# jasonleebrown/machisplin

Hardware: AMD Instinct MI355X
Metric: grid Mcells/s (ensemble+TPS predict) + TPS-solve GFLOP/s (higher is better)
Workload: dtype f64; 1 GPU; cfg3: 5000 stations, 3 covariates, 10000x10000 grid, 6-model ensemble + TPS residual correction; stations=5000, covariates=3 x float32 planes resident in HBM, rf_trees=500, tps_mode=global (one fit on all stations, GCV lambda, V73:748-753), parallelism=rowband1 + bcast(coef) + 1 all-gather

## Files before the change

include/machisplin_hip.h:

```cpp
#ifndef MACHISPLIN_HIP_H
#define MACHISPLIN_HIP_H

#include <stdint.h>

#if defined(__GNUC__)
#define MHS_API __attribute__((visibility("default")))
#else
#define MHS_API
#endif

#ifdef __cplusplus
extern "C" {
#endif

enum {
    MHS_OK = 0,
    MHS_ERR_INVALID = 1,
    MHS_ERR_HIP = 2,
    MHS_ERR_NODEVICE = 3,
    MHS_ERR_NUMERIC = 4,
    MHS_ERR_ALLOC = 5
};

enum { MHS_F64 = 0, MHS_F32 = 1, MHS_I16 = 2 };

enum {
    MHS_GCV_FIELDS = 0,
    MHS_GCV_CONVERGED = 1
};

typedef struct mhs_grid {
    double xmin, ymax;
    double xres, yres;
    int64_t nrow, ncol;
} mhs_grid;

typedef struct mhs_tps mhs_tps;
typedef struct mhs_model mhs_model;

MHS_API const char *mhs_last_error(void);
MHS_API const char *mhs_version(void);
MHS_API int mhs_init(int device);
MHS_API int mhs_shutdown(void);
MHS_API int mhs_device_count(int *count);
MHS_API int mhs_sync(void *stream);
MHS_API int mhs_fit_reserve_cus(int n_cus, int *previous);
MHS_API int mhs_timer_start(void *stream);
MHS_API int mhs_timer_stop(void *stream, double *elapsed_ms);

MHS_API int mhs_tps_fit(const double *xy, const double *y, int64_t N, double lambda,
                int gcv_mode, mhs_tps **out);
MHS_API int mhs_tps_fit_many(const double *const *xy, const double *const *y, const int64_t *N, int64_t count,
                             double lambda, int gcv_mode, mhs_tps **out, int *status);
MHS_API int mhs_tps_reduction_cache(int enable);
MHS_API int mhs_host_gcv_tridiag(const double *diag, const double *offdiag, const double *g,
                                 int64_t m, int64_t n_unique, int64_t n_obs, double pure_ss,
                                 double lambda, int gcv_mode, double *lambda_out,
                                 double *gcv_out, double *eff_df_out, double *q_out);
MHS_API int mhs_host_gcv_band(const double *ab, int bw, const double *g, int64_t m, int64_t n_unique,
                              int64_t n_obs, double pure_ss, double lambda, int gcv_mode,
                              double *lambda_out, double *gcv_out, double *eff_df_out, double *q_out);
MHS_API int mhs_band32_reduce(const double *B, const double *g, int64_t m, double *ab, double *gq,
                              const double *r, double *Qr, int *breakdown);
MHS_API int mhs_band32_gcv_terms(const double *ab, const double *g, int64_t m, const double *lambda, int n_lambda,
                                 int deriv, double *neg, double *tr_inv, double *gM2g);
MHS_API int mhs_band32_solve(const double *ab, const double *g, int64_t m, double lambda, double *q);
MHS_API int mhs_tps_from_coef(const double *knots_uv ,
                      const double *c, const double *d3, int64_t n, double lambda,
                      const double *center2, const double *scale2, mhs_tps **out);
MHS_API int mhs_tps_size(const mhs_tps *t, int64_t *n);
MHS_API int mhs_tps_get(const mhs_tps *t, double *c, double *d3, double *knots_uv, double *lambda,
                double *center2, double *scale2, double *eff_df, double *gcv);
MHS_API int mhs_tps_free(mhs_tps *t);

MHS_API int mhs_tps_predict_grid(const mhs_tps *t, const mhs_grid *g, int64_t r0, int64_t r1,
                         int64_t c0, int64_t c1, double *out_host);
MHS_API int mhs_tps_eval_mode(int mode);
MHS_API int mhs_tps_eval_plan(const mhs_tps *t, int *tile_cols, int *tile_rows, int64_t *node_pairs,
                      int64_t *cell_pairs);
MHS_API int mhs_tps_predict_grid_dev(const mhs_tps *t, const mhs_grid *g, int64_t r0, int64_t r1,
                             int64_t c0, int64_t c1, double *out_dev, int64_t ld, void *stream);
MHS_API int mhs_tps_predict_rows_dev(const mhs_tps *t, const mhs_grid *g, int64_t r0, int64_t r1, int64_t c0, int64_t c1,
                                     int64_t b0, int64_t b1, double *out_dev, int64_t ld, void *stream);
MHS_API int mhs_tps_predict_points(const mhs_tps *t, const double *xy, int64_t n, double *out_host);

#define MHS_TPS_SE_MAX_N 2048
MHS_API int mhs_tps_sigma2(const mhs_tps *t, double *sigma2);
MHS_API int mhs_tps_predict_se_points(const mhs_tps *t, const double *xy, int64_t n, double sigma2, double *out_host);
MHS_API int mhs_tps_predict_se_grid(const mhs_tps *t, const mhs_grid *g, int64_t r0, int64_t r1, int64_t c0, int64_t c1,
                                    double sigma2, double *out_host);
MHS_API int mhs_tps_predict_se_grid_dev(const mhs_tps *t, const mhs_grid *g, int64_t r0, int64_t r1, int64_t c0, int64_t c1,
                                        double sigma2, double *out_dev, int64_t ld, void *stream);


MHS_API int mhs_lm_load(const double *coef, int p, mhs_model **out);
MHS_API int mhs_lm_fit(const double *X, const double *y, int64_t n, int p, double *coef);
MHS_API int mhs_svr_fit(const double *X, const double *y, int64_t n, int p, double sigma, double C, double epsilon,
                        double tol, int64_t max_iter, double *beta, double *b, double *x_center, double *x_scale,
                        double *y_center, double *y_scale, int64_t *n_iter);
MHS_API int mhs_nnet_fit(const double *X, const double *y, int64_t n, int p, int size, double *wts, int maxit,
                         double abstol, double reltol, double *value, int *counts, int *fail);
MHS_API int mhs_nnet_load(const double *wts, int p, int size, double y_scale, double y_shift,
                          mhs_model **out);
MHS_API int mhs_earth_load(const double *coef, const int32_t *dirs, const double *cuts, int nterms,
                           int p, mhs_model **out);
MHS_API int mhs_svr_load(const double *alpha, const double *sv, int64_t nsv, int p, double b,
                         double sigma, const double *x_center, const double *x_scale,
                         double y_center, double y_scale, mhs_model **out);
MHS_API int mhs_gbm_load(double init_f, int64_t n_trees, const int64_t *tree_offsets,
                         const int32_t *split_var, const double *split_val, const int32_t *left,
                         const int32_t *right, const int32_t *missing, int p, mhs_model **out);
MHS_API int mhs_gbm_grow_many(int count, const double *const *X, const double *const *y, const int64_t *n, int p,
                              const int32_t *const *bags, const int64_t *bag_size, int n_new, int interaction_depth,
                              int n_minobsinnode, double shrinkage, int first_call, double *const *F, double *init_f,
                              int64_t *const *tree_offsets, int32_t *const *split_var, double *const *split_val,
                              int32_t *const *left, int32_t *const *right, int32_t *const *missing);
MHS_API int mhs_rf_load(int64_t n_trees, const int64_t *tree_offsets, const int32_t *left,
                        const int32_t *right, const int32_t *status, const int32_t *best_var,
                        const double *split, const double *node_pred, int p, mhs_model **out);
MHS_API int mhs_model_free(mhs_model *m);

typedef struct mhs_stack {
    const void *data;
    int32_t n_layers;
    int32_t dtype;
    int64_t plane_stride;
    int64_t ld;
    double nodata;
} mhs_stack;

MHS_API int mhs_predict_dev(const mhs_model *m, const mhs_grid *g, const mhs_stack *covars,
                            int64_t r0, int64_t r1, int64_t c0, int64_t c1, double weight,
                            int accumulate, double *out_dev, int64_t ld, void *stream);
MHS_API int mhs_members_predict_dev(const mhs_model *const *models, const double *weights, int n_models,
                            const mhs_grid *g, const mhs_stack *covars, int64_t r0, int64_t r1, int64_t c0,
                            int64_t c1, int accumulate, double *out_dev, int64_t ld, void *stream);
MHS_API int mhs_ensemble_predict_dev(const mhs_model *const *models, const double *weights,
                                     int n_models, double wt_total, const mhs_grid *g,
                                     const mhs_stack *covars, int64_t r0, int64_t r1, int64_t c0,
                                     int64_t c1, double *out_dev, int64_t ld, void *stream);
MHS_API int mhs_ensemble_predict(const mhs_model *const *models, const double *weights,
                                 int n_models, double wt_total, const mhs_grid *g,
                                 const mhs_stack *covars, int64_t r0, int64_t r1, int64_t c0,
                                 int64_t c1, double *out_host);
MHS_API int mhs_predict_points(const mhs_model *m, const double *X, int64_t n, double *out_host);
MHS_API int mhs_gbm_staged_points(const mhs_model *m, const double *X, int64_t n, int step, double *out_host);
MHS_API int mhs_model_info(const mhs_model *m, int *kind, int *p, int64_t *n_trees);

MHS_API int mhs_gbm_probe_last(const mhs_model *m, int64_t *cost, int64_t *count);
MHS_API int mhs_residual_points(const mhs_model *const *models, const double *weights, int n_models, double wt_total,
                                const double *X, const double *resp, int64_t n, double *out_host);

MHS_API int mhs_scale_add_dev(const double *a, double divisor, const double *b, double *out,
                              int64_t n, void *stream);


MHS_API int mhs_crop_window(const mhs_grid *g, const double *ext4, int64_t *win4);
MHS_API int mhs_step3_tile_windows(const mhs_grid *g, int64_t tile_edge, double fit_overlap,
                                   double keep_overlap, int64_t *nRx, int64_t *nCx,
                                   int64_t *fit_win, int64_t *keep_win, int64_t capacity);
MHS_API int mhs_tiles_create_windows(const mhs_grid *g, int64_t out_ncol, int64_t out_nrow,
                                     double feather_d, double *boxes, int64_t *win);
MHS_API int mhs_seam_count(int64_t nRx, int64_t nCx, int64_t *n_seams);
MHS_API int mhs_cells_from_xy(const mhs_grid *g, const double *xy, int64_t n, int64_t *rows,
                              int64_t *cols);
MHS_API int mhs_mosaic_feather_dev(const mhs_grid *g, int64_t nRx, int64_t nCx,
                                   const int64_t *tile_win, const double *const *tile_dev,
                                   int merge_mode, double *out_dev, int64_t ld,
                                   int64_t *seam_win_out, void *stream);
MHS_API int mhs_mosaic_feather(const mhs_grid *g, int64_t nRx, int64_t nCx, const int64_t *tile_win,
                               const double *const *tile_host, int merge_mode, double *out_host);
MHS_API int mhs_gather_cells_dev(const double *plane_dev, int64_t ld, const int64_t *rows,
                                 const int64_t *cols, int64_t n, double *out_host, void *stream);

MHS_API int mhs_tps_surface(const mhs_grid *g, const double *xy, const double *resid, int64_t n,
                            const double *cov1_at_stations, int64_t tile_edge, double lambda,
                            int gcv_mode, double *out_host, int64_t *tiles_out);
MHS_API int mhs_tps_tiles_dev(const mhs_grid *g, const double *xy, const double *resid, int64_t n,
                      const double *cov1_at_stations, int64_t tile_edge, double lambda, int gcv_mode,
                      const int64_t *tile_ids, int64_t n_ids, double *const *out_dev_ptrs);
MHS_API int mhs_tps_surface_dev(const mhs_grid *g, const double *xy, const double *resid, int64_t n,
                                const double *cov1_at_stations, int64_t tile_edge, double lambda,
                                int gcv_mode, double *out_dev, int64_t ld, int64_t *tiles_out,
                                void *stream);
MHS_API int mhs_tps_surface_se(const mhs_grid *g, const double *xy, const double *resid, int64_t n,
                               const double *cov1_at_stations, int64_t tile_edge, double lambda, int gcv_mode,
                               double *out_host, int64_t *tiles_out);
MHS_API int mhs_tps_surface_se_dev(const mhs_grid *g, const double *xy, const double *resid, int64_t n,
                                   const double *cov1_at_stations, int64_t tile_edge, double lambda,
                                   int gcv_mode, double *out_dev, int64_t ld, int64_t *tiles_out,
                                   void *stream);

MHS_API int mhs_init_devices(int n_devices, const int *device_ids);
MHS_API int mhs_device_slots(int *n_slots, int *device_ids );

typedef struct mhs_multi_stack mhs_multi_stack;
MHS_API int mhs_multi_stack_create(const mhs_grid *g, const mhs_stack *covars_host, double slot0_share,
                                   mhs_multi_stack **out);
MHS_API int mhs_multi_stack_free(mhs_multi_stack *ms);
MHS_API int mhs_plan_row_bands(int64_t nrow, int n_slots, double slot0_share, int64_t *r0, int64_t *r1, int64_t *band,
                               int64_t *lead);
MHS_API int mhs_multi_stack_bands(const mhs_multi_stack *ms, int *n_slots, int64_t *r0 , int64_t *r1 );

typedef struct mhs_mltps_info {
    double rsq_model, rsq_final;
    double lambda;
    int64_t n_knots;
    int64_t tiles_rows, tiles_cols;
    int32_t used_tps;
    int32_t n_slots;
    int32_t collective;
    int32_t reserved_;
    int64_t band_r0[16], band_r1[16];
    double band_ms[16];
    double tiles_ms[16];
    double fit_ms;
    double step_ms;
    double upload_ms, download_ms;
    double suggested_slot0_share;
    int64_t tiles_pulled_bytes[16];
    int32_t tiles_owned[16];
} mhs_mltps_info;

MHS_API int mhs_mltps_grid_multi_dev(const mhs_model *const *models, const double *weights, int n_models,
                                     double wt_total, mhs_multi_stack *ms, const double *X, const double *resp,
                                     int64_t n, int64_t tile_edge, double lambda, int gcv_mode, int gather,
                                     mhs_mltps_info *info );
MHS_API int mhs_multi_final_download(const mhs_multi_stack *ms, double *final_host);
MHS_API int mhs_multi_final_dev(const mhs_multi_stack *ms, int slot, double **band_dev, int64_t *r0, int64_t *r1,
                                double **full_dev);
MHS_API int mhs_multi_trim(void);
MHS_API int mhs_mltps_grid_multi(const mhs_model *const *models, const double *weights, int n_models, double wt_total,
                                 const mhs_grid *g, const mhs_stack *covars_host, const double *X, const double *resp,
                                 int64_t n, int64_t tile_edge, double lambda, int gcv_mode, double slot0_share,
                                 double *final_host, mhs_mltps_info *info );

typedef struct mhs_unit {
    const mhs_model *const *models;
    const double *weights;
    int32_t n_models, reserved_;
    double wt_total;
    const double *X, *resp;
    int64_t n;
} mhs_unit;
typedef struct mhs_units_info {
    int32_t n_slots, reserved_;
    int64_t n_units;
    double step_ms, unit_ms_sum, unit_ms_max;
    double slot_ms[16];
} mhs_units_info;
MHS_API int mhs_tiles_units_multi(const mhs_grid *g, const mhs_stack *covars_host, int64_t out_ncol, int64_t out_nrow,
                                  double feather_d, int n_layers, const mhs_unit *units, int tps, int64_t tile_edge,
                                  double lambda, int gcv_mode, double *const *merged_host, double *rsq,
                                  mhs_units_info *info );

typedef struct mhs_tiff_info {
    int64_t width, height;
    int32_t bits, sample_format;
    int32_t compression, n_ifd;
    int32_t dtype;
    int32_t has_geo;
    double nodata;
    double xmin, ymax, xres, yres;
} mhs_tiff_info;
MHS_API int mhs_tiff_info_read(const char *path, int ifd, mhs_tiff_info *out);
MHS_API int mhs_tiff_read_host(const char *path, int ifd, void *out, int64_t out_bytes);
MHS_API int mhs_tiff_read_dev(const char *path, int ifd, void *out_dev, int64_t ld_elems, void *stream);
MHS_API int mhs_tiff_write_f32_host(const char *path, const mhs_grid *g, const float *data, double nodata,
                                    int compression);
MHS_API int mhs_tiff_write_f32_dev(const char *path, const mhs_grid *g, const double *plane_dev, int64_t ld,
                                   double nodata, int compression, void *stream);
MHS_API int mhs_tfw_read(const char *path, double *six);

#ifdef __cplusplus
}
#endif
#endif
```

machisplin_amd/_lib.py:

```python
from __future__ import annotations

import atexit
import ctypes as C
import os
import threading

_HERE = os.path.dirname(os.path.abspath(__file__))
LIB_PATH = os.path.join(_HERE, "libmachisplin_hip.so")

OK, ERR_INVALID, ERR_HIP, ERR_NODEVICE, ERR_NUMERIC, ERR_ALLOC = range(6)
F64, F32, I16 = 0, 1, 2
GCV_FIELDS, GCV_CONVERGED = 0, 1


class MhsError(RuntimeError):
    def __init__(self, code: int, msg: str):
        super().__init__(f"[mhs status {code}] {msg}")
        self.code = code


class Grid(C.Structure):
    _fields_ = [("xmin", C.c_double), ("ymax", C.c_double), ("xres", C.c_double),
                ("yres", C.c_double), ("nrow", C.c_int64), ("ncol", C.c_int64)]


class Stack(C.Structure):
    _fields_ = [("data", C.c_void_p), ("n_layers", C.c_int32), ("dtype", C.c_int32),
                ("plane_stride", C.c_int64), ("ld", C.c_int64), ("nodata", C.c_double)]


class TiffInfo(C.Structure):
    _fields_ = [("width", C.c_int64), ("height", C.c_int64), ("bits", C.c_int32), ("sample_format", C.c_int32),
                ("compression", C.c_int32), ("n_ifd", C.c_int32), ("dtype", C.c_int32), ("has_geo", C.c_int32),
                ("nodata", C.c_double), ("xmin", C.c_double), ("ymax", C.c_double), ("xres", C.c_double),
                ("yres", C.c_double)]


class MltpsInfo(C.Structure):
    _fields_ = [("rsq_model", C.c_double), ("rsq_final", C.c_double), ("lambda_", C.c_double), ("n_knots", C.c_int64),
                ("tiles_rows", C.c_int64), ("tiles_cols", C.c_int64), ("used_tps", C.c_int32), ("n_slots", C.c_int32),
                ("collective", C.c_int32), ("reserved_", C.c_int32), ("band_r0", C.c_int64 * 16), ("band_r1", C.c_int64 * 16),
                ("band_ms", C.c_double * 16), ("tiles_ms", C.c_double * 16), ("fit_ms", C.c_double), ("step_ms", C.c_double),
                ("upload_ms", C.c_double), ("download_ms", C.c_double), ("suggested_slot0_share", C.c_double),
                ("tiles_pulled_bytes", C.c_int64 * 16), ("tiles_owned", C.c_int32 * 16)]


class Unit(C.Structure):
    _fields_ = [("models", C.POINTER(C.c_void_p)), ("weights", C.POINTER(C.c_double)), ("n_models", C.c_int32),
                ("reserved_", C.c_int32), ("wt_total", C.c_double), ("X", C.c_void_p), ("resp", C.c_void_p), ("n", C.c_int64)]


class UnitsInfo(C.Structure):
    _fields_ = [("n_slots", C.c_int32), ("reserved_", C.c_int32), ("n_units", C.c_int64), ("step_ms", C.c_double),
                ("unit_ms_sum", C.c_double), ("unit_ms_max", C.c_double), ("slot_ms", C.c_double * 16)]


_dp = C.POINTER(C.c_double)
_vp = C.c_void_p
_i64 = C.c_int64

SIGNATURES = {
    "mhs_last_error": (C.c_char_p, []),
    "mhs_version": (C.c_char_p, []),
    "mhs_init": (C.c_int, [C.c_int]),
    "mhs_shutdown": (C.c_int, []),
    "mhs_device_count": (C.c_int, [C.POINTER(C.c_int)]),
    "mhs_sync": (C.c_int, [_vp]),
    "mhs_tps_reduction_cache": (C.c_int, [C.c_int]),
    "mhs_fit_reserve_cus": (C.c_int, [C.c_int, C.POINTER(C.c_int)]),
    "mhs_timer_start": (C.c_int, [_vp]),
    "mhs_timer_stop": (C.c_int, [_vp, _dp]),
    "mhs_tps_fit": (C.c_int, [_vp, _vp, _i64, C.c_double, C.c_int, C.POINTER(_vp)]),
    "mhs_tps_fit_many": (C.c_int, [_vp, _vp, _vp, _i64, C.c_double, C.c_int, _vp, _vp]),
    "mhs_host_gcv_tridiag": (C.c_int, [_vp, _vp, _vp, _i64, _i64, _i64, C.c_double, C.c_double, C.c_int,
                                       _dp, _dp, _dp, _vp]),
    "mhs_host_gcv_band": (C.c_int, [_vp, C.c_int, _vp, _i64, _i64, _i64, C.c_double, C.c_double, C.c_int,
                                    _dp, _dp, _dp, _vp]),
    "mhs_band32_reduce": (C.c_int, [_vp, _vp, _i64, _vp, _vp, _vp, _vp, C.POINTER(C.c_int)]),
    "mhs_band32_gcv_terms": (C.c_int, [_vp, _vp, _i64, _vp, C.c_int, C.c_int, _vp, _vp, _vp]),
    "mhs_band32_solve": (C.c_int, [_vp, _vp, _i64, C.c_double, _vp]),
    "mhs_tps_from_coef": (C.c_int, [_vp, _vp, _vp, _i64, C.c_double, _vp, _vp, C.POINTER(_vp)]),
    "mhs_tps_size": (C.c_int, [_vp, C.POINTER(_i64)]),
    "mhs_tps_get": (C.c_int, [_vp, _vp, _vp, _vp, _dp, _vp, _vp, _dp, _dp]),
    "mhs_tps_free": (C.c_int, [_vp]),
    "mhs_tps_predict_grid": (C.c_int, [_vp, C.POINTER(Grid), _i64, _i64, _i64, _i64, _vp]),
    "mhs_tps_predict_grid_dev": (C.c_int, [_vp, C.POINTER(Grid), _i64, _i64, _i64, _i64, _vp, _i64, _vp]),
    "mhs_tps_predict_rows_dev": (C.c_int, [_vp, C.POINTER(Grid), _i64, _i64, _i64, _i64, _i64, _i64, _vp, _i64, _vp]),
    "mhs_tps_predict_points": (C.c_int, [_vp, _vp, _i64, _vp]),
    "mhs_tps_sigma2": (C.c_int, [_vp, _dp]),
    "mhs_tps_predict_se_points": (C.c_int, [_vp, _vp, _i64, C.c_double, _vp]),
    "mhs_tps_predict_se_grid": (C.c_int, [_vp, C.POINTER(Grid), _i64, _i64, _i64, _i64, C.c_double, _vp]),
    "mhs_tps_predict_se_grid_dev": (C.c_int, [_vp, C.POINTER(Grid), _i64, _i64, _i64, _i64, C.c_double, _vp, _i64, _vp]),
    "mhs_tps_eval_mode": (C.c_int, [C.c_int]),
    "mhs_tps_eval_plan": (C.c_int, [_vp, C.POINTER(C.c_int), C.POINTER(C.c_int), C.POINTER(_i64), C.POINTER(_i64)]),
    "mhs_lm_load": (C.c_int, [_vp, C.c_int, C.POINTER(_vp)]),
    "mhs_lm_fit": (C.c_int, [_vp, _vp, _i64, C.c_int, _vp]),
    "mhs_svr_fit": (C.c_int, [_vp, _vp, _i64, C.c_int, C.c_double, C.c_double, C.c_double, C.c_double, _i64, _vp, _vp, _vp, _vp,
                              _vp, _vp, _vp]),
    "mhs_nnet_fit": (C.c_int, [_vp, _vp, _i64, C.c_int, C.c_int, _vp, C.c_int, C.c_double, C.c_double, _vp, _vp, _vp]),
    "mhs_nnet_load": (C.c_int, [_vp, C.c_int, C.c_int, C.c_double, C.c_double, C.POINTER(_vp)]),
    "mhs_earth_load": (C.c_int, [_vp, _vp, _vp, C.c_int, C.c_int, C.POINTER(_vp)]),
    "mhs_svr_load": (C.c_int, [_vp, _vp, _i64, C.c_int, C.c_double, C.c_double, _vp, _vp, C.c_double,
                               C.c_double, C.POINTER(_vp)]),
    "mhs_gbm_load": (C.c_int, [C.c_double, _i64, _vp, _vp, _vp, _vp, _vp, _vp, C.c_int, C.POINTER(_vp)]),
    "mhs_gbm_grow_many": (C.c_int, [C.c_int, _vp, _vp, _vp, C.c_int, _vp, _vp, C.c_int, C.c_int, C.c_int, C.c_double, C.c_int, _vp, _vp,
                                    _vp, _vp, _vp, _vp, _vp, _vp]),
    "mhs_rf_load": (C.c_int, [_i64, _vp, _vp, _vp, _vp, _vp, _vp, _vp, C.c_int, C.POINTER(_vp)]),
    "mhs_model_free": (C.c_int, [_vp]),
    "mhs_predict_dev": (C.c_int, [_vp, C.POINTER(Grid), C.POINTER(Stack), _i64, _i64, _i64, _i64,
                                  C.c_double, C.c_int, _vp, _i64, _vp]),
    "mhs_members_predict_dev": (C.c_int, [C.POINTER(_vp), _dp, C.c_int, C.POINTER(Grid), C.POINTER(Stack), C.c_int64, C.c_int64,
                                          C.c_int64, C.c_int64, C.c_int, C.c_void_p, C.c_int64, C.c_void_p]),
    "mhs_ensemble_predict_dev": (C.c_int, [C.POINTER(_vp), _dp, C.c_int, C.c_double, C.POINTER(Grid),
                                           C.POINTER(Stack), _i64, _i64, _i64, _i64, _vp, _i64, _vp]),
    "mhs_ensemble_predict": (C.c_int, [C.POINTER(_vp), _dp, C.c_int, C.c_double, C.POINTER(Grid),
                                       C.POINTER(Stack), _i64, _i64, _i64, _i64, _vp]),
    "mhs_predict_points": (C.c_int, [_vp, _vp, _i64, _vp]),
    "mhs_gbm_staged_points": (C.c_int, [_vp, _vp, _i64, C.c_int, _vp]),
    "mhs_model_info": (C.c_int, [_vp, _vp, _vp, _vp]),
    "mhs_gbm_probe_last": (C.c_int, [_vp, _vp, _vp]),
    "mhs_residual_points": (C.c_int, [_vp, _vp, C.c_int, C.c_double, _vp, _vp, _i64, _vp]),
    "mhs_scale_add_dev": (C.c_int, [_vp, C.c_double, _vp, _vp, _i64, _vp]),
    "mhs_crop_window": (C.c_int, [C.POINTER(Grid), _vp, _vp]),
    "mhs_step3_tile_windows": (C.c_int, [C.POINTER(Grid), _i64, C.c_double, C.c_double, C.POINTER(_i64),
                                         C.POINTER(_i64), _vp, _vp, _i64]),
    "mhs_tiles_create_windows": (C.c_int, [C.POINTER(Grid), _i64, _i64, C.c_double, _vp, _vp]),
    "mhs_seam_count": (C.c_int, [_i64, _i64, C.POINTER(_i64)]),
    "mhs_cells_from_xy": (C.c_int, [C.POINTER(Grid), _vp, _i64, _vp, _vp]),
    "mhs_mosaic_feather_dev": (C.c_int, [C.POINTER(Grid), _i64, _i64, _vp, C.POINTER(_vp), C.c_int, _vp, _i64,
                                         _vp, _vp]),
    "mhs_mosaic_feather": (C.c_int, [C.POINTER(Grid), _i64, _i64, _vp, C.POINTER(_vp), C.c_int, _vp]),
    "mhs_gather_cells_dev": (C.c_int, [_vp, _i64, _vp, _vp, _i64, _vp, _vp]),
    "mhs_tiff_info_read": (C.c_int, [C.c_char_p, C.c_int, C.POINTER(TiffInfo)]),
    "mhs_tiff_read_host": (C.c_int, [C.c_char_p, C.c_int, _vp, _i64]),
    "mhs_tiff_read_dev": (C.c_int, [C.c_char_p, C.c_int, _vp, _i64, _vp]),
    "mhs_tiff_write_f32_host": (C.c_int, [C.c_char_p, C.POINTER(Grid), _vp, C.c_double, C.c_int]),
    "mhs_tiff_write_f32_dev": (C.c_int, [C.c_char_p, C.POINTER(Grid), _vp, _i64, C.c_double, C.c_int, _vp]),
    "mhs_tfw_read": (C.c_int, [C.c_char_p, _dp]),
    "mhs_tps_surface": (C.c_int, [C.POINTER(Grid), _vp, _vp, _i64, _vp, _i64, C.c_double, C.c_int, _vp, _vp]),
    "mhs_tps_tiles_dev": (C.c_int, [C.POINTER(Grid), _vp, _vp, _i64, _vp, _i64, C.c_double, C.c_int, _vp, _i64, _vp]),
    "mhs_tps_surface_dev": (C.c_int, [C.POINTER(Grid), _vp, _vp, _i64, _vp, _i64, C.c_double, C.c_int, _vp, _i64,
                                      _vp, _vp]),
    "mhs_tps_surface_se": (C.c_int, [C.POINTER(Grid), _vp, _vp, _i64, _vp, _i64, C.c_double, C.c_int, _vp, _vp]),
    "mhs_tps_surface_se_dev": (C.c_int, [C.POINTER(Grid), _vp, _vp, _i64, _vp, _i64, C.c_double, C.c_int, _vp, _i64,
                                         _vp, _vp]),
    "mhs_init_devices": (C.c_int, [C.c_int, C.POINTER(C.c_int)]),
    "mhs_device_slots": (C.c_int, [C.POINTER(C.c_int), C.POINTER(C.c_int)]),
    "mhs_multi_stack_create": (C.c_int, [C.POINTER(Grid), C.POINTER(Stack), C.c_double, C.POINTER(_vp)]),
    "mhs_multi_stack_free": (C.c_int, [_vp]),
    "mhs_plan_row_bands": (C.c_int, [_i64, C.c_int, C.c_double, _vp, _vp, C.POINTER(_i64), C.POINTER(_i64)]),
    "mhs_multi_trim": (C.c_int, []),
    "mhs_multi_stack_bands": (C.c_int, [_vp, C.POINTER(C.c_int), _vp, _vp]),
    "mhs_mltps_grid_multi_dev": (C.c_int, [C.POINTER(_vp), _dp, C.c_int, C.c_double, _vp, _vp, _vp, _i64, _i64, C.c_double,
                                           C.c_int, C.c_int, C.POINTER(MltpsInfo)]),
    "mhs_multi_final_download": (C.c_int, [_vp, _vp]),
    "mhs_multi_final_dev": (C.c_int, [_vp, C.c_int, C.POINTER(_vp), C.POINTER(_i64), C.POINTER(_i64), C.POINTER(_vp)]),
    "mhs_mltps_grid_multi": (C.c_int, [C.POINTER(_vp), _dp, C.c_int, C.c_double, C.POINTER(Grid), C.POINTER(Stack), _vp, _vp,
                                       _i64, _i64, C.c_double, C.c_int, C.c_double, _vp, C.POINTER(MltpsInfo)]),
    "mhs_tiles_units_multi": (C.c_int, [C.POINTER(Grid), C.POINTER(Stack), _i64, _i64, C.c_double, C.c_int, C.POINTER(Unit),
                                        C.c_int, _i64, C.c_double, C.c_int, C.POINTER(_vp), _vp, C.POINTER(UnitsInfo)]),
}

_lock = threading.Lock()
_lib = None
_inited_device = None


def _hip_runtimes_mapped():
    libs = set()
    try:
        with open("/proc/self/maps") as f:
            for line in f:
                if "libamdhip64" in line:
                    libs.add(line.split()[-1])
    except OSError:
        pass
    return libs


def load() -> C.CDLL:
    global _lib
    with _lock:
        if _lib is not None:
            return _lib
        if not os.path.exists(LIB_PATH):
            raise ImportError(
                f"{LIB_PATH} is missing: build it with `python -c 'import __graft_entry__ as g; g.build()'` "
                "(or `make -C machisplin_amd/csrc`).  machisplin_amd has no CPU fallback.")
        import torch
        lib = C.CDLL(LIB_PATH, mode=C.RTLD_GLOBAL)
        for name, (res, args) in SIGNATURES.items():
            fn = getattr(lib, name)
            fn.restype = res
            fn.argtypes = args
        mapped = _hip_runtimes_mapped()
        if len(mapped) > 1:
            raise ImportError(f"two HIP runtimes are mapped into this process: {sorted(mapped)}")
        _lib = lib
        return lib


def check(rc: int) -> None:
    if rc != OK:
        raise MhsError(rc, load().mhs_last_error().decode(errors="replace"))


def init(device: int | None = None) -> int:
    global _inited_device
    lib = load()
    if device is None:
        if _inited_device is not None:
            return _inited_device
        device = int(os.environ.get("LOCAL_RANK", "0"))
    if _inited_device == device:
        return device
    check(lib.mhs_init(int(device)))
    if _inited_device is None:
        atexit.register(_shutdown)
    _inited_device = device
    return device


def _shutdown() -> None:
    global _inited_device
    if _lib is not None and _inited_device is not None:
        _lib.mhs_shutdown()
        _inited_device = None


def lib() -> C.CDLL:
    if _inited_device is None:
        init()
    return load()


def ptr(a) -> int:
    if a is None:
        return None
    if hasattr(a, "data_ptr"):
        return a.data_ptr()
    return a.ctypes.data
```

machisplin_amd/csrc/common.h:

```cpp
#pragma once
#include <hip/hip_runtime.h>
#include <stdint.h>
#include <chrono>
#include <memory>
#include <mutex>
#include <string>
#include <vector>
#include "machisplin_hip.h"

namespace mhs {

void set_error(const char *fmt, ...);
int hip_fail(hipError_t e, const char *what, const char *file, int line);

#define MHS_HIP(call)                                                        \
    do {                                                                     \
        hipError_t e_ = (call);                                              \
        if (e_ != hipSuccess) return mhs::hip_fail(e_, #call, __FILE__, __LINE__); \
    } while (0)

#define MHS_REQUIRE(cond, msg)                                               \
    do {                                                                     \
        if (!(cond)) { mhs::set_error("%s: %s", __func__, msg); return MHS_ERR_INVALID; } \
    } while (0)

constexpr int LOG_TAB_BITS = 10;
constexpr int LOG_TAB_N = 1 << LOG_TAB_BITS;

constexpr int FIT_PANEL_CUS = 32;
struct FitLane {
    hipStream_t s = nullptr, s2 = nullptr;
    hipStream_t ms = nullptr, ms2 = nullptr;
    hipStream_t s2r = nullptr;
    std::vector<hipEvent_t> pool;
    char *arena = nullptr;
    size_t arena_cap = 0;
    double *pinned = nullptr;
};

struct Context {
    bool ready = false;
    int device = -1;
    hipStream_t stream = nullptr;
    std::vector<FitLane *> lanes;
    FitLane *batch = nullptr;
    double2 *log_tab = nullptr;
    double *exp_tab = nullptr;
    double *points_arena = nullptr;
    size_t points_arena_cap = 0;
    char *mosaic_arena[2] = {nullptr, nullptr};
    size_t mosaic_arena_cap[2] = {0, 0};
    double *surface_arena = nullptr;
    size_t surface_arena_cap = 0;
    hipEvent_t ev0 = nullptr, ev1 = nullptr;
    char *pipe_arena = nullptr;
    size_t pipe_arena_cap = 0;
    hipStream_t pipe_h2d = nullptr, pipe_d2h = nullptr, pipe_comp = nullptr;
    hipEvent_t pipe_in[8] = {}, pipe_done[8] = {}, pipe_out[8] = {};
    hipStream_t upload = nullptr;
    int n_cu = 0;
    int reserved_cus = 0;
    int masked_cus = 0;
    hipStream_t masked_stream = nullptr;
    std::vector<uint32_t> comp_mask;
    hipEvent_t mask_ev0 = nullptr, mask_ev1 = nullptr;
};
constexpr int MAX_SLOTS = 16;
int current_slot();
int slot_count();
int bind_slot(int slot);
struct SlotBind {
    int prev;
    explicit SlotBind(int slot) : prev(current_slot()) { (void)bind_slot(slot); }
    ~SlotBind() { (void)bind_slot(prev); }
    SlotBind(const SlotBind &) = delete;
    SlotBind &operator=(const SlotBind &) = delete;
};
std::mutex &pipe_mutex();
int host_pipe(size_t arena_bytes);
std::mutex &mask_mutex();
std::mutex &mosaic_mutex();
int cpu_budget();
int mosaic_lane();
void set_mosaic_lane(int lane);
Context &ctx();
Context &ctx_slot(int slot);
int fit_lane(int i, FitLane **out);
int batch_lane(FitLane **out);
std::mutex &batch_mutex();
int tps_fit_lane(FitLane &L, const double *xy, const double *y, int64_t N, double lambda, int gcv_mode,
                 int gcv_threads, mhs_tps **out);
void *pool_alloc(size_t bytes);
void pool_release(void *p);
void pool_clear();
int require_ready();
int mosaic_feather_impl(const mhs_grid *g, int64_t nRx, int64_t nCx, const int64_t *tile_win, const double *const *tile_dev,
                        int merge_mode, double *out_dev, int64_t ld, int64_t *seam_win_out, void *stream, bool finite_tiles,
                        int64_t row_lo = 0, int64_t row_hi = -1);
void reduction_cache_clear();
void multi_reset();
int h2d_sync(void *dst, const void *src, size_t bytes);
inline hipStream_t pick_stream(void *s) { return (hipStream_t)s; }
inline double now_ms() {
    return std::chrono::duration<double, std::milli>(std::chrono::steady_clock::now().time_since_epoch()).count();
}

template <typename T>
struct DevBuf {
    T *p = nullptr;
    size_t n = 0;
    DevBuf() = default;
    DevBuf(const DevBuf &) = delete;
    DevBuf &operator=(const DevBuf &) = delete;
    ~DevBuf() { if (p) (void)hipFree(p); }
    hipError_t alloc(size_t count) {
        if (p) { (void)hipFree(p); p = nullptr; }
        n = count;
        return hipMalloc((void **)&p, (count ? count : 1) * sizeof(T));
    }
    T *release() { T *q = p; p = nullptr; return q; }
};

struct Knot { double u, v, cw, pad; };

}

struct mhs_tps;
namespace mhs {
struct TpsPrep;
struct SeState;
void se_state_free(SeState *s);
int upload_knots(mhs_tps *t);
int tps_free_quiet(mhs_tps *t);
int tps_predict_rows_dev(const mhs_tps *t, const mhs_grid *g, int64_t r0, int64_t r1, int64_t c0, int64_t c1,
                         int64_t b0, int64_t b1, double *out_dev, int64_t ld, void *stream);
}

struct mhs_model;
namespace mhs {
int model_on_slot(const mhs_model *m, int slot, const mhs_model **out);
int members_rows_dev(const mhs_model *const *models, const double *weights, int n_models, int accumulate, int scale, double wt_total,
                     const mhs_grid *g, const void *buf, int64_t buf_r0, int64_t buf_r1, int n_layers, int dtype, int64_t ld,
                     double nodata, int64_t b0, int64_t b1, double *out_dev, int64_t ld_out, hipStream_t st);
int ensemble_band_dev(const mhs_model *const *models, const double *weights, int n_models, double wt_total, const mhs_grid *g,
                      const void *band_data, int n_layers, int dtype, int64_t ld, double nodata, int64_t b0, int64_t b1,
                      double *out_dev, int64_t ld_out, hipStream_t st);
}

struct mhs_tps {
    int64_t n = 0;
    double lambda = 0, eff_df = 0, gcv = 0;
    double center[2] = {0, 0}, scale[2] = {1, 1};
    double d[3] = {0, 0, 0};
    std::vector<double> c;
    std::vector<double> knots_uv;
    mhs::Knot *knots_dev = nullptr;
    struct FarPlan {
        double xmin = 0, ymax = 0, xres = 0, yres = 0;
        int64_t r0 = -1, r1 = -1, c0 = -1, c1 = -1;
        int tx = 0, ty = 0, ntx = 0, nty = 0;
        mhs::Knot *sorted_dev = nullptr;
        int *bin_start_dev = nullptr;
        double *nodes_dev = nullptr;
        double *lx_dev = nullptr, *ly_dev = nullptr;
        size_t nodes_cap = 0, bins_cap = 0, lx_cap = 0, ly_cap = 0;
        bool last_used = false;
        hipStream_t last_stream = nullptr;
        bool in_flight = false;
        int64_t node_pairs = 0, cell_pairs = 0;
    } far;
    std::mutex mu;
    std::shared_ptr<const mhs::TpsPrep> prep;
    mhs::SeState *se = nullptr;
};
```

machisplin_amd/csrc/multi.hip:

```cpp
#include <atomic>
#include <chrono>
#include <cmath>
#include <condition_variable>
#include <cstdio>
#include <cstdlib>
#include <cstring>
#include <deque>
#include <dlfcn.h>
#include <mutex>
#include <string>
#include <thread>
#include <vector>
#include "common.h"

using namespace mhs;

namespace {

constexpr int64_t BAND_ROWS_ALIGN = 16;

struct MultiSlot {
    hipStream_t s = nullptr;
    hipEvent_t e0 = nullptr, e1 = nullptr;
    hipStream_t u = nullptr;
    hipEvent_t up[5] = {}, dn[5] = {};
    hipStream_t h = nullptr;
};
MultiSlot g_ms[MAX_SLOTS];
std::mutex g_ms_mu;

int multi_slot(int slot, MultiSlot **out) {
    std::lock_guard<std::mutex> lk(g_ms_mu);
    MultiSlot &m = g_ms[slot];
    if (!m.s) {
        MHS_HIP(hipStreamCreateWithFlags(&m.s, hipStreamNonBlocking));
        MHS_HIP(hipEventCreate(&m.e0));
        MHS_HIP(hipEventCreate(&m.e1));
        int prio_lo = 0, prio_hi = 0;
        MHS_HIP(hipDeviceGetStreamPriorityRange(&prio_lo, &prio_hi));
        MHS_HIP(hipStreamCreateWithPriority(&m.u, hipStreamNonBlocking, prio_lo));
        MHS_HIP(hipStreamCreateWithPriority(&m.h, hipStreamNonBlocking, prio_lo));
        for (hipEvent_t &e : m.up) MHS_HIP(hipEventCreateWithFlags(&e, hipEventDisableTiming));
        for (hipEvent_t &e : m.dn) MHS_HIP(hipEventCreateWithFlags(&e, hipEventDisableTiming));
    }
    *out = &m;
    return MHS_OK;
}

typedef void *nccl_comm;
struct Rccl {
    void *h = nullptr;
    int (*CommInitAll)(nccl_comm *, int, const int *) = nullptr;
    int (*CommDestroy)(nccl_comm) = nullptr;
    int (*AllGather)(const void *, void *, size_t, int, nccl_comm, hipStream_t) = nullptr;
    const char *(*GetErrorString)(int) = nullptr;
    nccl_comm comm[MAX_SLOTS] = {};
    int n = 0;
    bool tried = false, usable = false;
    std::string why;
};
Rccl g_rccl;
std::mutex g_rccl_mu;
constexpr int NCCL_FLOAT64 = 8;

bool slots_distinct() {
    const int n = slot_count();
    for (int a = 0; a < n; ++a)
        for (int b = a + 1; b < n; ++b)
            if (ctx_slot(a).device == ctx_slot(b).device) return false;
    return true;
}

void rccl_prepare() {
    std::lock_guard<std::mutex> lk(g_rccl_mu);
    const int n = slot_count();
    if (g_rccl.tried && g_rccl.n == n) return;
    g_rccl.tried = true; g_rccl.usable = false; g_rccl.n = n;
    if (!slots_distinct()) { g_rccl.why = "slots share a physical device (RCCL needs one device per rank): peer copies instead"; return; }
    if (getenv("MHS_MULTI_NO_RCCL")) { g_rccl.why = "MHS_MULTI_NO_RCCL is set: peer copies instead"; return; }
    if (!g_rccl.h) {
        for (const char *name : {"librccl.so.1", "librccl.so", "/opt/rocm/lib/librccl.so.1"}) {
            g_rccl.h = dlopen(name, RTLD_NOW | RTLD_GLOBAL);
            if (g_rccl.h) break;
        }
        if (!g_rccl.h) { g_rccl.why = std::string("librccl not found: ") + dlerror(); return; }
        g_rccl.CommInitAll = (int (*)(nccl_comm *, int, const int *))dlsym(g_rccl.h, "ncclCommInitAll");
        g_rccl.CommDestroy = (int (*)(nccl_comm))dlsym(g_rccl.h, "ncclCommDestroy");
        g_rccl.AllGather = (int (*)(const void *, void *, size_t, int, nccl_comm, hipStream_t))dlsym(g_rccl.h, "ncclAllGather");
        g_rccl.GetErrorString = (const char *(*)(int))dlsym(g_rccl.h, "ncclGetErrorString");
        if (!g_rccl.CommInitAll || !g_rccl.CommDestroy || !g_rccl.AllGather) { g_rccl.why = "librccl lacks ncclCommInitAll / ncclAllGather"; return; }
    }
    int devs[MAX_SLOTS];
    for (int k = 0; k < n; ++k) devs[k] = ctx_slot(k).device;
    const int rc = g_rccl.CommInitAll(g_rccl.comm, n, devs);
    if (rc != 0) {
        g_rccl.why = std::string("ncclCommInitAll failed: ") + (g_rccl.GetErrorString ? g_rccl.GetErrorString(rc) : "?");
        return;
    }
    g_rccl.usable = true;
    g_rccl.why = "rccl";
}

void rccl_reset() {
    std::lock_guard<std::mutex> lk(g_rccl_mu);
    if (g_rccl.usable && g_rccl.CommDestroy)
        for (int k = 0; k < g_rccl.n; ++k) if (g_rccl.comm[k]) { (void)g_rccl.CommDestroy(g_rccl.comm[k]); g_rccl.comm[k] = nullptr; }
    g_rccl.tried = g_rccl.usable = false;
    g_rccl.n = 0;
}

struct Barrier {
    std::mutex mu;
    std::condition_variable cv;
    int n, waiting = 0;
    uint64_t phase = 0;
    explicit Barrier(int n_) : n(n_) {}
    void wait() {
        std::unique_lock<std::mutex> lk(mu);
        const uint64_t ph = phase;
        if (++waiting == n) { waiting = 0; ++phase; cv.notify_all(); }
        else cv.wait(lk, [&] { return phase != ph; });
    }
};

struct Team {
    int n;
    Barrier bar;
    std::atomic<int> rc{MHS_OK};
    std::mutex err_mu;
    std::string err;
    explicit Team(int n_) : n(n_), bar(n_) {}
    bool failed() const { return rc.load() != MHS_OK; }
    void fail(int code) {
        int expected = MHS_OK;
        if (rc.compare_exchange_strong(expected, code)) {
            std::lock_guard<std::mutex> lk(err_mu);
            err = mhs_last_error();
        }
    }
    template <typename F>
    int run(F body) {
        const int home = current_slot();
        std::vector<std::thread> th;
        auto wrap = [&](int slot) {
            SlotBind bind(slot);
            body(slot);
        };
        for (int k = 1; k < n; ++k) th.emplace_back(wrap, k);
        wrap(0);
        for (std::thread &t : th) t.join();
        (void)bind_slot(home);
        if (failed()) { set_error("%s", err.c_str()); return rc.load(); }
        return MHS_OK;
    }
};

#define TEAM_DO(team, expr)                                      \
    do {                                                         \
        if (!(team).failed()) { const int rc_ = (expr); if (rc_ != MHS_OK) (team).fail(rc_); } \
    } while (0)

struct BandPlan {
    int64_t band = 0, lead = 0;
    std::vector<int64_t> r0, r1;
};

BandPlan plan_bands(int64_t nrow, int n, double slot0_share) {
    BandPlan p;
    p.r0.assign((size_t)n, 0); p.r1.assign((size_t)n, 0);
    if (n == 1) { p.band = nrow; p.r1[0] = nrow; return p; }
    const int64_t even = (nrow + n - 1) / n;
    const int64_t align = even >= BAND_ROWS_ALIGN ? BAND_ROWS_ALIGN : 1;
    auto up = [&](int64_t v) { return (v + align - 1) / align * align; };
    auto equal = [&] {
        p.band = up(even); p.lead = 0;
        for (int k = 0; k < n; ++k) { p.r0[(size_t)k] = std::min<int64_t>(k * p.band, nrow); p.r1[(size_t)k] = std::min<int64_t>((k + 1) * p.band, nrow); }
    };
    if (std::isnan(slot0_share)) { equal(); return p; }
    const double sh = std::min(std::max(slot0_share, 0.0), 1.0);
    int64_t n0 = std::min<int64_t>(nrow, (int64_t)llround(sh * (double)nrow / (double)align) * align);
    const int64_t rest = nrow - n0, others = n - 1;
    const int64_t h = up((rest + others - 1) / others);
    if (n0 > h) { equal(); return p; }
    p.band = std::max(h, n0); p.lead = p.band - n0;
    p.r0[0] = 0; p.r1[0] = n0;
    for (int k = 1; k < n; ++k) {
        p.r0[(size_t)k] = std::min<int64_t>(n0 + (k - 1) * h, nrow);
        p.r1[(size_t)k] = std::min<int64_t>(n0 + k * h, nrow);
    }
    return p;
}

}

struct MultiBand {
    int64_t r0 = 0, r1 = 0;
    char *cov = nullptr;
    double *ens = nullptr;
    double *tot = nullptr;
    double *full = nullptr;
    double *tiles = nullptr;
    size_t tiles_cap = 0;
};

struct mhs_multi_stack {
    mhs_grid g{};
    int C = 0, dtype = 0;
    int64_t ld = 0;
    double nodata = NAN;
    int n = 0;
    int dev[MAX_SLOTS] = {};
    BandPlan plan;
    MultiBand b[MAX_SLOTS];
    int used_tps = 0;
    bool gathered = false;
    bool have_result = false;
    const mhs_stack *pending = nullptr;
    double *pending_out = nullptr;
    bool downloaded = false;
    double upload_ms = 0;
    double download_ms = 0;
};

namespace {

size_t elem_size(int dtype) { return dtype == MHS_F64 ? 8 : dtype == MHS_F32 ? 4 : 2; }

struct Balance { int n = 0; int64_t nrow = 0, ncol = 0, stations = 0; double share = NAN; };
Balance g_balance;
std::mutex g_balance_mu;

mhs_multi_stack *g_host_ms = nullptr;
std::mutex g_host_mu;
struct UnitsArena { char *base = nullptr; size_t cap = 0; };
UnitsArena g_units_arena[MAX_SLOTS];

constexpr int RING_BUFS = 8, SINK_THREADS = 3;
constexpr size_t RING_CHUNK = (size_t)8 << 20;
struct PinnedRing { char *buf[RING_BUFS] = {}; hipEvent_t ev[RING_BUFS] = {}; bool ok = false; };
PinnedRing g_ring[MAX_SLOTS];

int ring_prepare(int slot) {
    PinnedRing &R = g_ring[slot];
    if (R.ok) return MHS_OK;
    for (int b = 0; b < RING_BUFS; ++b) {
        if (!R.buf[b]) MHS_HIP(hipHostMalloc((void **)&R.buf[b], RING_CHUNK, hipHostMallocDefault));
        if (!R.ev[b]) MHS_HIP(hipEventCreateWithFlags(&R.ev[b], hipEventDisableTiming));
    }
    R.ok = true;
    return MHS_OK;
}

class HostSink {
  public:
    HostSink(int slot, hipStream_t st) : slot_(slot), st_(st), R_(g_ring[slot]) {
        for (int b = 0; b < RING_BUFS; ++b) free_[b] = true;
        const int nth = std::min(SINK_THREADS, std::max(1, cpu_budget() / (4 * std::max(1, slot_count()))));
        for (int w = 0; w < nth; ++w) th_.emplace_back([this] { work(); });
    }
    ~HostSink() {
        { std::lock_guard<std::mutex> lk(mu_); stop_ = true; }
        cv_.notify_all();
        for (std::thread &t : th_) t.join();
    }
    int download(void *dst, const void *src, size_t bytes) {
        size_t off = 0;
        for (int c = 0; off < bytes; ++c) {
            const size_t sz = std::min(RING_CHUNK, bytes - off);
            int b = -1;
            {
                std::unique_lock<std::mutex> lk(mu_);
                cv_.wait(lk, [&] { for (int q = 0; q < RING_BUFS; ++q) if (free_[q]) { b = q; return true; } return false; });
                free_[b] = false;
            }
            hipError_t e = hipMemcpyAsync(R_.buf[b], (const char *)src + off, sz, hipMemcpyDeviceToHost, st_);
            if (e == hipSuccess) e = hipEventRecord(R_.ev[b], st_);
            if (e != hipSuccess) {
                set_error("HostSink: %s", hipGetErrorString(e));
                std::lock_guard<std::mutex> lk(mu_);
                free_[b] = true; rc_ = MHS_ERR_HIP;
                break;
            }
            {
                std::lock_guard<std::mutex> lk(mu_);
                jobs_.push_back(Job{b, (char *)dst + off, sz});
                ++pending_;
            }
            cv_.notify_all();
            off += sz;
        }
        std::unique_lock<std::mutex> lk(mu_);
        cv_.wait(lk, [&] { return pending_ == 0; });
        return rc_;
    }

  private:
    struct Job { int b; char *dst; size_t sz; };
    void work() {
        SlotBind bind(slot_);
        for (;;) {
            Job j;
            {
                std::unique_lock<std::mutex> lk(mu_);
                cv_.wait(lk, [&] { return stop_ || !jobs_.empty(); });
                if (jobs_.empty()) return;
                j = jobs_.front(); jobs_.pop_front();
            }
            const hipError_t e = hipEventSynchronize(R_.ev[j.b]);
            if (e == hipSuccess) memcpy(j.dst, R_.buf[j.b], j.sz);
            {
                std::lock_guard<std::mutex> lk(mu_);
                if (e != hipSuccess) rc_ = MHS_ERR_HIP;
                free_[j.b] = true; --pending_;
            }
            cv_.notify_all();
        }
    }
    int slot_;
    hipStream_t st_;
    PinnedRing &R_;
    std::vector<std::thread> th_;
    std::mutex mu_;
    std::condition_variable cv_;
    std::deque<Job> jobs_;
    bool free_[RING_BUFS];
    int pending_ = 0, rc_ = MHS_OK;
    bool stop_ = false;
};

bool stack_current(const mhs_multi_stack *ms) {
    if (ms->n != slot_count()) return false;
    for (int k = 0; k < ms->n; ++k) if (!ctx_slot(k).ready || ctx_slot(k).device != ms->dev[k]) return false;
    return true;
}

int free_stack(mhs_multi_stack *ms) {
    if (!ms) return MHS_OK;
    if (!stack_current(ms)) { delete ms; return MHS_OK; }
    const int home = current_slot();
    for (int k = 0; k < ms->n; ++k) {
        (void)bind_slot(k);
        MultiBand &b = ms->b[k];
        if (g_ms[k].s) (void)hipStreamSynchronize(g_ms[k].s);
        for (void *q : {(void *)b.cov, (void *)b.ens, (void *)b.tot, (void *)b.full, (void *)b.tiles})
            if (q) (void)hipFree(q);
    }
    (void)bind_slot(home);
    delete ms;
    return MHS_OK;
}

}

static void trim_caches() {
    std::lock_guard<std::mutex> lk(g_host_mu);
    if (g_host_ms) { bool alive = true; for (int k = 0; k < g_host_ms->n; ++k) alive = alive && ctx_slot(k).ready; if (alive) free_stack(g_host_ms); else delete g_host_ms; }
    g_host_ms = nullptr;
    const int home = current_slot();
    for (int k = 0; k < MAX_SLOTS; ++k) {
        if (ctx_slot(k).ready) {
            (void)bind_slot(k);
            if (g_units_arena[k].base) { (void)hipDeviceSynchronize(); (void)hipFree(g_units_arena[k].base); }
            for (int b = 0; b < RING_BUFS; ++b) {
                if (g_ring[k].buf[b]) (void)hipHostFree(g_ring[k].buf[b]);
                if (g_ring[k].ev[b]) (void)hipEventDestroy(g_ring[k].ev[b]);
            }
        }
        g_units_arena[k] = UnitsArena();
        g_ring[k] = PinnedRing();
    }
    (void)bind_slot(home);
}

extern "C" int mhs_multi_trim(void) {
    if (int rc = require_ready()) return rc;
    trim_caches();
    return MHS_OK;
}

void mhs::multi_reset() {
    trim_caches();
    rccl_reset();
    std::lock_guard<std::mutex> lk(g_ms_mu);
    for (int k = 0; k < MAX_SLOTS; ++k) {
        MultiSlot &m = g_ms[k];
        if (!m.s) continue;
        if (ctx_slot(k).ready) {
            SlotBind bind(k);
            (void)hipStreamSynchronize(m.s); (void)hipStreamDestroy(m.s);
            (void)hipEventDestroy(m.e0); (void)hipEventDestroy(m.e1);
            if (m.u) { (void)hipStreamSynchronize(m.u); (void)hipStreamDestroy(m.u); }
            if (m.h) { (void)hipStreamSynchronize(m.h); (void)hipStreamDestroy(m.h); }
            for (hipEvent_t e : m.up) if (e) (void)hipEventDestroy(e);
            for (hipEvent_t e : m.dn) if (e) (void)hipEventDestroy(e);
        }
        m = MultiSlot();
    }
}

extern "C" {

static int stack_build(const mhs_grid *g, const mhs_stack *covars_host, double slot0_share, bool upload, mhs_multi_stack **out) {
    if (int rc = require_ready()) return rc;
    MHS_REQUIRE(g && covars_host && covars_host->data && out, "NULL argument");
    MHS_REQUIRE(g->nrow > 0 && g->ncol > 0 && g->xres > 0 && g->yres > 0, "bad grid geometry");
    MHS_REQUIRE(covars_host->n_layers >= 1 && covars_host->n_layers <= 64, "bad number of layers");
    MHS_REQUIRE(covars_host->dtype == MHS_F64 || covars_host->dtype == MHS_F32 || covars_host->dtype == MHS_I16, "bad stack dtype");
    MHS_REQUIRE(covars_host->ld >= g->ncol && covars_host->plane_stride >= covars_host->ld * g->nrow, "stack strides smaller than the grid");
    const int n = slot_count();
    mhs_multi_stack *ms = new mhs_multi_stack();
    ms->g = *g; ms->C = covars_host->n_layers; ms->dtype = covars_host->dtype; ms->ld = g->ncol; ms->nodata = covars_host->nodata;
    ms->n = n;
    for (int k = 0; k < n; ++k) ms->dev[k] = ctx_slot(k).device;
    ms->plan = plan_bands(g->nrow, n, slot0_share);
    const size_t esz = elem_size(ms->dtype);
    Team team(n);
    const int rc = team.run([&](int slot) {
        MultiBand &b = ms->b[slot];
        b.r0 = ms->plan.r0[(size_t)slot]; b.r1 = ms->plan.r1[(size_t)slot];
        const int64_t nb = b.r1 - b.r0;
        auto work = [&]() -> int {
            MultiSlot *S = nullptr;
            if (int rc2 = multi_slot(slot, &S)) return rc2;
            if (nb == 0) return MHS_OK;
            const size_t plane = (size_t)nb * (size_t)ms->ld * esz;
            MHS_HIP(hipMalloc((void **)&b.cov, plane * (size_t)ms->C));
            MHS_HIP(hipMalloc((void **)&b.ens, sizeof(double) * (size_t)nb * (size_t)g->ncol));
            MHS_HIP(hipMalloc((void **)&b.tot, sizeof(double) * (size_t)nb * (size_t)g->ncol));
            if (!upload) return MHS_OK;
            for (int k = 0; k < ms->C; ++k) {
                const char *src = (const char *)covars_host->data + ((size_t)k * covars_host->plane_stride + (size_t)b.r0 * covars_host->ld) * esz;
                if (covars_host->ld == g->ncol)
                    MHS_HIP(hipMemcpyAsync(b.cov + plane * k, src, plane, hipMemcpyHostToDevice, S->s));
                else
                    MHS_HIP(hipMemcpy2DAsync(b.cov + plane * k, (size_t)ms->ld * esz, src, (size_t)covars_host->ld * esz, (size_t)g->ncol * esz,
                                             (size_t)nb, hipMemcpyHostToDevice, S->s));
            }
            MHS_HIP(hipStreamSynchronize(S->s));
            return MHS_OK;
        };
        TEAM_DO(team, work());
    });
    if (rc) { free_stack(ms); return rc; }
    *out = ms;
    return MHS_OK;
}

int mhs_multi_stack_create(const mhs_grid *g, const mhs_stack *covars_host, double slot0_share, mhs_multi_stack **out) {
    return stack_build(g, covars_host, slot0_share, true, out);
}

int mhs_multi_stack_free(mhs_multi_stack *ms) { return free_stack(ms); }

int mhs_plan_row_bands(int64_t nrow, int n_slots, double slot0_share, int64_t *r0, int64_t *r1, int64_t *band, int64_t *lead) {
    MHS_REQUIRE(nrow > 0 && n_slots >= 1 && n_slots <= MAX_SLOTS && r0 && r1, "bad arguments");
    const BandPlan p = plan_bands(nrow, n_slots, slot0_share);
    for (int k = 0; k < n_slots; ++k) { r0[k] = p.r0[(size_t)k]; r1[k] = p.r1[(size_t)k]; }
    if (band) *band = p.band;
    if (lead) *lead = p.lead;
    return MHS_OK;
}

int mhs_multi_stack_bands(const mhs_multi_stack *ms, int *n_slots, int64_t *r0, int64_t *r1) {
    MHS_REQUIRE(ms && n_slots, "NULL argument");
    *n_slots = ms->n;
    for (int k = 0; k < ms->n; ++k) {
        if (r0) r0[k] = ms->b[k].r0;
        if (r1) r1[k] = ms->b[k].r1;
    }
    return MHS_OK;
}

}

namespace {

enum { BANDS_UP = 0, BANDS_UP_F64 = 1, BANDS_DOWN = 2 };
constexpr int MAX_SUB = 5;
int sub_bands(int64_t r0, int64_t r1, int mode, int64_t cut[MAX_SUB + 1]) {
    static const int pct[3][MAX_SUB] = {{4, 16, 40, 40, 0}, {3, 6, 13, 28, 50}, {48, 30, 14, 6, 2}};
    const int nq = mode == BANDS_UP ? 4 : 5;
    const int64_t nb = r1 - r0;
    cut[0] = r0;
    for (int q = 0, a = 0; q < nq; ++q) {
        a += pct[mode][q];
        cut[q + 1] = q == nq - 1 ? r1 : std::min(r1, std::max(cut[q], (r0 + nb * a / 100 + BAND_ROWS_ALIGN / 2) / BAND_ROWS_ALIGN * BAND_ROWS_ALIGN));
    }
    return nq;
}

struct Uploader {
    std::thread th;
    std::mutex mu;
    std::condition_variable cv;
    int issued = 0, rc = MHS_OK;
    std::string err;
    template <typename F>
    void start(int slot, int nq, F issue) {
        th = std::thread([this, slot, nq, issue] {
            SlotBind bind(slot);
            for (int q = 0; q < nq; ++q) {
                const int r = issue(q);
                std::lock_guard<std::mutex> lk(mu);
                if (r) { rc = r; err = mhs_last_error(); issued = nq; } else issued = q + 1;
                cv.notify_all();
                if (r) break;
            }
        });
    }
    int wait(int q) {
        std::unique_lock<std::mutex> lk(mu);
        cv.wait(lk, [&] { return issued > q; });
        if (rc) set_error("%s", err.c_str());
        return rc;
    }
    void join() { if (th.joinable()) th.join(); }
    ~Uploader() { join(); }
};

struct StepShared {
    std::vector<double> resid;
    double rsq_model = NAN, tss = NAN;
    int64_t nk = 0;
    std::vector<double> c, knots_uv;
    double d[3] = {0, 0, 0}, center[2] = {0, 0}, scale[2] = {1, 1}, lambda = NAN;
    int64_t nRx = 1, nCx = 1;
    std::vector<int64_t> fit_win, keep_win;
    std::vector<int> owner;
    std::vector<size_t> tile_cells;
    std::vector<int64_t> slot_off[MAX_SLOTS];
    size_t slot_need[MAX_SLOTS] = {};
    int64_t pulled_bytes[MAX_SLOTS] = {};
    std::vector<double> f_actual;
    int used_tps = 0;
    double rsq_final = NAN;
    double fit_ms = 0, band_ms[MAX_SLOTS] = {}, tiles_ms[MAX_SLOTS] = {}, upload_ms[MAX_SLOTS] = {}, download_ms[MAX_SLOTS] = {};
};

}

extern "C" {

int mhs_mltps_grid_multi_dev(const mhs_model *const *models, const double *weights, int n_models, double wt_total,
                             mhs_multi_stack *ms, const double *X, const double *resp, int64_t n, int64_t tile_edge,
                             double lambda, int gcv_mode, int gather, mhs_mltps_info *info) {
    if (int rc = require_ready()) return rc;
    MHS_REQUIRE(models && weights && n_models >= 1 && n_models <= 8 && ms && X && resp && n > 3, "bad arguments");
    MHS_REQUIRE(stack_current(ms), "the stack was built for another set of device slots");
    MHS_REQUIRE(wt_total != 0.0 && !std::isnan(wt_total), "wt_total must be non-zero");
    const int N = ms->n;
    const mhs_grid g = ms->g;
    const int p = ms->C + 2;
    int kind0 = 0, p0 = 0;
    for (int k = 0; k < n_models; ++k) {
        MHS_REQUIRE(models[k] != nullptr, "NULL model");
        if (int rc = mhs_model_info(models[k], &kind0, &p0, nullptr)) return rc;
        MHS_REQUIRE(p0 == p, "a model's predictor count does not match the stack (layers + 2)");
    }
    const double t_step0 = now_ms();
    const double *knots = X + (size_t)(p - 2) * (size_t)n;
    std::vector<int64_t> rows((size_t)n), cols((size_t)n);
    if (int rc = mhs_cells_from_xy(&g, knots, n, rows.data(), cols.data())) return rc;
    StepShared S;
    S.f_actual.assign((size_t)n, NAN);
    int64_t nt = 1;
    if (tile_edge > 0) {
        if (int rc = mhs_step3_tile_windows(&g, tile_edge, 0.2, 0.025, &S.nRx, &S.nCx, nullptr, nullptr, 0)) return rc;
        nt = S.nRx * S.nCx;
    }
    const bool tiled = nt > 1;
    if (tiled) {
        S.fit_win.resize((size_t)nt * 4); S.keep_win.resize((size_t)nt * 4);
        if (int rc = mhs_step3_tile_windows(&g, tile_edge, 0.2, 0.025, &S.nRx, &S.nCx, S.fit_win.data(), S.keep_win.data(), nt)) return rc;
        S.tile_cells.resize((size_t)nt);
        S.owner.assign((size_t)nt, 0);
        for (int k = 0; k < N; ++k) S.slot_off[k].assign((size_t)nt, -1);
        for (int64_t h = 0; h < nt; ++h) {
            const int64_t *kw = &S.keep_win[(size_t)h * 4];
            S.tile_cells[(size_t)h] = ((size_t)((kw[1] - kw[0]) * (kw[3] - kw[2])) + 31) & ~(size_t)31;
            int64_t best_rows = -1;
            for (int k = 0; k < N; ++k) {
                const int64_t ov = std::min(kw[1], ms->b[k].r1) - std::max(kw[0], ms->b[k].r0);
                if (ov > best_rows) { best_rows = ov; S.owner[(size_t)h] = k; }
            }
            for (int k = 0; k < N; ++k) {
                const bool reaches = ms->b[k].r1 > ms->b[k].r0 && kw[0] < ms->b[k].r1 && kw[1] > ms->b[k].r0;
                if (reaches || S.owner[(size_t)h] == k) { S.slot_off[k][(size_t)h] = (int64_t)S.slot_need[k]; S.slot_need[k] += S.tile_cells[(size_t)h]; }
            }
        }
    }
    if (gather) rccl_prepare();
    const bool use_rccl = gather && g_rccl.usable;
    std::vector<const mhs_model *> mods((size_t)N * (size_t)n_models);
    std::vector<mhs_tps *> tps((size_t)N, nullptr);
    Team team(N);
    const int rc = team.run([&](int slot) {
        MultiBand &b = ms->b[slot];
        const int64_t nb = b.r1 - b.r0;
        MultiSlot *M = nullptr;
        TEAM_DO(team, multi_slot(slot, &M));
        for (int k = 0; k < n_models; ++k) TEAM_DO(team, model_on_slot(models[k], slot, &mods[(size_t)slot * n_models + k]));
        const mhs_model *const *my = &mods[(size_t)slot * n_models];
        auto fit = [&]() -> int {
            S.resid.resize((size_t)n);
            if (int rc2 = mhs_residual_points(my, weights, n_models, wt_total, X, resp, n, S.resid.data())) return rc2;
            long double msum = 0.0L, ss = 0.0L, rs = 0.0L;
            for (int64_t i = 0; i < n; ++i) msum += resp[i];
            const double mean = (double)(msum / (long double)n);
            for (int64_t i = 0; i < n; ++i) { ss += (long double)((resp[i] - mean) * (resp[i] - mean)); rs += (long double)(S.resid[(size_t)i] * S.resid[(size_t)i]); }
            S.tss = (double)ss; S.rsq_model = 1.0 - (double)rs / (double)ss;
            if (tiled) return MHS_OK;
            const double t0 = now_ms();
            mhs_tps *t = nullptr;
            if (int rc2 = mhs_tps_fit(knots, S.resid.data(), n, lambda, gcv_mode, &t)) return rc2;
            S.fit_ms = now_ms() - t0;
            tps[0] = t;
            if (int rc2 = mhs_tps_size(t, &S.nk)) return rc2;
            S.c.resize((size_t)S.nk); S.knots_uv.resize((size_t)S.nk * 2);
            return mhs_tps_get(t, S.c.data(), S.d, S.knots_uv.data(), &S.lambda, S.center, S.scale, nullptr, nullptr);
        };
        const bool piped = ms->pending && ms->pending_out;
        const int banded = n_models > 1 ? n_models - 1 : 1;
        Uploader up;
        if (ms->pending && nb > 0 && !team.failed()) {
            const mhs_stack *h = ms->pending;
            const size_t esz = elem_size(ms->dtype), plane = (size_t)nb * (size_t)ms->ld * esz;
            int64_t cut[MAX_SUB + 1];
            const int nq = sub_bands(b.r0, b.r1, ms->dtype == MHS_F64 ? BANDS_UP_F64 : BANDS_UP, cut);
            const double t0 = now_ms();
            up.start(slot, nq, [=, &S](int q) -> int {
                const int64_t rows_q = cut[q + 1] - cut[q];
                for (int k = 0; k < ms->C && rows_q > 0; ++k) {
                    const char *src = (const char *)h->data + ((size_t)k * h->plane_stride + (size_t)cut[q] * h->ld) * esz;
                    char *dst = b.cov + plane * k + (size_t)(cut[q] - b.r0) * (size_t)ms->ld * esz;
                    if (h->ld == g.ncol)
                        MHS_HIP(hipMemcpyAsync(dst, src, (size_t)rows_q * (size_t)ms->ld * esz, hipMemcpyHostToDevice, M->u));
                    else
                        MHS_HIP(hipMemcpy2DAsync(dst, (size_t)ms->ld * esz, src, (size_t)h->ld * esz, (size_t)g.ncol * esz, (size_t)rows_q,
                                                 hipMemcpyHostToDevice, M->u));
                }
                MHS_HIP(hipEventRecord(M->up[q], M->u));
                if (q == nq - 1) S.upload_ms[slot] = now_ms() - t0;
                return MHS_OK;
            });
            std::thread fitter;
            int fit_rc = MHS_OK;
            std::string fit_err;
            if (slot == 0)
                fitter = std::thread([&] {
                    SlotBind bind(slot);
                    fit_rc = fit();
                    if (fit_rc) fit_err = mhs_last_error();
                });
            auto launch = [&]() -> int {
                MHS_HIP(hipEventRecord(M->e0, M->s));
                for (int q = 0; q < nq; ++q) {
                    if (int rc2 = up.wait(q)) return rc2;
                    MHS_HIP(hipStreamWaitEvent(M->s, M->up[q], 0));
                    if (int rc2 = members_rows_dev(my, weights, banded, 0, 0, wt_total, &g, b.cov, b.r0, b.r1, ms->C, ms->dtype, ms->ld, ms->nodata,
                                                   cut[q], cut[q + 1], b.ens + (size_t)(cut[q] - b.r0) * (size_t)g.ncol, g.ncol, M->s)) return rc2;
                }
                if (!piped) {
                    if (int rc2 = members_rows_dev(my + banded, weights + banded, n_models - banded, 1, 1, wt_total, &g, b.cov, b.r0, b.r1,
                                                   ms->C, ms->dtype, ms->ld, ms->nodata, b.r0, b.r1, b.ens, g.ncol, M->s)) return rc2;
                    MHS_HIP(hipEventRecord(M->e1, M->s));
                }
                return MHS_OK;
            };
            TEAM_DO(team, launch());
            if (fitter.joinable()) {
                fitter.join();
                if (fit_rc) { set_error("%s", fit_err.c_str()); team.fail(fit_rc); }
            }
            up.join();
            if (team.failed()) (void)hipStreamSynchronize(M->u);
        } else {
            if (nb > 0 && !team.failed()) {
                auto launch = [&]() -> int {
                    MHS_HIP(hipEventRecord(M->e0, M->s));
                    if (int rc2 = ensemble_band_dev(my, weights, n_models, wt_total, &g, b.cov, ms->C, ms->dtype, ms->ld, ms->nodata, b.r0, b.r1,
                                                    b.ens, g.ncol, M->s)) return rc2;
                    MHS_HIP(hipEventRecord(M->e1, M->s));
                    return MHS_OK;
                };
                TEAM_DO(team, launch());
            }
            if (slot == 0) TEAM_DO(team, fit());
        }
        team.bar.wait();
        auto down = [&]() -> int {
            int64_t cut[MAX_SUB + 1];
            const int nd = sub_bands(b.r0, b.r1, BANDS_DOWN, cut);
            for (int q = 0; q < nd; ++q) {
                const size_t off = (size_t)(cut[q] - b.r0) * (size_t)g.ncol;
                if (cut[q + 1] > cut[q]) {
                    if (int rc2 = members_rows_dev(my + banded, weights + banded, n_models - banded, 1, 1, wt_total, &g, b.cov, b.r0, b.r1, ms->C,
                                                   ms->dtype, ms->ld, ms->nodata, cut[q], cut[q + 1], b.ens + off, g.ncol, M->s)) return rc2;
                    if (int rc2 = mhs_scale_add_dev(b.ens + off, 1.0, b.tot + off, b.tot + off, (cut[q + 1] - cut[q]) * g.ncol, M->s)) return rc2;
                }
                MHS_HIP(hipEventRecord(M->dn[q], M->s));
            }
            MHS_HIP(hipEventRecord(M->e1, M->s));
            const double t0 = now_ms();
            for (int q = 0; q < nd; ++q) {
                if (cut[q + 1] == cut[q]) continue;
                const size_t off = (size_t)(cut[q] - b.r0) * (size_t)g.ncol;
                MHS_HIP(hipStreamWaitEvent(M->u, M->dn[q], 0));
                if (q == nd - 1) S.download_ms[slot] = -now_ms();
                MHS_HIP(hipMemcpyAsync(ms->pending_out + (size_t)b.r0 * (size_t)g.ncol + off, b.tot + off,
                                       sizeof(double) * (size_t)(cut[q + 1] - cut[q]) * (size_t)g.ncol, hipMemcpyDeviceToHost, M->u));
            }
            MHS_HIP(hipStreamSynchronize(M->u));
            S.download_ms[slot] = S.download_ms[slot] < 0 ? S.download_ms[slot] + now_ms() : now_ms() - t0;
            return MHS_OK;
        };
        if (!tiled) {
            if (slot != 0 && nb > 0)
                TEAM_DO(team, mhs_tps_from_coef(S.knots_uv.data(), S.c.data(), S.d, S.nk, S.lambda, S.center, S.scale, &tps[(size_t)slot]));
            if (nb > 0)
                TEAM_DO(team, tps_predict_rows_dev(tps[(size_t)slot], &g, 0, g.nrow, 0, g.ncol, b.r0, b.r1, b.tot, g.ncol, M->s));
            if (piped && nb > 0) {
                const int rcd = team.failed() ? MHS_OK : down();
                if (rcd) { (void)hipStreamSynchronize(M->u); team.fail(rcd); }
            }
        } else {
            const double t0 = now_ms();
            auto my_tiles = [&]() -> int {
                if (b.tiles_cap < S.slot_need[slot]) {
                    if (b.tiles) { MHS_HIP(hipStreamSynchronize(M->s)); MHS_HIP(hipFree(b.tiles)); b.tiles = nullptr; b.tiles_cap = 0; }
                    MHS_HIP(hipMalloc((void **)&b.tiles, sizeof(double) * S.slot_need[slot]));
                    b.tiles_cap = S.slot_need[slot];
                }
                std::vector<int64_t> ids;
                std::vector<double *> outs;
                for (int64_t h = 0; h < nt; ++h)
                    if (S.owner[(size_t)h] == slot) { ids.push_back(h); outs.push_back(b.tiles + S.slot_off[slot][(size_t)h]); }
                if (ids.empty()) return MHS_OK;
                return mhs_tps_tiles_dev(&g, knots, S.resid.data(), n, X , tile_edge, lambda, gcv_mode,
                                         ids.data(), (int64_t)ids.size(), outs.data());
            };
            TEAM_DO(team, my_tiles());
            S.tiles_ms[slot] = now_ms() - t0;
            team.bar.wait();
            auto bring = [&]() -> int {
                if (nb == 0) return MHS_OK;
                std::vector<const double *> ptrs((size_t)nt, nullptr);
                for (int64_t h = 0; h < nt; ++h) {
                    const int64_t *kw = &S.keep_win[(size_t)h * 4];
                    if (!(kw[0] < b.r1 && kw[1] > b.r0)) continue;
                    const int o = S.owner[(size_t)h];
                    ptrs[(size_t)h] = b.tiles + S.slot_off[slot][(size_t)h];
                    if (o == slot) continue;
                    const size_t bytes = sizeof(double) * S.tile_cells[(size_t)h];
                    MHS_HIP(hipMemcpyPeerAsync(b.tiles + S.slot_off[slot][(size_t)h], ctx_slot(slot).device,
                                               ms->b[o].tiles + S.slot_off[o][(size_t)h], ctx_slot(o).device, bytes, M->s));
                    S.pulled_bytes[slot] += (int64_t)bytes;
                }
                return mosaic_feather_impl(&g, S.nRx, S.nCx, S.keep_win.data(), ptrs.data(), 0, b.tot, g.ncol, nullptr, M->s, true, b.r0, b.r1);
            };
            TEAM_DO(team, bring());
            if (piped && nb > 0) {
                const int rcd = team.failed() ? MHS_OK : down();
                if (rcd) { (void)hipStreamSynchronize(M->u); team.fail(rcd); }
            }
        }
        if (nb > 0 && !team.failed()) {
            auto step5 = [&]() -> int {
                if (!piped) if (int rc2 = mhs_scale_add_dev(b.ens, 1.0, b.tot, b.tot, nb * g.ncol, M->s)) return rc2;
                std::vector<int64_t> rr, cc, idx;
                for (int64_t i = 0; i < n; ++i)
                    if (rows[(size_t)i] >= b.r0 && rows[(size_t)i] < b.r1 && cols[(size_t)i] >= 0) {
                        rr.push_back(rows[(size_t)i] - b.r0); cc.push_back(cols[(size_t)i]); idx.push_back(i);
                    }
                std::vector<double> f(rr.size());
                if (int rc2 = mhs_gather_cells_dev(b.tot, g.ncol, rr.data(), cc.data(), (int64_t)rr.size(), f.data(), M->s)) return rc2;
                for (size_t q = 0; q < idx.size(); ++q) S.f_actual[(size_t)idx[q]] = f[q];
                return MHS_OK;
            };
            TEAM_DO(team, step5());
        }
        team.bar.wait();
        if (slot == 0 && !team.failed()) {
            long double rs = 0.0L;
            for (int64_t i = 0; i < n; ++i) { const double e = resp[i] - S.f_actual[(size_t)i]; rs += (long double)(e * e); }
            S.rsq_final = 1.0 - (double)rs / S.tss;
            S.used_tps = S.rsq_final > S.rsq_model ? 1 : 0;
        }
        team.bar.wait();
        const bool go = !team.failed();
        if (piped && nb > 0 && go && !S.used_tps) {
            auto resend = [&]() -> int {
                MHS_HIP(hipMemcpyAsync(ms->pending_out + (size_t)b.r0 * (size_t)g.ncol, b.ens, sizeof(double) * (size_t)nb * (size_t)g.ncol,
                                       hipMemcpyDeviceToHost, M->s));
                return MHS_OK;
            };
            TEAM_DO(team, resend());
        }
        if (gather && go) {
            auto stitch = [&]() -> int {
                const int64_t band = ms->plan.band;
                if (!b.full) MHS_HIP(hipMalloc((void **)&b.full, sizeof(double) * (size_t)band * (size_t)N * (size_t)g.ncol));
                const double *src = S.used_tps ? b.tot : b.ens;
                double *mine = b.full + ((size_t)ms->plan.lead + (size_t)b.r0) * (size_t)g.ncol;
                if (nb > 0) MHS_HIP(hipMemcpyAsync(mine, src, sizeof(double) * (size_t)nb * (size_t)g.ncol, hipMemcpyDeviceToDevice, M->s));
                return MHS_OK;
            };
            int rcs = stitch();
            if (rcs) team.fail(rcs);
            team.bar.wait();
            const bool go2 = !team.failed();
            if (go2 && use_rccl) {
                const size_t count = (size_t)ms->plan.band * (size_t)g.ncol;
                const int rcn = g_rccl.AllGather(b.full + (size_t)slot * count, b.full, count, NCCL_FLOAT64, g_rccl.comm[slot], M->s);
                if (rcn != 0) { set_error("ncclAllGather failed: %s", g_rccl.GetErrorString ? g_rccl.GetErrorString(rcn) : "?"); team.fail(MHS_ERR_HIP); }
            } else if (go2 && nb > 0) {
                auto push = [&]() -> int {
                    const double *mine = b.full + ((size_t)ms->plan.lead + (size_t)b.r0) * (size_t)g.ncol;
                    for (int o = 0; o < N; ++o) {
                        if (o == slot) continue;
                        double *dst = ms->b[o].full + ((size_t)ms->plan.lead + (size_t)b.r0) * (size_t)g.ncol;
                        MHS_HIP(hipMemcpyPeerAsync(dst, ctx_slot(o).device, mine, ctx_slot(slot).device, sizeof(double) * (size_t)nb * (size_t)g.ncol, M->s));
                    }
                    return MHS_OK;
                };
                rcs = push();
                if (rcs) team.fail(rcs);
            }
        }
        if (M) (void)hipStreamSynchronize(M->s);
        if (nb > 0 && M && !team.failed()) {
            float ms_f = 0.f;
            if (hipEventElapsedTime(&ms_f, M->e0, M->e1) == hipSuccess) S.band_ms[slot] = (double)ms_f;
        }
        team.bar.wait();
        if (tps[(size_t)slot]) { (void)mhs_tps_free(tps[(size_t)slot]); tps[(size_t)slot] = nullptr; }
    });
    if (ms->pending) {
        ms->downloaded = !rc && ms->pending_out;
        ms->pending = nullptr; ms->pending_out = nullptr;
        ms->upload_ms = ms->download_ms = 0;
        for (int k = 0; k < N; ++k) { ms->upload_ms = std::max(ms->upload_ms, S.upload_ms[k]); ms->download_ms = std::max(ms->download_ms, S.download_ms[k]); }
    }
    if (rc) return rc;
    ms->used_tps = S.used_tps;
    ms->gathered = gather != 0;
    ms->have_result = true;
    const double step_ms = now_ms() - t_step0;
    double suggested = NAN;
    if (N > 1 && !tiled) {
        double ms_per_row = 0.0;
        int64_t rows_timed = 0;
        for (int k = 0; k < N; ++k) if (ms->b[k].r1 > ms->b[k].r0) { ms_per_row += S.band_ms[k]; rows_timed += ms->b[k].r1 - ms->b[k].r0; }
        if (rows_timed > 0 && ms_per_row > 0) {
            const double cells_ms = ms_per_row / (double)rows_timed * (double)g.nrow;
            const double s0 = 1.0 / N - S.fit_ms * (N - 1) / ((double)N * cells_ms);
            suggested = std::min(std::max(s0, 0.0), 1.0 / N);
            std::lock_guard<std::mutex> lk(g_balance_mu);
            const bool same_shape = g_balance.n == N && g_balance.nrow == g.nrow && g_balance.ncol == g.ncol && g_balance.stations == n;
            if (!same_shape || !(fabs(suggested - g_balance.share) <= 0.05 / (double)N))
                g_balance = Balance{N, g.nrow, g.ncol, n, suggested};
        }
    }
    if (info) {
        memset(info, 0, sizeof(*info));
        info->rsq_model = S.rsq_model; info->rsq_final = S.rsq_final; info->lambda = tiled ? NAN : S.lambda;
        info->n_knots = tiled ? 0 : S.nk; info->used_tps = S.used_tps; info->n_slots = N;
        info->tiles_rows = S.nRx; info->tiles_cols = S.nCx;
        info->collective = !gather ? 0 : use_rccl ? 1 : 2;
        info->fit_ms = S.fit_ms; info->step_ms = step_ms; info->suggested_slot0_share = suggested;
        for (int k = 0; k < N; ++k) {
            info->band_r0[k] = ms->b[k].r0; info->band_r1[k] = ms->b[k].r1; info->band_ms[k] = S.band_ms[k]; info->tiles_ms[k] = S.tiles_ms[k];
            info->tiles_pulled_bytes[k] = S.pulled_bytes[k];
            info->tiles_owned[k] = 0;
            for (size_t h = 0; h < S.owner.size(); ++h) if (S.owner[h] == k) ++info->tiles_owned[k];
        }
    }
    return MHS_OK;
}

int mhs_multi_final_download(const mhs_multi_stack *ms, double *final_host) {
    if (int rc = require_ready()) return rc;
    MHS_REQUIRE(ms && final_host && ms->have_result, "no result to download");
    MHS_REQUIRE(stack_current(ms), "the stack was built for another set of device slots");
    Team team(ms->n);
    return team.run([&](int slot) {
        const MultiBand &b = ms->b[slot];
        const int64_t nb = b.r1 - b.r0;
        auto work = [&]() -> int {
            if (nb == 0) return MHS_OK;
            MultiSlot *M = nullptr;
            if (int rc2 = multi_slot(slot, &M)) return rc2;
            const double *src = ms->used_tps ? b.tot : b.ens;
            MHS_HIP(hipMemcpyAsync(final_host + (size_t)b.r0 * (size_t)ms->g.ncol, src, sizeof(double) * (size_t)nb * (size_t)ms->g.ncol,
                                   hipMemcpyDeviceToHost, M->s));
            MHS_HIP(hipStreamSynchronize(M->s));
            return MHS_OK;
        };
        TEAM_DO(team, work());
    });
}

int mhs_multi_final_dev(const mhs_multi_stack *ms, int slot, double **band_dev, int64_t *r0, int64_t *r1, double **full_dev) {
    MHS_REQUIRE(ms && slot >= 0 && slot < ms->n && ms->have_result, "bad arguments");
    const MultiBand &b = ms->b[slot];
    if (band_dev) *band_dev = ms->used_tps ? b.tot : b.ens;
    if (r0) *r0 = b.r0;
    if (r1) *r1 = b.r1;
    if (full_dev) *full_dev = (ms->gathered && b.full) ? b.full + (size_t)ms->plan.lead * (size_t)ms->g.ncol : nullptr;
    return MHS_OK;
}

int mhs_mltps_grid_multi(const mhs_model *const *models, const double *weights, int n_models, double wt_total, const mhs_grid *g,
                         const mhs_stack *covars_host, const double *X, const double *resp, int64_t n, int64_t tile_edge,
                         double lambda, int gcv_mode, double slot0_share, double *final_host, mhs_mltps_info *info) {
    if (int rc = require_ready()) return rc;
    MHS_REQUIRE(g && covars_host && final_host, "NULL argument");
    double share = slot0_share;
    if (std::isnan(share)) {
        std::lock_guard<std::mutex> lk(g_balance_mu);
        if (g_balance.n == slot_count() && g_balance.nrow == g->nrow && g_balance.ncol == g->ncol && g_balance.stations == n) share = g_balance.share;
    }
    MHS_REQUIRE(covars_host->data && g->nrow > 0 && g->ncol > 0, "bad arguments");
    MHS_REQUIRE(covars_host->dtype == MHS_F64 || covars_host->dtype == MHS_F32 || covars_host->dtype == MHS_I16, "bad stack dtype");
    MHS_REQUIRE(covars_host->ld >= g->ncol && covars_host->plane_stride >= covars_host->ld * g->nrow, "stack strides smaller than the grid");
    std::lock_guard<std::mutex> lk(g_host_mu);
    const double t0 = now_ms();
    const BandPlan want = plan_bands(g->nrow, slot_count(), share);
    mhs_multi_stack *ms = g_host_ms;
    if (ms && !(stack_current(ms) && ms->g.nrow == g->nrow && ms->g.ncol == g->ncol && ms->C == covars_host->n_layers &&
                ms->dtype == covars_host->dtype && ms->plan.r0 == want.r0 && ms->plan.r1 == want.r1)) {
        free_stack(ms);
        ms = g_host_ms = nullptr;
    }
    if (!ms) {
        if (int rc = stack_build(g, covars_host, share, false, &ms)) return rc;
        g_host_ms = ms;
    }
    ms->g = *g; ms->nodata = covars_host->nodata; ms->have_result = false;
    ms->pending = covars_host;
    ms->pending_out = final_host;
    ms->downloaded = false;
    const double t1 = now_ms();
    int rc = mhs_mltps_grid_multi_dev(models, weights, n_models, wt_total, ms, X, resp, n, tile_edge, lambda, gcv_mode, 0, info);
    ms->pending = nullptr; ms->pending_out = nullptr;
    const double t2 = now_ms();
    if (!rc && !ms->downloaded) rc = mhs_multi_final_download(ms, final_host);
    if (info && !rc) { info->upload_ms = (t1 - t0) + ms->upload_ms; info->download_ms = ms->downloaded ? ms->download_ms : now_ms() - t2; }
    return rc;
}

}

namespace {

struct UnitSlot {
    std::vector<char *> cov;
    double *ens = nullptr, *tps = nullptr;
    std::vector<double *> merge_in;
    double *merged = nullptr;
};

struct LayerBoard {
    std::mutex mu;
    std::condition_variable cv;
    std::vector<int64_t> done;
    bool stop = false;
    void finished(int l) { std::lock_guard<std::mutex> lk(mu); ++done[(size_t)l]; cv.notify_all(); }
    void abort() { std::lock_guard<std::mutex> lk(mu); stop = true; cv.notify_all(); }
    bool wait(int l, int64_t n_tiles) {
        std::unique_lock<std::mutex> lk(mu);
        cv.wait(lk, [&] { return stop || done[(size_t)l] >= n_tiles; });
        return !stop;
    }
};

}

extern "C" int mhs_tiles_units_multi(const mhs_grid *g, const mhs_stack *covars_host, int64_t out_ncol, int64_t out_nrow,
                                     double feather_d, int n_layers, const mhs_unit *units, int tps, int64_t tile_edge,
                                     double lambda, int gcv_mode, double *const *merged_host, double *rsq,
                                     mhs_units_info *info) {
    if (int rc = require_ready()) return rc;
    MHS_REQUIRE(g && covars_host && covars_host->data && units && merged_host, "NULL argument");
    MHS_REQUIRE(g->nrow > 0 && g->ncol > 0 && g->xres > 0 && g->yres > 0, "bad grid geometry");
    MHS_REQUIRE(out_ncol >= 1 && out_nrow >= 1 && out_ncol * out_nrow <= 4096 && n_layers >= 1, "bad tile layout");
    MHS_REQUIRE(covars_host->dtype == MHS_F64 || covars_host->dtype == MHS_F32 || covars_host->dtype == MHS_I16, "bad stack dtype");
    MHS_REQUIRE(covars_host->ld >= g->ncol && covars_host->plane_stride >= covars_host->ld * g->nrow, "stack strides smaller than the grid");
    const int N = slot_count();
    const int64_t n_tiles = out_ncol * out_nrow, n_units = n_tiles * n_layers;
    const int C = covars_host->n_layers, p = C + 2;
    const size_t esz = elem_size(covars_host->dtype);
    std::vector<double> boxes((size_t)n_tiles * 4);
    std::vector<int64_t> win((size_t)n_tiles * 4);
    if (int rc = mhs_tiles_create_windows(g, out_ncol, out_nrow, feather_d, boxes.data(), win.data())) return rc;
    int64_t max_cells = 0;
    for (int64_t t = 0; t < n_tiles; ++t) max_cells = std::max(max_cells, (win[4 * t + 1] - win[4 * t]) * (win[4 * t + 3] - win[4 * t + 2]));
    for (int64_t u = 0; u < n_units; ++u) {
        const mhs_unit &U = units[u];
        MHS_REQUIRE(U.models && U.weights && U.n_models >= 1 && U.n_models <= 8 && U.X && U.resp && U.n > 3, "bad unit");
        MHS_REQUIRE(U.wt_total != 0.0 && !std::isnan(U.wt_total), "a unit's wt_total must be non-zero");
    }
    std::lock_guard<std::mutex> arena_lk(g_host_mu);
    const double t_start = now_ms();
    std::vector<double *> plane((size_t)n_units, nullptr);
    std::vector<double> rsq_model((size_t)n_units, NAN), rsq_final((size_t)n_units, NAN), unit_ms((size_t)n_units, 0.0);
    std::vector<UnitSlot> us((size_t)N);
    LayerBoard board;
    board.done.assign((size_t)n_layers, 0);
    Team team(N);
    const int rc = team.run([&](int slot) {
        UnitSlot &L = us[(size_t)slot];
        MultiSlot *M = nullptr;
        TEAM_DO(team, multi_slot(slot, &M));
        auto alloc = [&]() -> int {
            auto cells_of = [&](int64_t t) { return (size_t)((win[4 * t + 1] - win[4 * t]) * (win[4 * t + 3] - win[4 * t + 2])); };
            auto up = [](size_t bytes) { return (bytes + 255) & ~(size_t)255; };
            std::vector<char> mine((size_t)n_tiles, 0);
            size_t need = 2 * up(sizeof(double) * (size_t)max_cells);
            for (int64_t u = slot; u < n_units; u += N) { mine[(size_t)(u % n_tiles)] = 1; need += up(sizeof(double) * cells_of(u % n_tiles)); }
            for (int64_t t = 0; t < n_tiles; ++t) if (mine[(size_t)t]) need += up(cells_of(t) * esz * (size_t)C);
            bool merges = false;
            for (int l = slot; l < n_layers; l += N) merges = merges || merged_host[l] != nullptr;
            if (merges) {
                for (int64_t t = 0; t < n_tiles; ++t) need += up(sizeof(double) * cells_of(t));
                need += up(sizeof(double) * (size_t)g->nrow * (size_t)g->ncol);
            }
            UnitsArena &A = g_units_arena[slot];
            if (need > A.cap) {
                if (A.base) { MHS_HIP(hipDeviceSynchronize()); MHS_HIP(hipFree(A.base)); A.base = nullptr; A.cap = 0; }
                MHS_HIP(hipMalloc((void **)&A.base, need));
                A.cap = need;
            }
            char *q = A.base;
            auto take = [&](size_t bytes) { char *r = q; q += up(bytes); return r; };
            L.ens = (double *)take(sizeof(double) * (size_t)max_cells);
            L.tps = (double *)take(sizeof(double) * (size_t)max_cells);
            L.cov.assign((size_t)n_tiles, nullptr);
            for (int64_t t = 0; t < n_tiles; ++t) if (mine[(size_t)t]) L.cov[(size_t)t] = take(cells_of(t) * esz * (size_t)C);
            for (int64_t u = slot; u < n_units; u += N)
                plane[(size_t)u] = (double *)take(sizeof(double) * cells_of(u % n_tiles));
            if (merges) {
                L.merge_in.assign((size_t)n_tiles, nullptr);
                for (int64_t t = 0; t < n_tiles; ++t) L.merge_in[(size_t)t] = (double *)take(sizeof(double) * cells_of(t));
                L.merged = (double *)take(sizeof(double) * (size_t)g->nrow * (size_t)g->ncol);
            }
            return MHS_OK;
        };
        TEAM_DO(team, alloc());
        TEAM_DO(team, mhs_tps_reduction_cache(1));
        std::vector<int64_t> order;
        std::vector<int> pos((size_t)n_tiles, -1);
        for (int64_t u = slot; u < n_units; u += N)
            if (pos[(size_t)(u % n_tiles)] < 0) { pos[(size_t)(u % n_tiles)] = (int)order.size(); order.push_back(u % n_tiles); }
        std::vector<hipEvent_t> tev(order.size(), nullptr);
        Uploader pre;
        if (!order.empty() && !team.failed())
            pre.start(slot, (int)order.size(), [&](int q) -> int {
                const int64_t t = order[(size_t)q];
                const int64_t *w = &win[(size_t)t * 4];
                const int64_t nr = w[1] - w[0], nc = w[3] - w[2];
                for (int k = 0; k < C; ++k) {
                    const char *src = (const char *)covars_host->data + ((size_t)k * covars_host->plane_stride + (size_t)w[0] * covars_host->ld + (size_t)w[2]) * esz;
                    MHS_HIP(hipMemcpy2DAsync(L.cov[(size_t)t] + (size_t)k * (size_t)nr * (size_t)nc * esz, (size_t)nc * esz, src, (size_t)covars_host->ld * esz,
                                             (size_t)nc * esz, (size_t)nr, hipMemcpyHostToDevice, M->h));
                }
                MHS_HIP(hipEventCreateWithFlags(&tev[(size_t)q], hipEventDisableTiming));
                MHS_HIP(hipEventRecord(tev[(size_t)q], M->h));
                return MHS_OK;
            });
        std::vector<char> ready((size_t)n_tiles, 0);
        std::thread merger;
        {
            bool any = false;
            for (int l = slot; l < n_layers; l += N) any = any || merged_host[l] != nullptr;
            if (any && !team.failed()) merger = std::thread([&, slot] {
                SlotBind bind(slot);
                set_mosaic_lane(1);
                if (const int rcr = ring_prepare(slot)) { team.fail(rcr); board.abort(); return; }
                HostSink sink(slot, M->u);
                for (int l = slot; l < n_layers; l += N) {
                    if (!merged_host[l]) continue;
                    if (!board.wait(l, n_tiles)) return;
                    auto merge = [&]() -> int {
                        std::vector<const double *> ptrs((size_t)n_tiles);
                        for (int64_t t = 0; t < n_tiles; ++t) {
                            const int64_t u = (int64_t)l * n_tiles + t;
                            const int owner = (int)(u % N);
                            const size_t bytes = sizeof(double) * (size_t)((win[4 * t + 1] - win[4 * t]) * (win[4 * t + 3] - win[4 * t + 2]));
                            if (owner == slot) { ptrs[(size_t)t] = plane[(size_t)u]; continue; }
                            MHS_HIP(hipMemcpyPeerAsync(L.merge_in[(size_t)t], ctx_slot(slot).device, plane[(size_t)u], ctx_slot(owner).device, bytes, M->u));
                            ptrs[(size_t)t] = L.merge_in[(size_t)t];
                        }
                        if (int rc2 = mhs_mosaic_feather_dev(g, out_nrow, out_ncol, win.data(), ptrs.data(), 1, L.merged, g->ncol, nullptr, M->u)) return rc2;
                        return sink.download(merged_host[l], L.merged, sizeof(double) * (size_t)g->nrow * (size_t)g->ncol);
                    };
                    const int rcm = merge();
                    if (rcm) { team.fail(rcm); board.abort(); (void)hipStreamSynchronize(M->u); return; }
                }
            });
        }
        for (int64_t u = slot; u < n_units && !team.failed(); u += N) {
            const int64_t t = u % n_tiles;
            const mhs_unit &U = units[u];
            const int64_t *w = &win[(size_t)t * 4];
            const int64_t nr = w[1] - w[0], nc = w[3] - w[2];
            auto run = [&]() -> int {
                const double t0 = now_ms();
                mhs_grid gt = {g->xmin + (double)w[2] * g->xres, g->ymax - (double)w[0] * g->yres, g->xres, g->yres, nr, nc};
                if (!ready[(size_t)t]) {
                    if (int rc2 = pre.wait(pos[(size_t)t])) return rc2;
                    MHS_HIP(hipStreamWaitEvent(M->s, tev[(size_t)pos[(size_t)t]], 0));
                    ready[(size_t)t] = 1;
                }
                std::vector<const mhs_model *> my((size_t)U.n_models);
                int p0 = 0;
                for (int k = 0; k < U.n_models; ++k) {
                    MHS_REQUIRE(U.models[k] != nullptr, "NULL model in a unit");
                    if (int rc2 = mhs_model_info(U.models[k], nullptr, &p0, nullptr)) return rc2;
                    MHS_REQUIRE(p0 == p, "a unit's model does not match the stack (layers + 2 predictors)");
                    if (int rc2 = model_on_slot(U.models[k], slot, &my[(size_t)k])) return rc2;
                }
                if (int rc2 = ensemble_band_dev(my.data(), U.weights, U.n_models, U.wt_total, &gt, L.cov[(size_t)t], C, covars_host->dtype, nc,
                                                covars_host->nodata, 0, nr, L.ens, nc, M->s)) return rc2;
                std::vector<double> res((size_t)U.n);
                if (int rc2 = mhs_residual_points(my.data(), U.weights, U.n_models, U.wt_total, U.X, U.resp, U.n, res.data())) return rc2;
                long double msum = 0.0L, tss_l = 0.0L, rs = 0.0L;
                for (int64_t i = 0; i < U.n; ++i) msum += U.resp[i];
                const double mean = (double)(msum / (long double)U.n);
                for (int64_t i = 0; i < U.n; ++i) { tss_l += (long double)((U.resp[i] - mean) * (U.resp[i] - mean)); rs += (long double)(res[(size_t)i] * res[(size_t)i]); }
                const double tss = (double)tss_l;
                rsq_model[(size_t)u] = 1.0 - (double)rs / tss;
                const double *fin = L.ens;
                if (tps) {
                    const double *knots = U.X + (size_t)(p - 2) * (size_t)U.n;
                    if (int rc2 = mhs_tps_surface_dev(&gt, knots, res.data(), U.n, U.X, tile_edge, lambda, gcv_mode, L.tps, nc, nullptr, M->s)) return rc2;
                    if (int rc2 = mhs_scale_add_dev(L.ens, 1.0, L.tps, L.tps, nr * nc, M->s)) return rc2;
                    std::vector<int64_t> rows((size_t)U.n), cols((size_t)U.n);
                    if (int rc2 = mhs_cells_from_xy(&gt, knots, U.n, rows.data(), cols.data())) return rc2;
                    std::vector<double> f((size_t)U.n);
                    if (int rc2 = mhs_gather_cells_dev(L.tps, nc, rows.data(), cols.data(), U.n, f.data(), M->s)) return rc2;
                    rs = 0.0L;
                    for (int64_t i = 0; i < U.n; ++i) { const double e = U.resp[i] - f[(size_t)i]; rs += (long double)(e * e); }
                    rsq_final[(size_t)u] = 1.0 - (double)rs / tss;
                    if (rsq_final[(size_t)u] > rsq_model[(size_t)u]) fin = L.tps;
                }
                MHS_HIP(hipMemcpyAsync(plane[(size_t)u], fin, sizeof(double) * (size_t)nr * (size_t)nc, hipMemcpyDeviceToDevice, M->s));
                MHS_HIP(hipStreamSynchronize(M->s));
                unit_ms[(size_t)u] = now_ms() - t0;
                return MHS_OK;
            };
            TEAM_DO(team, run());
            if (team.failed()) board.abort(); else board.finished((int)(u / n_tiles));
        }
        if (team.failed()) board.abort();
        if (ctx().ready) (void)mhs_tps_reduction_cache(0);
        pre.join();
        if (M && M->h) (void)hipStreamSynchronize(M->h);
        for (hipEvent_t e : tev) if (e) (void)hipEventDestroy(e);
        if (merger.joinable()) merger.join();
        team.bar.wait();
        if (M) (void)hipStreamSynchronize(M->s);
    });
    if (rc) return rc;
    if (rsq) for (int64_t u = 0; u < n_units; ++u) { rsq[2 * u] = rsq_model[(size_t)u]; rsq[2 * u + 1] = rsq_final[(size_t)u]; }
    if (info) {
        memset(info, 0, sizeof(*info));
        info->n_slots = N; info->n_units = n_units; info->step_ms = now_ms() - t_start;
        for (int64_t u = 0; u < n_units; ++u) {
            info->unit_ms_sum += unit_ms[(size_t)u];
            info->unit_ms_max = std::max(info->unit_ms_max, unit_ms[(size_t)u]);
            info->slot_ms[u % N] += unit_ms[(size_t)u];
        }
    }
    return MHS_OK;
}
```

machisplin_amd/csrc/tps_eval.hip:

```cpp
#include <algorithm>
#include <cmath>
#include <cstdlib>
#include <cstring>
#include <vector>
#include "common.h"
#include "devmath.h"
#include "tps_batch.h"

namespace mhs {

constexpr int EVAL_ROWS = 4;
constexpr int EVAL_WAVES = 4;
constexpr int EVAL_TILE_ROWS = EVAL_ROWS * EVAL_WAVES;

struct EvalGeom {
    double xmin, ymax, xres, yres;
    double cx, cy, sx, sy;
    double d0, d1, d2;
    int64_t r0, c0;
    int nr, nc;
    int64_t ld;
};

__device__ __forceinline__ void tps_accumulate(const Knot *__restrict__ knots, const int j0, const int j1,
                                               const double u, const double (&v)[EVAL_ROWS],
                                               double (&acc)[EVAL_ROWS], const double2 *tab) {
#pragma unroll 2
    for (int j = j0; j < j1; ++j) {
        const Knot kn = knots[j];
        const double dx = u - kn.u;
        const double dx2 = dx * dx;
#pragma unroll
        for (int k = 0; k < EVAL_ROWS; ++k) {
            const double dy = v[k] - kn.v;
            const double dd = fma(dy, dy, dx2);
            acc[k] = fma(kn.cw, r2logr2(dd, tab), acc[k]);
        }
    }
}

__device__ __forceinline__ void eval_direct_block(const Knot *__restrict__ knots, int n, const double2 *tab, const EvalGeom &g,
                                                  double *__restrict__ out, int bx, int by) {
    const int lane = threadIdx.x & 63;
    const int wave = threadIdx.x >> 6;
    const int col = bx * 64 + lane;
    const int row0 = by * EVAL_TILE_ROWS + wave * EVAL_ROWS;
    if (row0 >= g.nr) return;

    const double x = g.xmin + ((double)(g.c0 + col) + 0.5) * g.xres;
    const double u = (x - g.cx) / g.sx;
    double v[EVAL_ROWS], acc[EVAL_ROWS];
#pragma unroll
    for (int k = 0; k < EVAL_ROWS; ++k) {
        const double y = g.ymax - ((double)(g.r0 + row0 + k) + 0.5) * g.yres;
        v[k] = (y - g.cy) / g.sy;
        acc[k] = 0.0;
    }

    tps_accumulate(knots, 0, n, u, v, acc, tab);

    if (col < g.nc) {
#pragma unroll
        for (int k = 0; k < EVAL_ROWS; ++k)
            if (row0 + k < g.nr)
                out[(int64_t)(row0 + k) * g.ld + col] = g.d0 + g.d1 * u + g.d2 * v[k] + acc[k];
    }
}

__global__ __launch_bounds__(64 * EVAL_WAVES) void tps_eval_grid_kernel(
    const Knot *__restrict__ knots, int n, const double2 *__restrict__ gtab, EvalGeom g,
    double *__restrict__ out) {
    __shared__ double2 tab[LOG_TAB_N];
    stage_log_table(tab, gtab);
    eval_direct_block(knots, n, tab, g, out, blockIdx.x, blockIdx.y);
}

__global__ __launch_bounds__(256) void tps_eval_points_kernel(
    const Knot *__restrict__ knots, int n, const double2 *__restrict__ gtab, EvalGeom g,
    const double *__restrict__ px, const double *__restrict__ py, int64_t npts,
    double *__restrict__ out) {
    __shared__ double2 tab[LOG_TAB_N];
    stage_log_table(tab, gtab);
    const int64_t i = (int64_t)blockIdx.x * 256 + threadIdx.x;
    const int64_t ii = i < npts ? i : npts - 1;
    const double u = (px[ii] - g.cx) / g.sx;
    const double v = (py[ii] - g.cy) / g.sy;
    double acc = 0.0;
    for (int j = 0; j < n; ++j) {
        const Knot kn = knots[j];
        const double dx = u - kn.u, dy = v - kn.v;
        const double dd = fma(dy, dy, dx * dx);
        acc = fma(kn.cw, r2logr2(dd, tab), acc);
    }
    if (i < npts) out[i] = g.d0 + g.d1 * u + g.d2 * v + acc;
}

constexpr int FF_N = 16;
constexpr int FF_NODES = FF_N * FF_N;
constexpr int FF_PAD = 2;

struct FarGeom {
    int tx, ty, ntx, nty;
    double t[FF_N];
    int row_lo, row_hi, ty_lo, ty_hi;
};

__device__ __forceinline__ void ff_nodes_block(const Knot *__restrict__ knots, int n, const int *__restrict__ bin_start,
                                               const double2 *tab, const EvalGeom &g, const FarGeom &f,
                                               double *__restrict__ nodes, int blk) {
    const int lane = threadIdx.x & 63;
    const int tile = f.ty_lo * f.ntx + blk * 4 + (threadIdx.x >> 6);
    if (tile >= f.ty_hi * f.ntx) return;
    const int tyi = tile / f.ntx, txi = tile - tyi * f.ntx;
    const int a = lane & 15, bg = lane >> 4;
    const double hx = 0.5 * (double)f.tx * g.xres, hy = 0.5 * (double)f.ty * g.yres;
    const double xc = g.xmin + (double)(g.c0 + (int64_t)txi * f.tx) * g.xres + hx;
    const double yc = g.ymax - (double)(g.r0 + (int64_t)tyi * f.ty) * g.yres - hy;
    const double u = (xc + hx * f.t[a] - g.cx) / g.sx;
    double v[EVAL_ROWS], acc[EVAL_ROWS];
#pragma unroll
    for (int k = 0; k < EVAL_ROWS; ++k) {
        v[k] = (yc + hy * f.t[bg * EVAL_ROWS + k] - g.cy) / g.sy;
        acc[k] = 0.0;
    }
    const int nbx = f.ntx + 2 * FF_PAD;
    int j = 0;
#pragma unroll 1
    for (int r = 0; r < 3; ++r) {
        const int *row = bin_start + (int64_t)(tyi + FF_PAD - 1 + r) * nbx + (txi + FF_PAD - 1);
        const int s0 = row[0], e0 = row[3];
        tps_accumulate(knots, j, s0, u, v, acc, tab);
        j = e0;
    }
    tps_accumulate(knots, j, n, u, v, acc, tab);
#pragma unroll
    for (int k = 0; k < EVAL_ROWS; ++k)
        nodes[(int64_t)tile * FF_NODES + (bg * EVAL_ROWS + k) * FF_N + a] = g.d0 + g.d1 * u + g.d2 * v[k] + acc[k];
}

__global__ __launch_bounds__(256) void tps_ff_nodes_kernel(const Knot *__restrict__ knots, int n,
                                                           const int *__restrict__ bin_start,
                                                           const double2 *__restrict__ gtab, EvalGeom g,
                                                           FarGeom f, double *__restrict__ nodes) {
    __shared__ double2 tab[LOG_TAB_N];
    stage_log_table(tab, gtab);
    ff_nodes_block(knots, n, bin_start, tab, g, f, nodes, blockIdx.x);
}

struct FfCellsShared {
    double2 tab[LOG_TAB_N];
    double sF[FF_NODES];
    double sG[FF_N][64];
};
__device__ __forceinline__ void ff_cells_block(const Knot *__restrict__ knots, const int *__restrict__ bin_start,
                                               const double2 *__restrict__ gtab, const EvalGeom &g, const FarGeom &f,
                                               const double *__restrict__ nodes, const double *__restrict__ lx,
                                               const double *__restrict__ ly, double *__restrict__ out, FfCellsShared &sh,
                                               int bx, int by_in) {
    const int lane = threadIdx.x & 63;
    const int wave = threadIdx.x >> 6;
    const int cchunks = f.tx / 64, rchunks = f.ty / EVAL_TILE_ROWS;
    const int txi = bx / cchunks, cc = bx - txi * cchunks;
    const int by = by_in + f.ty_lo * rchunks;
    const int tyi = by / rchunks, rc = by - tyi * rchunks;
    const int tile = tyi * f.ntx + txi;
    const int lcol = cc * 64 + lane;
    const int lrow0 = rc * EVAL_TILE_ROWS + wave * EVAL_ROWS;
    const int col = txi * f.tx + lcol;
    const int row0 = tyi * f.ty + lrow0;
    if (tyi * f.ty + rc * EVAL_TILE_ROWS >= f.row_hi || tyi * f.ty + (rc + 1) * EVAL_TILE_ROWS <= f.row_lo ||
        txi * f.tx + cc * 64 >= g.nc) return;
    for (int i = threadIdx.x; i < LOG_TAB_N; i += 64 * EVAL_WAVES) sh.tab[i] = gtab[i];
    sh.sF[threadIdx.x] = nodes[(int64_t)tile * FF_NODES + threadIdx.x];
    __syncthreads();
    {
        double lxr[FF_N];
#pragma unroll
        for (int a = 0; a < FF_N; ++a) lxr[a] = lx[(int64_t)lcol * FF_N + a];
#pragma unroll
        for (int k = 0; k < EVAL_ROWS; ++k) {
            const int b = wave * EVAL_ROWS + k;
            double s = 0.0;
#pragma unroll
            for (int a = 0; a < FF_N; ++a) s = fma(sh.sF[b * FF_N + a], lxr[a], s);
            sh.sG[b][lane] = s;
        }
    }
    __syncthreads();
    const double x = g.xmin + ((double)(g.c0 + col) + 0.5) * g.xres;
    const double u = (x - g.cx) / g.sx;
    double v[EVAL_ROWS], acc[EVAL_ROWS];
#pragma unroll
    for (int k = 0; k < EVAL_ROWS; ++k) {
        const double y = g.ymax - ((double)(g.r0 + row0 + k) + 0.5) * g.yres;
        v[k] = (y - g.cy) / g.sy;
        const double *lyr = ly + (int64_t)(lrow0 + k) * FF_N;
        double s = 0.0;
#pragma unroll
        for (int b = 0; b < FF_N; ++b) s = fma(lyr[b], sh.sG[b][lane], s);
        acc[k] = s;
    }
    const int nbx = f.ntx + 2 * FF_PAD;
#pragma unroll 1
    for (int r = 0; r < 3; ++r) {
        const int *brow = bin_start + (int64_t)(tyi + FF_PAD - 1 + r) * nbx + (txi + FF_PAD - 1);
        tps_accumulate(knots, brow[0], brow[3], u, v, acc, sh.tab);
    }
    if (col < g.nc) {
#pragma unroll
        for (int k = 0; k < EVAL_ROWS; ++k)
            if (row0 + k >= f.row_lo && row0 + k < f.row_hi) out[(int64_t)(row0 + k - f.row_lo) * g.ld + col] = acc[k];
    }
}

__global__ __launch_bounds__(64 * EVAL_WAVES) void tps_ff_cells_kernel(
    const Knot *__restrict__ knots, const int *__restrict__ bin_start, const double2 *__restrict__ gtab,
    EvalGeom g, FarGeom f, const double *__restrict__ nodes, const double *__restrict__ lx,
    const double *__restrict__ ly, double *__restrict__ out) {
    __shared__ FfCellsShared sh;
    ff_cells_block(knots, bin_start, gtab, g, f, nodes, lx, ly, out, sh, blockIdx.x, blockIdx.y);
}

struct EvalWindow {
    EvalGeom g;
    FarGeom f;
    const Knot *knots;
    const int *bin_start;
    double *nodes;
    const double *lx, *ly;
    double *out;
    const double *d3;
    int n, far;
    int node_blocks;
    int cgx, cgy;
};
__global__ __launch_bounds__(256) void tps_batch_nodes_kernel(const EvalWindow *__restrict__ W, const double2 *__restrict__ gtab) {
    __shared__ double2 tab[LOG_TAB_N];
    const EvalWindow &D = W[blockIdx.y];
    if (!D.far || (int)blockIdx.x >= D.node_blocks) return;
    stage_log_table(tab, gtab);
    EvalGeom g = D.g;
    g.d0 = D.d3[0]; g.d1 = D.d3[1]; g.d2 = D.d3[2];
    ff_nodes_block(D.knots, D.n, D.bin_start, tab, g, D.f, D.nodes, blockIdx.x);
}
__global__ __launch_bounds__(64 * EVAL_WAVES) void tps_batch_cells_kernel(const EvalWindow *__restrict__ W, const double2 *__restrict__ gtab) {
    __shared__ FfCellsShared sh;
    const EvalWindow &D = W[blockIdx.y];
    if ((int)blockIdx.x >= D.cgx * D.cgy) return;
    const int by = blockIdx.x / D.cgx, bx = blockIdx.x - by * D.cgx;
    if (D.far) {
        ff_cells_block(D.knots, D.bin_start, gtab, D.g, D.f, D.nodes, D.lx, D.ly, D.out, sh, bx, by);
    } else {
        stage_log_table(sh.tab, gtab);
        EvalGeom g = D.g;
        g.d0 = D.d3[0]; g.d1 = D.d3[1]; g.d2 = D.d3[2];
        eval_direct_block(D.knots, D.n, sh.tab, g, D.out, bx, by);
    }
}

int upload_knots(mhs_tps *t) {
    std::vector<Knot> h((size_t)t->n);
    const double k = 0.5 / (8.0 * M_PI);
    for (int64_t j = 0; j < t->n; ++j) {
        h[j].u = t->knots_uv[j];
        h[j].v = t->knots_uv[t->n + j];
        h[j].cw = t->c[j] * k;
        h[j].pad = 0.0;
    }
    t->far.r0 = -1;
    if (t->knots_dev) { (void)hipDeviceSynchronize(); pool_release(t->knots_dev); t->knots_dev = nullptr; }
    t->knots_dev = (Knot *)pool_alloc(sizeof(Knot) * (size_t)(t->n ? t->n : 1));
    if (!t->knots_dev) return MHS_ERR_ALLOC;
    return h2d_sync(t->knots_dev, h.data(), sizeof(Knot) * (size_t)t->n);
}

static EvalGeom make_geom(const mhs_tps *t, const mhs_grid *g, int64_t r0, int64_t r1, int64_t c0,
                          int64_t c1, int64_t ld) {
    EvalGeom e;
    if (g) { e.xmin = g->xmin; e.ymax = g->ymax; e.xres = g->xres; e.yres = g->yres; }
    else { e.xmin = e.ymax = 0; e.xres = e.yres = 1; }
    e.cx = t->center[0]; e.cy = t->center[1]; e.sx = t->scale[0]; e.sy = t->scale[1];
    e.d0 = t->d[0]; e.d1 = t->d[1]; e.d2 = t->d[2];
    e.r0 = r0; e.c0 = c0; e.nr = (int)(r1 - r0); e.nc = (int)(c1 - c0); e.ld = ld;
    return e;
}

static int g_eval_mode = 0;

template <typename T>
static int grow(T **p, size_t *cap, size_t need) {
    if (*cap >= need && *p) return MHS_OK;
    if (*p) { (void)hipDeviceSynchronize(); pool_release(*p); *p = nullptr; *cap = 0; }
    *p = (T *)pool_alloc((need ? need : 1) * sizeof(T));
    if (!*p) return MHS_ERR_ALLOC;
    *cap = need;
    return MHS_OK;
}

static void cheb_matrix(int cells, bool flip, const double (&t)[FF_N], std::vector<double> &L) {
    double w[FF_N];
    for (int a = 0; a < FF_N; ++a) w[a] = ((a & 1) ? -1.0 : 1.0) * sin((2 * a + 1) * M_PI / (2.0 * FF_N));
    L.assign((size_t)cells * FF_N, 0.0);
    for (int i = 0; i < cells; ++i) {
        double tau = (2.0 * i + 1.0) / (double)cells - 1.0;
        if (flip) tau = -tau;
        int hit = -1;
        double q[FF_N], sum = 0.0;
        for (int a = 0; a < FF_N; ++a) {
            const double d = tau - t[a];
            if (d == 0.0) { hit = a; break; }
            q[a] = w[a] / d;
            sum += q[a];
        }
        for (int a = 0; a < FF_N; ++a) L[(size_t)i * FF_N + a] = hit >= 0 ? (a == hit ? 1.0 : 0.0) : q[a] / sum;
    }
}

static void far_plan_choose(const double *knots_uv, int64_t N, const EvalGeom &e, FarGeom *f, bool *use,
                            std::vector<double> &kc, std::vector<double> &kr) {
    *use = false;
    if (g_eval_mode == 1 || e.nc < 64 || e.nr < 16 || N < 32) return;
    kc.resize((size_t)N); kr.resize((size_t)N);
    int64_t inside = 0;
    for (int64_t j = 0; j < N; ++j) {
        const double x = knots_uv[j] * e.sx + e.cx, y = knots_uv[N + j] * e.sy + e.cy;
        kc[j] = (x - e.xmin) / e.xres - (double)e.c0;
        kr[j] = (e.ymax - y) / e.yres - (double)e.r0;
        if (kc[j] >= 0 && kc[j] < e.nc && kr[j] >= 0 && kr[j] < e.nr) ++inside;
    }
    const double cells = (double)e.nr * (double)e.nc;
    const double rho = (double)(inside > 0 ? inside : 1) / cells;
    const double aspect = (e.xres / e.sx) / (e.yres / e.sy);
    double best = 1e300;
    int btx = 0, bty = 0;
    for (int tx = 64; tx <= 1024; tx += 64) {
        int ty = (int)llround((double)tx * aspect / 16.0) * 16;
        if (ty < 16) ty = 16;
        if (ty > 4096) continue;
        const double ntx = ceil((double)e.nc / tx), nty = ceil((double)e.nr / ty);
        const double cost = ntx * nty * FF_NODES * (double)N / cells + 9.0 * rho * tx * ty + 4.0;
        if (cost < best) { best = cost; btx = tx; bty = ty; }
    }
    if (btx == 0) return;
    if (g_eval_mode != 2 && best > 0.5 * (double)N) return;
    const double tile_aspect = ((double)btx * e.xres / e.sx) / ((double)bty * e.yres / e.sy);
    if (tile_aspect > 1.25 || tile_aspect < 0.8) return;
    f->tx = btx; f->ty = bty;
    f->ntx = (int)((e.nc + btx - 1) / btx); f->nty = (int)((e.nr + bty - 1) / bty);
    for (int a = 0; a < FF_N; ++a) f->t[a] = cos((2 * a + 1) * M_PI / (2.0 * FF_N));
    f->row_lo = 0; f->row_hi = e.nr; f->ty_lo = 0; f->ty_hi = f->nty;
    *use = true;
}
static void far_plan_sort(int64_t N, const EvalGeom &e, const FarGeom &f, const std::vector<double> &kc,
                          const std::vector<double> &kr, std::vector<int> &start, std::vector<int> &order,
                          int64_t *node_pairs, int64_t *cell_pairs) {
    const int btx = f.tx, bty = f.ty;
    const int nbx = f.ntx + 2 * FF_PAD, nby = f.nty + 2 * FF_PAD;
    std::vector<int> bin((size_t)N);
    start.assign((size_t)nbx * nby + 1, 0);
    for (int64_t j = 0; j < N; ++j) {
        double bx = floor(kc[j] / btx), by = floor(kr[j] / bty);
        bx = std::min(std::max(bx, (double)-FF_PAD), (double)(f.ntx + FF_PAD - 1));
        by = std::min(std::max(by, (double)-FF_PAD), (double)(f.nty + FF_PAD - 1));
        bin[j] = ((int)by + FF_PAD) * nbx + ((int)bx + FF_PAD);
        ++start[(size_t)bin[j] + 1];
    }
    for (size_t b = 0; b + 1 < start.size(); ++b) start[b + 1] += start[b];
    std::vector<int> fill(start.begin(), start.end() - 1);
    order.resize((size_t)N);
    for (int64_t j = 0; j < N; ++j) order[(size_t)fill[(size_t)bin[j]]++] = (int)j;
    int64_t np = 0, cp = 0;
    for (int tyi = 0; tyi < f.nty; ++tyi)
        for (int txi = 0; txi < f.ntx; ++txi) {
            int64_t near = 0;
            for (int r = 0; r < 3; ++r) {
                const size_t b = (size_t)(tyi + FF_PAD - 1 + r) * nbx + (size_t)(txi + FF_PAD - 1);
                near += start[b + 3] - start[b];
            }
            const int64_t tc = std::min<int64_t>(btx, e.nc - (int64_t)txi * btx) * std::min<int64_t>(bty, e.nr - (int64_t)tyi * bty);
            np += (int64_t)FF_NODES * (N - near);
            cp += tc * near;
        }
    if (node_pairs) *node_pairs = np;
    if (cell_pairs) *cell_pairs = cp;
}

static int plan_far(mhs_tps *t, const mhs_grid *g, const EvalGeom &e, int64_t r1, int64_t c1, FarGeom *f, bool *use) {
    const int64_t N = t->n;
    std::vector<double> kc, kr;
    far_plan_choose(t->knots_uv.data(), N, e, f, use, kc, kr);
    if (!*use) return MHS_OK;
    const int btx = f->tx, bty = f->ty;
    mhs_tps::FarPlan &P = t->far;
    const bool same = P.sorted_dev && P.xmin == e.xmin && P.ymax == e.ymax && P.xres == e.xres && P.yres == e.yres &&
                      P.r0 == e.r0 && P.r1 == r1 && P.c0 == e.c0 && P.c1 == c1 && P.tx == btx && P.ty == bty;
    if (same) return MHS_OK;
    if (P.in_flight) { MHS_HIP(hipStreamSynchronize(P.last_stream)); P.in_flight = false; }
    std::vector<int> start, order;
    far_plan_sort(N, e, *f, kc, kr, start, order, &P.node_pairs, &P.cell_pairs);
    std::vector<Knot> sorted((size_t)N);
    const double kk = 0.5 / (8.0 * M_PI);
    for (int64_t p = 0; p < N; ++p) {
        const int j = order[(size_t)p];
        Knot &k = sorted[(size_t)p];
        k.u = t->knots_uv[j]; k.v = t->knots_uv[N + j]; k.cw = t->c[j] * kk; k.pad = 0.0;
    }
    std::vector<double> lx, ly;
    cheb_matrix(btx, false, f->t, lx);
    cheb_matrix(bty, true, f->t, ly);
    if (!P.sorted_dev) { P.sorted_dev = (Knot *)pool_alloc(sizeof(Knot) * (size_t)N); if (!P.sorted_dev) return MHS_ERR_ALLOC; }
    if (int rc = grow(&P.bin_start_dev, &P.bins_cap, start.size())) return rc;
    if (int rc = grow(&P.nodes_dev, &P.nodes_cap, (size_t)f->ntx * f->nty * FF_NODES)) return rc;
    if (int rc = grow(&P.lx_dev, &P.lx_cap, lx.size())) return rc;
    if (int rc = grow(&P.ly_dev, &P.ly_cap, ly.size())) return rc;
    if (int rc = h2d_sync(P.sorted_dev, sorted.data(), sizeof(Knot) * (size_t)N)) return rc;
    if (int rc = h2d_sync(P.bin_start_dev, start.data(), sizeof(int) * start.size())) return rc;
    if (int rc = h2d_sync(P.lx_dev, lx.data(), sizeof(double) * lx.size())) return rc;
    if (int rc = h2d_sync(P.ly_dev, ly.data(), sizeof(double) * ly.size())) return rc;
    P.xmin = e.xmin; P.ymax = e.ymax; P.xres = e.xres; P.yres = e.yres;
    P.r0 = e.r0; P.r1 = r1; P.c0 = e.c0; P.c1 = c1; P.tx = btx; P.ty = bty; P.ntx = f->ntx; P.nty = f->nty;
    return MHS_OK;
}

struct EvalBatch {
    struct Item {
        EvalWindow w;
        int64_t knot_off = 0;
        int res_index = 0;
        size_t bins_off = 0, nodes_off = 0;
        int lxy = -1;
    };
    struct Mats { int tx, ty; std::vector<double> lx, ly; size_t lx_off = 0, ly_off = 0; };
    std::vector<Item> items;
    std::vector<EvalWindow> wh;
    std::vector<int> bins;
    std::vector<Mats> mats;
    size_t nodes_total = 0;
    unsigned max_node_blocks = 0, max_cell_blocks = 0;
};
EvalBatch *eval_batch_create() { return new EvalBatch(); }
void eval_batch_destroy(EvalBatch *B) { delete B; }

struct EvalPlan { EvalBatch::Item it; std::vector<int> start; bool far = false; };
static int eval_plan_one(const double *knots_uv, int n, const double *center, const double *scale, const mhs_grid *grid,
                         int64_t r0, int64_t r1, int64_t c0, int64_t c1, double *out_dev, int64_t ld, EvalPlan &P, std::vector<int> &perm) {
    MHS_REQUIRE(r1 - r0 < (1LL << 30) && c1 - c0 < (1LL << 30) && r1 > r0 && c1 > c0, "window too large or empty");
    EvalBatch::Item &it = P.it;
    memset(&it.w, 0, sizeof(it.w));
    EvalGeom &e = it.w.g;
    e.xmin = grid->xmin; e.ymax = grid->ymax; e.xres = grid->xres; e.yres = grid->yres;
    e.cx = center[0]; e.cy = center[1]; e.sx = scale[0]; e.sy = scale[1];
    e.d0 = e.d1 = e.d2 = 0.0;
    e.r0 = r0; e.c0 = c0; e.nr = (int)(r1 - r0); e.nc = (int)(c1 - c0); e.ld = ld;
    it.w.out = out_dev; it.w.n = n;
    std::vector<double> kc, kr;
    far_plan_choose(knots_uv, n, e, &it.w.f, &P.far, kc, kr);
    perm.resize((size_t)n);
    if (P.far) {
        std::vector<int> order;
        far_plan_sort(n, e, it.w.f, kc, kr, P.start, order, nullptr, nullptr);
        for (int p = 0; p < n; ++p) perm[(size_t)order[(size_t)p]] = p;
        it.w.far = 1;
        it.w.node_blocks = (it.w.f.ntx * it.w.f.nty + 3) / 4;
        it.w.cgx = it.w.f.ntx * (it.w.f.tx / 64);
        it.w.cgy = it.w.f.nty * (it.w.f.ty / EVAL_TILE_ROWS);
    } else {
        for (int p = 0; p < n; ++p) perm[(size_t)p] = p;
        it.w.far = 0; it.w.node_blocks = 0;
        it.w.cgx = (e.nc + 63) / 64;
        it.w.cgy = (e.nr + EVAL_TILE_ROWS - 1) / EVAL_TILE_ROWS;
    }
    return MHS_OK;
}
static void eval_plan_commit(EvalBatch *B, EvalPlan &P, int res_index, int64_t knot_off) {
    EvalBatch::Item &it = P.it;
    it.knot_off = knot_off; it.res_index = res_index;
    if (P.far) {
        it.bins_off = B->bins.size();
        B->bins.insert(B->bins.end(), P.start.begin(), P.start.end());
        it.nodes_off = B->nodes_total;
        B->nodes_total += (size_t)it.w.f.ntx * it.w.f.nty * FF_NODES;
        it.lxy = -1;
        for (size_t q = 0; q < B->mats.size(); ++q)
            if (B->mats[q].tx == it.w.f.tx && B->mats[q].ty == it.w.f.ty) it.lxy = (int)q;
        if (it.lxy < 0) {
            EvalBatch::Mats m;
            m.tx = it.w.f.tx; m.ty = it.w.f.ty;
            cheb_matrix(m.tx, false, it.w.f.t, m.lx);
            cheb_matrix(m.ty, true, it.w.f.t, m.ly);
            it.lxy = (int)B->mats.size();
            B->mats.push_back(std::move(m));
        }
    }
    B->max_node_blocks = std::max(B->max_node_blocks, (unsigned)it.w.node_blocks);
    B->max_cell_blocks = std::max(B->max_cell_blocks, (unsigned)(it.w.cgx * it.w.cgy));
    B->items.push_back(it);
}
int eval_batch_add(EvalBatch *B, const double *knots_uv, int n, const double *center, const double *scale, const mhs_grid *grid,
                   int64_t r0, int64_t r1, int64_t c0, int64_t c1, double *out_dev, int64_t ld, int res_index, int64_t knot_off,
                   std::vector<int> &perm) {
    EvalPlan P;
    if (int rc = eval_plan_one(knots_uv, n, center, scale, grid, r0, r1, c0, c1, out_dev, ld, P, perm)) return rc;
    eval_plan_commit(B, P, res_index, knot_off);
    return MHS_OK;
}
EvalPlanHandle *eval_batch_plan(const double *knots_uv, int n, const double *center, const double *scale, const mhs_grid *grid,
                                int64_t r0, int64_t r1, int64_t c0, int64_t c1, double *out_dev, int64_t ld, std::vector<int> &perm, int *rc_out) {
    EvalPlan *P = new EvalPlan();
    const int rc = eval_plan_one(knots_uv, n, center, scale, grid, r0, r1, c0, c1, out_dev, ld, *P, perm);
    if (rc_out) *rc_out = rc;
    if (rc) { delete P; return nullptr; }
    return reinterpret_cast<EvalPlanHandle *>(P);
}
void eval_batch_commit(EvalBatch *B, EvalPlanHandle *h, int res_index, int64_t knot_off) {
    EvalPlan *P = reinterpret_cast<EvalPlan *>(h);
    eval_plan_commit(B, *P, res_index, knot_off);
    delete P;
}
void eval_plan_drop(EvalPlanHandle *h) { delete reinterpret_cast<EvalPlan *>(h); }

static size_t eb_up(size_t x) { return (x + 255) & ~(size_t)255; }
size_t eval_batch_device_bytes(const EvalBatch *B) {
    size_t off = 0;
    off = eb_up(off + sizeof(EvalWindow) * B->items.size());
    off = eb_up(off + sizeof(int) * B->bins.size());
    for (const EvalBatch::Mats &m : B->mats) off = eb_up(off + sizeof(double) * (m.lx.size() + m.ly.size()));
    off = eb_up(off + sizeof(double) * B->nodes_total);
    return off;
}

int eval_batch_launch(EvalBatch *B, char *dev, const Knot *knots_base, const SmallResult *res_base, hipStream_t s) {
    if (B->items.empty()) return MHS_OK;
    size_t off = 0;
    EvalWindow *wdev = (EvalWindow *)(dev + off); off = eb_up(off + sizeof(EvalWindow) * B->items.size());
    int *bins_dev = (int *)(dev + off); off = eb_up(off + sizeof(int) * B->bins.size());
    std::vector<double *> lxd, lyd;
    for (EvalBatch::Mats &m : B->mats) {
        double *p = (double *)(dev + off);
        off = eb_up(off + sizeof(double) * (m.lx.size() + m.ly.size()));
        lxd.push_back(p); lyd.push_back(p + m.lx.size());
        MHS_HIP(hipMemcpyAsync(p, m.lx.data(), sizeof(double) * m.lx.size(), hipMemcpyHostToDevice, s));
        MHS_HIP(hipMemcpyAsync(p + m.lx.size(), m.ly.data(), sizeof(double) * m.ly.size(), hipMemcpyHostToDevice, s));
    }
    double *nodes_dev = (double *)(dev + off);
    std::vector<EvalWindow> &w = B->wh;
    w.resize(B->items.size());
    for (size_t k = 0; k < B->items.size(); ++k) {
        const EvalBatch::Item &it = B->items[k];
        w[k] = it.w;
        w[k].knots = knots_base + it.knot_off;
        w[k].d3 = res_base[it.res_index].d;
        if (it.w.far) {
            w[k].bin_start = bins_dev + it.bins_off;
            w[k].nodes = nodes_dev + it.nodes_off;
            w[k].lx = lxd[(size_t)it.lxy]; w[k].ly = lyd[(size_t)it.lxy];
        }
    }
    MHS_HIP(hipMemcpyAsync(wdev, w.data(), sizeof(EvalWindow) * w.size(), hipMemcpyHostToDevice, s));
    if (!B->bins.empty()) MHS_HIP(hipMemcpyAsync(bins_dev, B->bins.data(), sizeof(int) * B->bins.size(), hipMemcpyHostToDevice, s));
    const unsigned nt = (unsigned)B->items.size();
    MHS_REQUIRE(nt <= 65535u, "too many windows for one launch");
    if (B->max_node_blocks > 0)
        hipLaunchKernelGGL(tps_batch_nodes_kernel, dim3(B->max_node_blocks, nt), dim3(256), 0, s, wdev, ctx().log_tab);
    hipLaunchKernelGGL(tps_batch_cells_kernel, dim3(B->max_cell_blocks, nt), dim3(64 * EVAL_WAVES), 0, s, wdev, ctx().log_tab);
    MHS_HIP(hipGetLastError());
    return MHS_OK;
}

}

using namespace mhs;

extern "C" {

int mhs_tps_from_coef(const double *knots_uv, const double *c, const double *d3, int64_t n,
                      double lambda, const double *center2, const double *scale2, mhs_tps **out) {
    if (int rc = require_ready()) return rc;
    MHS_REQUIRE(knots_uv && c && d3 && center2 && scale2 && out, "NULL argument");
    MHS_REQUIRE(n >= 1 && n < (1LL << 31), "n out of range");
    MHS_REQUIRE(scale2[0] > 0 && scale2[1] > 0, "scale must be positive");
    mhs_tps *t = new mhs_tps();
    t->n = n;
    t->lambda = lambda;
    t->eff_df = t->gcv = NAN;
    t->c.assign(c, c + n);
    t->knots_uv.assign(knots_uv, knots_uv + 2 * n);
    memcpy(t->d, d3, sizeof(t->d));
    memcpy(t->center, center2, sizeof(t->center));
    memcpy(t->scale, scale2, sizeof(t->scale));
    if (int rc = upload_knots(t)) { mhs_tps_free(t); return rc; }
    *out = t;
    return MHS_OK;
}

int mhs_tps_size(const mhs_tps *t, int64_t *n) {
    MHS_REQUIRE(t && n, "NULL argument");
    *n = t->n;
    return MHS_OK;
}

int mhs_tps_get(const mhs_tps *t, double *c, double *d3, double *knots_uv, double *lambda,
                double *center2, double *scale2, double *eff_df, double *gcv) {
    MHS_REQUIRE(t != nullptr, "NULL handle");
    if (c) memcpy(c, t->c.data(), sizeof(double) * (size_t)t->n);
    if (d3) memcpy(d3, t->d, sizeof(t->d));
    if (knots_uv) memcpy(knots_uv, t->knots_uv.data(), sizeof(double) * 2 * (size_t)t->n);
    if (lambda) *lambda = t->lambda;
    if (center2) memcpy(center2, t->center, sizeof(t->center));
    if (scale2) memcpy(scale2, t->scale, sizeof(t->scale));
    if (eff_df) *eff_df = t->eff_df;
    if (gcv) *gcv = t->gcv;
    return MHS_OK;
}

}
int mhs::tps_free_quiet(mhs_tps *t) {
    if (!t) return MHS_OK;
    for (void *q : {(void *)t->knots_dev, (void *)t->far.sorted_dev, (void *)t->far.bin_start_dev, (void *)t->far.nodes_dev,
                    (void *)t->far.lx_dev, (void *)t->far.ly_dev}) pool_release(q);
    se_state_free(t->se);
    delete t;
    return MHS_OK;
}
extern "C" {

int mhs_tps_free(mhs_tps *t) {
    if (!t) return MHS_OK;
    if ((t->knots_dev || t->se) && ctx().ready) (void)hipDeviceSynchronize();
    return tps_free_quiet(t);
}

int mhs_tps_eval_mode(int mode) {
    MHS_REQUIRE(mode >= 0 && mode <= 2, "mode must be 0 (auto), 1 (direct) or 2 (far-field-interpolated)");
    g_eval_mode = mode;
    return MHS_OK;
}

int mhs_tps_eval_plan(const mhs_tps *t, int *tile_cols, int *tile_rows, int64_t *node_pairs, int64_t *cell_pairs) {
    MHS_REQUIRE(t != nullptr, "NULL handle");
    const mhs_tps::FarPlan &P = t->far;
    if (tile_cols) *tile_cols = P.last_used ? P.tx : 0;
    if (tile_rows) *tile_rows = P.last_used ? P.ty : 0;
    if (node_pairs) *node_pairs = P.last_used ? P.node_pairs : 0;
    if (cell_pairs) *cell_pairs = P.last_used ? P.cell_pairs : 0;
    return MHS_OK;
}

int mhs_tps_predict_grid_dev(const mhs_tps *t, const mhs_grid *g, int64_t r0, int64_t r1,
                             int64_t c0, int64_t c1, double *out_dev, int64_t ld, void *stream) {
    return tps_predict_rows_dev(t, g, r0, r1, c0, c1, r0, r1, out_dev, ld, stream);
}

int mhs_tps_predict_rows_dev(const mhs_tps *t, const mhs_grid *g, int64_t r0, int64_t r1, int64_t c0, int64_t c1,
                             int64_t b0, int64_t b1, double *out_dev, int64_t ld, void *stream) {
    return tps_predict_rows_dev(t, g, r0, r1, c0, c1, b0, b1, out_dev, ld, stream);
}

}

int mhs::tps_predict_rows_dev(const mhs_tps *t, const mhs_grid *g, int64_t r0, int64_t r1, int64_t c0, int64_t c1,
                              int64_t b0, int64_t b1, double *out_dev, int64_t ld, void *stream) {
    if (int rc = require_ready()) return rc;
    MHS_REQUIRE(t && g && out_dev, "NULL argument");
    MHS_REQUIRE(g->nrow > 0 && g->ncol > 0 && g->xres > 0 && g->yres > 0, "bad grid geometry");
    MHS_REQUIRE(0 <= r0 && r0 <= r1 && r1 <= g->nrow && 0 <= c0 && c0 <= c1 && c1 <= g->ncol,
                "window outside the grid");
    MHS_REQUIRE(r0 <= b0 && b0 <= b1 && b1 <= r1, "row band outside the window");
    MHS_REQUIRE(ld >= c1 - c0, "ld smaller than the window width");
    MHS_REQUIRE(r1 - r0 < (1LL << 30) && c1 - c0 < (1LL << 30), "window too large");
    if (b1 == b0 || c1 == c0) return MHS_OK;
    const EvalGeom e = make_geom(t, g, r0, r1, c0, c1, ld);
    FarGeom f;
    bool far = false;
    mhs_tps *tm = const_cast<mhs_tps *>(t);
    std::lock_guard<std::mutex> lk(tm->mu);
    if (int rc = plan_far(tm, g, e, r1, c1, &f, &far)) return rc;
    tm->far.last_used = far;
    if (far) {
        mhs_tps::FarPlan &Pm = tm->far;
        if (Pm.in_flight && Pm.last_stream != pick_stream(stream)) MHS_HIP(hipStreamSynchronize(Pm.last_stream));
        Pm.last_stream = pick_stream(stream);
        Pm.in_flight = true;
        const mhs_tps::FarPlan &P = t->far;
        f.row_lo = (int)(b0 - r0); f.row_hi = (int)(b1 - r0);
        f.ty_lo = f.row_lo / f.ty; f.ty_hi = (f.row_hi + f.ty - 1) / f.ty;
        const int ntiles = f.ntx * (f.ty_hi - f.ty_lo);
        dim3 cgrid((unsigned)(f.ntx * (f.tx / 64)), (unsigned)((f.ty_hi - f.ty_lo) * (f.ty / EVAL_TILE_ROWS)));
        MHS_REQUIRE(cgrid.y <= 65535u, "too many rows for one launch");
        hipLaunchKernelGGL(tps_ff_nodes_kernel, dim3((unsigned)((ntiles + 3) / 4)), dim3(256), 0, pick_stream(stream),
                           P.sorted_dev, (int)t->n, P.bin_start_dev, ctx().log_tab, e, f, P.nodes_dev);
        hipLaunchKernelGGL(tps_ff_cells_kernel, cgrid, dim3(64 * EVAL_WAVES), 0, pick_stream(stream), P.sorted_dev,
                           P.bin_start_dev, ctx().log_tab, e, f, P.nodes_dev, P.lx_dev, P.ly_dev, out_dev);
        MHS_HIP(hipGetLastError());
        return MHS_OK;
    }
    const EvalGeom eb = make_geom(t, g, b0, b1, c0, c1, ld);
    dim3 grid((unsigned)((eb.nc + 63) / 64), (unsigned)((eb.nr + EVAL_TILE_ROWS - 1) / EVAL_TILE_ROWS));
    MHS_REQUIRE(grid.y <= 65535u, "too many rows for one launch");
    hipLaunchKernelGGL(tps_eval_grid_kernel, grid, dim3(64 * EVAL_WAVES), 0, pick_stream(stream),
                       t->knots_dev, (int)t->n, ctx().log_tab, eb, out_dev);
    MHS_HIP(hipGetLastError());
    return MHS_OK;
}

extern "C" {

int mhs_tps_predict_grid(const mhs_tps *t, const mhs_grid *g, int64_t r0, int64_t r1, int64_t c0,
                         int64_t c1, double *out_host) {
    if (int rc = require_ready()) return rc;
    MHS_REQUIRE(t && g && out_host, "NULL argument");
    MHS_REQUIRE(0 <= r0 && r0 <= r1 && 0 <= c0 && c0 <= c1, "bad window");
    const int64_t nr = r1 - r0, nc = c1 - c0;
    if (nr == 0 || nc == 0) return MHS_OK;
    std::lock_guard<std::mutex> lk(pipe_mutex());
    if (int rc = host_pipe(sizeof(double) * (size_t)(nr * nc))) return rc;
    double *buf = (double *)ctx().pipe_arena;
    hipStream_t s = ctx().pipe_comp;
    if (int rc = mhs_tps_predict_grid_dev(t, g, r0, r1, c0, c1, buf, nc, s)) return rc;
    MHS_HIP(hipMemcpyAsync(out_host, buf, sizeof(double) * (size_t)(nr * nc), hipMemcpyDeviceToHost, s));
    MHS_HIP(hipStreamSynchronize(s));
    return MHS_OK;
}

int mhs_tps_predict_points(const mhs_tps *t, const double *xy, int64_t n, double *out_host) {
    if (int rc = require_ready()) return rc;
    MHS_REQUIRE(t && out_host && (xy || n == 0), "NULL argument");
    MHS_REQUIRE(n >= 0, "negative n");
    if (n == 0) return MHS_OK;
    DevBuf<double> dxy, dout;
    MHS_HIP(dxy.alloc((size_t)(2 * n)));
    MHS_HIP(dout.alloc((size_t)n));
    hipStream_t s = ctx().stream;
    MHS_HIP(hipMemcpyAsync(dxy.p, xy, sizeof(double) * 2 * (size_t)n, hipMemcpyHostToDevice, s));
    const EvalGeom e = make_geom(t, nullptr, 0, 0, 0, 0, 0);
    hipLaunchKernelGGL(tps_eval_points_kernel, dim3((unsigned)((n + 255) / 256)), dim3(256), 0, s,
                       t->knots_dev, (int)t->n, ctx().log_tab, e, dxy.p, dxy.p + n, n, dout.p);
    MHS_HIP(hipGetLastError());
    MHS_HIP(hipMemcpyAsync(out_host, dout.p, sizeof(double) * (size_t)n, hipMemcpyDeviceToHost, s));
    MHS_HIP(hipStreamSynchronize(s));
    return MHS_OK;
}

}
```

machisplin_amd/sharded.py:

```python
from __future__ import annotations

import contextlib
import os

import numpy as np

FIT_RESERVE_CANDIDATES = (0, 32, 64, 96)


BAND_ALIGN = 16


def row_bands(nrow: int, world: int, rank0_share: float | None = None):
    if world == 1:
        return nrow, [(0, nrow)]
    even = -(-nrow // world)
    align = BAND_ALIGN if even >= BAND_ALIGN else 1
    up = lambda n: -(-n // align) * align
    if rank0_share is None:
        band = up(even)
        return band, [(min(r * band, nrow), min((r + 1) * band, nrow)) for r in range(world)]
    n0 = min(nrow, int(round(min(max(rank0_share, 0.0), 1.0) * nrow / align)) * align)
    rest, others = nrow - n0, world - 1
    h = up(-(-rest // others))
    if n0 > h:
        n0 = h = up(-(-nrow // world))
        return h, [(min(r * h, nrow), min((r + 1) * h, nrow)) for r in range(world)]
    bands = [(0, n0)] + [(min(n0 + k * h, nrow), min(n0 + (k + 1) * h, nrow)) for k in range(others)]
    return max(h, n0), bands


def balanced_rank0_share(world: int, cells_ms: float, fit_ms: float) -> float:
    if world <= 1:
        return 1.0
    s0 = 1.0 / world - fit_ms * (world - 1) / (world * max(cells_ms, 1e-9))
    return min(max(s0, 0.0), 1.0 / world)


def tps_msg_len(n_stations: int) -> int:
    return 3 * int(n_stations) + 9


def pack_tps(knots, c, d, center, scale, lambda_, n_stations: int | None = None):
    knots = np.asarray(knots, dtype=np.float64)
    n = knots.shape[0]
    msg = np.concatenate([[float(n)], knots[:, 0], knots[:, 1], np.asarray(c, dtype=np.float64),
                          np.asarray(d, dtype=np.float64), np.asarray(center, dtype=np.float64),
                          np.asarray(scale, dtype=np.float64), [float(lambda_)]])
    if n_stations is not None:
        if n > n_stations:
            raise ValueError("fit has more knots than station rows")
        msg = np.concatenate([msg, np.zeros(tps_msg_len(n_stations) - msg.size)])
    return msg


def unpack_tps(buf):
    buf = np.asarray(buf, dtype=np.float64)
    n = int(buf[0])
    b = buf[1:]
    return {"knots": np.column_stack([b[:n], b[n:2 * n]]), "c": b[2 * n:3 * n], "d": b[3 * n:3 * n + 3],
            "center": b[3 * n + 3:3 * n + 5], "scale": b[3 * n + 5:3 * n + 7], "lambda": float(b[3 * n + 7]), "n": n}


class ShardedMltps:

    def __init__(self, ops, dist, rank: int, world: int, nrow: int, ncol: int, rank0_share: float | None = None):
        import torch
        self.ops, self.dist, self.rank, self.world = ops, dist, rank, world
        self.nrow, self.ncol = nrow, ncol
        self.band, self.bands = row_bands(nrow, world, rank0_share)
        self.r0, self.r1 = self.bands[rank]
        self.lead = self.band - (self.bands[0][1] - self.bands[0][0]) if world > 1 else 0
        kw = {"dtype": torch.float64, "device": ops.device}
        self.full = torch.zeros((self.band * world, ncol), **kw) if world > 1 else None
        self.pred = torch.zeros((self.band, ncol), **kw)
        self.tot = torch.zeros((self.band, ncol), **kw)
        self.torch = torch
        self.fit_reserve_cus = int(os.environ.get("MHS_FIT_RESERVE_CUS", 0))
        self.reservation_calibration = None

    def calibrate_reservation(self, candidates=FIT_RESERVE_CANDIDATES, repeats: int = 2):
        import time
        torch = self.torch
        if "MHS_FIT_RESERVE_CUS" in os.environ or not hasattr(self.ops, "reserve"):
            return None
        timings = {}
        for cus in candidates:
            self.fit_reserve_cus = cus
            best = float("inf")
            for _ in range(repeats):
                if self.world > 1:
                    self.dist.barrier()
                torch.cuda.synchronize()
                t0 = time.perf_counter()
                self.step()
                torch.cuda.synchronize()
                best = min(best, (time.perf_counter() - t0) * 1e3)
            timings[cus] = best
        if self.rank == 0:
            self.fit_reserve_cus = min(timings, key=lambda c: (timings[c], c))
        else:
            self.fit_reserve_cus = 0
        self.reservation_calibration = {"step_ms_by_reserved_units": timings, "chosen": self.fit_reserve_cus}
        return timings

    def step(self):
        side = getattr(self.ops, "side_stream", None) or contextlib.nullcontext
        with side():
            out = self._step()
        join = getattr(self.ops, "join_side_stream", None)
        if join:
            join()
        return out

    def _step(self):
        ops, torch = self.ops, self.torch
        nb = self.r1 - self.r0
        off = self.lead if self.rank == 0 else 0
        reserve = getattr(ops, "reserve", None) if (self.rank == 0 and self.fit_reserve_cus > 0 and nb > 0) else None
        prev = reserve(self.fit_reserve_cus) if reserve else None
        try:
            if nb > 0:
                ops.ensemble_band(self.r0, self.r1, self.pred[off:off + nb])
            knots, resid, resp, rows, cols = ops.station_residuals()
            n = knots.shape[0]
            msg = torch.zeros(tps_msg_len(n), dtype=torch.float64, device=ops.device)
            if self.rank == 0:
                packed0 = np.ascontiguousarray(ops.tps_fit(knots, resid))
                msg[:packed0.size].copy_(torch.from_numpy(packed0))
        finally:
            if prev is not None:
                reserve(prev)
        if self.world > 1:
            self.dist.broadcast(msg, src=0)
        packed = msg.cpu().numpy()
        rows, cols = np.asarray(rows), np.asarray(cols)
        band_pred, band_tot = self.pred[off:off + nb], self.tot[off:off + nb]
        f_actual = np.zeros(n)
        if nb > 0:
            ops.tps_band(packed, self.r0, self.r1, band_tot)
            ops.add(band_pred, band_tot, band_tot)
            mine = (rows >= self.r0) & (rows < self.r1)
            if mine.any():
                f_actual[mine] = ops.gather(band_tot, rows[mine] - self.r0, cols[mine])
        if self.world > 1:
            t = torch.from_numpy(f_actual).to(ops.device)
            self.dist.all_reduce(t)
            f_actual = t.cpu().numpy()
        f_actual[(rows < 0) | (cols < 0)] = np.nan
        tss = float(np.sum((resp - resp.mean()) ** 2))
        rsq_model = 1.0 - float(np.sum(resid ** 2)) / tss
        rsq_final = 1.0 - float(np.sum((resp - f_actual) ** 2)) / tss
        src = self.tot if rsq_final > rsq_model else self.pred
        if self.world > 1:
            self.dist.all_gather_into_tensor(self.full, src)
            final = self.full[self.lead:self.lead + self.nrow]
        else:
            final = src[:self.nrow]
        return {"final": final, "rsq_model": rsq_model, "rsq_final": rsq_final, "lambda": unpack_tps(packed)["lambda"]}


def assign_tiles(costs, world: int):
    order = sorted(range(len(costs)), key=lambda h: (-float(costs[h]), h))
    load, owner = [0.0] * world, [0] * len(costs)
    for h in order:
        r = min(range(world), key=lambda k: (load[k], k))
        owner[h] = r
        load[r] += float(costs[h])
    return owner


class TiledTpsShardedMltps:

    def __init__(self, ops, dist, rank: int, world: int, nrow: int, ncol: int, tile_edge: int = 1500):
        import torch
        self.ops, self.dist, self.rank, self.world = ops, dist, rank, world
        self.nrow, self.ncol = nrow, ncol
        self.band, self.bands = row_bands(nrow, world)
        self.r0, self.r1 = self.bands[rank]
        self.layout = ops.tps_tiles(tile_edge)
        keep = [tuple(int(v) for v in w) for w in self.layout["keep"]]
        self.keep = keep
        self.cells = [(w[1] - w[0]) * (w[3] - w[2]) for w in keep]
        self.owner = assign_tiles(self.layout["cost"], world)
        self.offset, fill = [0] * len(keep), [0] * world
        for h in range(len(keep)):
            self.offset[h] = fill[self.owner[h]]
            fill[self.owner[h]] += self.cells[h]
        self.band_len = self.band * ncol
        self.chunk = self.band_len + max(fill + [1])
        kw = {"dtype": torch.float64, "device": ops.device}
        self.full = torch.zeros(world * self.chunk, **kw)
        self.mine = self.full[:self.chunk] if world == 1 else torch.zeros(self.chunk, **kw)
        self.total = torch.zeros((nrow, ncol), **kw)
        self.pred_full = None
        self.torch = torch
        self.fit_reserve_cus = int(os.environ.get("MHS_TILED_FIT_RESERVE_CUS", 0))

    def _tile_view(self, buf, base, h):
        r0, r1, c0, c1 = self.keep[h]
        o = base + self.band_len + self.offset[h]
        return buf[o:o + self.cells[h]].view(r1 - r0, c1 - c0)

    def step(self):
        side = getattr(self.ops, "side_stream", None) or contextlib.nullcontext
        with side():
            out = self._step()
        join = getattr(self.ops, "join_side_stream", None)
        if join:
            join()
        return out

    def _step(self):
        ops = self.ops
        nb = self.r1 - self.r0
        reserve = getattr(ops, "reserve", None) if (self.fit_reserve_cus > 0 and nb > 0) else None
        prev = reserve(self.fit_reserve_cus) if reserve else None
        try:
            if nb > 0:
                ops.ensemble_band(self.r0, self.r1, self.mine[:nb * self.ncol].view(nb, self.ncol))
            knots, resid, resp, rows, cols = ops.station_residuals()
            mine = [h for h in range(len(self.keep)) if self.owner[h] == self.rank]
            if hasattr(ops, "tps_tiles_batch"):
                ops.tps_tiles_batch(mine, knots, resid, [self._tile_view(self.mine, 0, h) for h in mine])
            else:
                for h in mine:
                    ops.tps_tile(h, knots, resid, self._tile_view(self.mine, 0, h))
        finally:
            if prev is not None:
                reserve(prev)
        if self.world > 1:
            self.dist.all_gather_into_tensor(self.full, self.mine)
        tiles = [self._tile_view(self.full, self.owner[h] * self.chunk, h) for h in range(len(self.keep))]
        ops.tps_mosaic(self.layout["nRx"], self.layout["nCx"], self.keep, tiles, self.total)
        bands = []
        for r, (a, b) in enumerate(self.bands):
            if b > a:
                pb = self.full[r * self.chunk:r * self.chunk + (b - a) * self.ncol].view(b - a, self.ncol)
                bands.append((a, b, pb))
        f_tps = ops.gather(self.total, rows, cols)
        for a, b, pb in bands:
            ops.add(pb, self.total[a:b], self.total[a:b])
        f_actual = ops.gather(self.total, rows, cols)
        tss = float(np.sum((resp - resp.mean()) ** 2))
        rsq_model = 1.0 - float(np.sum(resid ** 2)) / tss
        rsq_final = 1.0 - float(np.sum((resp - f_actual) ** 2)) / tss
        if rsq_final > rsq_model:
            final = self.total
        else:
            if self.pred_full is None:
                self.pred_full = self.torch.zeros_like(self.total)
            for a, b, pb in bands:
                self.pred_full[a:b].copy_(pb)
            final = self.pred_full
        return {"final": final, "rsq_model": rsq_model, "rsq_final": rsq_final, "tps_at_stations": f_tps,
                "tile_owner": list(self.owner)}


class HipOps:

    def __init__(self, stack, int_xy, resp, models, weights, wt_total, lambda_=None, gcv_mode="fields",
                 timed: bool = False, keep=None):
        import torch
        from . import _lib, mltps
        self.torch, self._lib = torch, _lib
        self.stack, self.models, self.weights, self.wt_total = stack, models, list(weights), float(wt_total)
        self.lambda_, self.gcv_mode = lambda_, gcv_mode
        self.device = stack.planes.device
        X, rows, cols = mltps.station_predictors(stack, int_xy)
        y = np.asarray(resp, dtype=np.float64)
        own = ~np.isnan(X).any(axis=1) & ~np.isnan(y)
        keep = own if keep is None else (np.asarray(keep, dtype=bool) & own)
        self.X, self.rows, self.cols, self.y = X[keep], rows[keep], cols[keep], y[keep]
        self.n_stations = int(self.X.shape[0])
        self.timed = timed
        self.timings = {"ensemble_ms": [], "tps_eval_ms": [], "tps_fit_ms": [], "residuals_ms": []}
        self.last_fit = None
        self._pending = []

    def _timed(self, key, fn):
        if not self.timed:
            return fn()
        e0 = self.torch.cuda.Event(enable_timing=True)
        e1 = self.torch.cuda.Event(enable_timing=True)
        e0.record()
        r = fn()
        e1.record()
        self._pending.append((key, e0, e1))
        return r

    def collect(self):
        for key, e0, e1 in self._pending:
            self.timings.setdefault(key, []).append(e0.elapsed_time(e1))
        self._pending = []

    def reserve(self, n_cus):
        from . import _lib
        from .models import fit_reserve_cus
        if getattr(self, "_no_cu_mask", False):
            return None
        try:
            return fit_reserve_cus(n_cus)
        except _lib.MhsError:
            self._no_cu_mask = True
            return None

    @contextlib.contextmanager
    def side_stream(self):
        torch = self.torch
        if getattr(self, "_side", None) is None:
            self._side = torch.cuda.Stream(self.device)
        self._side.wait_stream(torch.cuda.current_stream(self.device))
        with torch.cuda.stream(self._side):
            yield

    def join_side_stream(self):
        if getattr(self, "_side", None) is not None:
            self.torch.cuda.current_stream(self.device).wait_stream(self._side)

    def ensemble_band(self, r0, r1, out):
        from .models import ensemble_predict
        g = self.stack.geom
        self._timed("ensemble_ms", lambda: ensemble_predict(self.stack, self.models, self.weights, self.wt_total,
                                                            window=(r0, r1, 0, g.ncol), out=out))

    def station_residuals(self):
        import time
        from .mltps import ensemble_residuals
        t0 = time.perf_counter()
        res = ensemble_residuals(self.models, self.weights, self.wt_total, self.X, self.y)
        self.timings["residuals_ms"].append((time.perf_counter() - t0) * 1e3)
        return self.X[:, -2:], res, self.y, self.rows, self.cols

    def tps_fit(self, knots, resid):
        import time
        from .tps import Tps
        t0 = time.perf_counter()
        fit = Tps(knots, resid, lambda_=self.lambda_, gcv_mode=self.gcv_mode)
        self.timings["tps_fit_ms"].append((time.perf_counter() - t0) * 1e3)
        self.last_fit = fit
        return pack_tps(fit.knots, fit.c, fit.d, fit.center, fit.scale, fit.lambda_)

    def tps_band(self, packed, r0, r1, out):
        from .tps import Tps, interpolate
        d = unpack_tps(packed)
        fit = Tps.from_coef(d["knots"], d["c"], d["d"], d["lambda"], d["center"], d["scale"])
        g = self.stack.geom
        self._timed("tps_eval_ms", lambda: interpolate(g, fit, rows=(r0, r1), out=out))
        self.last_eval_plan = fit.eval_plan()

    def tps_tiles(self, tile_edge):
        from . import tiles
        g = self.stack.geom
        nRx, nCx, fit, keep = tiles.step3_tile_windows(g, tile_edge)
        ok = ~np.isnan(self.X[:, 0])
        self._tile_sel, cost = [], []
        for h in range(nRx * nCx):
            fr0, fr1, fc0, fc1 = (int(v) for v in fit[h])
            sel = np.flatnonzero(ok & (self.rows >= fr0) & (self.rows < fr1) & (self.cols >= fc0) & (self.cols < fc1))
            self._tile_sel.append(sel)
            kr0, kr1, kc0, kc1 = (int(v) for v in keep[h])
            cost.append(float(sel.size) * (kr1 - kr0) * (kc1 - kc0) + float(sel.size) ** 3)
        self._tile_fit, self._tile_keep, self._tile_edge = fit, keep, tile_edge
        return {"nRx": int(nRx), "nCx": int(nCx), "keep": [tuple(int(v) for v in w) for w in keep], "cost": cost}

    def tps_tile(self, h, knots, resid, out):
        from .tps import Tps, interpolate
        sel = self._tile_sel[h]
        if sel.size < 10:
            out.zero_()
            return
        fr0, fr1, fc0, fc1 = (int(v) for v in self._tile_fit[h])
        kr0, kr1, kc0, kc1 = (int(v) for v in self._tile_keep[h])
        fit = Tps(knots[sel], resid[sel], lambda_=self.lambda_, gcv_mode=self.gcv_mode)
        gf = self.stack.geom.window(fr0, fr1, fc0, fc1)
        interpolate(gf, fit, window=(kr0 - fr0, kr1 - fr0, kc0 - fc0, kc1 - fc0), out=out)

    def tps_tiles_batch(self, hs, knots, resid, outs):
        import ctypes as C
        import time
        if not hs:
            return
        t0 = time.perf_counter()
        g = self.stack.geom.c_struct()
        xyf = np.asfortranarray(np.asarray(knots, dtype=np.float64))
        res = np.ascontiguousarray(resid, dtype=np.float64)
        cov = np.ascontiguousarray(self.X[:, 0], dtype=np.float64)
        ids = np.ascontiguousarray(hs, dtype=np.int64)
        ptrs = (C.c_void_p * len(hs))(*[o.data_ptr() for o in outs])
        mode = {"fields": self._lib.GCV_FIELDS, "converged": self._lib.GCV_CONVERGED}[self.gcv_mode]
        self._lib.check(self._lib.lib().mhs_tps_tiles_dev(C.byref(g), xyf.ctypes.data, res.ctypes.data, res.shape[0], cov.ctypes.data,
                                                          int(self._tile_edge), float("nan") if self.lambda_ is None else float(self.lambda_),
                                                          mode, ids.ctypes.data, len(hs), ptrs))
        self.timings.setdefault("tps_tiles_ms", []).append((time.perf_counter() - t0) * 1e3)

    def tps_mosaic(self, nRx, nCx, keep, tiles_, out):
        from . import tiles
        tiles.mosaic_feather(self.stack.geom, nRx, nCx, np.asarray(keep, dtype=np.int64), list(tiles_), merge_mode=False, out=out)

    def add(self, a, b, out):
        st = self.torch.cuda.current_stream(self.device).cuda_stream
        assert a.is_contiguous() and b.is_contiguous() and out.is_contiguous()
        self._lib.check(self._lib.lib().mhs_scale_add_dev(a.data_ptr(), 1.0, b.data_ptr(), out.data_ptr(), a.numel(), st))

    def gather(self, plane, rows, cols):
        from . import tiles
        return tiles.extract(plane, rows, cols)


def unit_owner(tile: int, layer: int, n_tiles: int, world: int):
    u = layer * n_tiles + tile
    return u % world, u // world


class TileShardedMltps:

    def __init__(self, ops, dist, rank: int, world: int, merge_on: str = "owner"):
        import torch
        if merge_on not in ("owner", "all"):
            raise ValueError("merge_on must be 'owner' or 'all'")
        self.ops, self.dist, self.rank, self.world, self.merge_on = ops, dist, rank, world, merge_on
        self.shapes = [(int(h), int(w)) for h, w in ops.tile_shapes]
        self.n_tiles, self.n_layers = len(self.shapes), int(ops.n_layers)
        n_units = self.n_tiles * self.n_layers
        self.slots = -(-n_units // world)
        self.slot_len = max(h * w for h, w in self.shapes) + 2
        kw = {"dtype": torch.float64, "device": ops.device}
        self.full = torch.zeros((world * self.slots, self.slot_len), **kw)
        self.mine = self.full[rank * self.slots:(rank + 1) * self.slots] if world == 1 else \
            torch.zeros((self.slots, self.slot_len), **kw)
        self.torch = torch

    def my_units(self):
        return [(t, l) for l in range(self.n_layers) for t in range(self.n_tiles)
                if unit_owner(t, l, self.n_tiles, self.world)[0] == self.rank]

    def _plane(self, buf, slot, tile):
        h, w = self.shapes[tile]
        return buf[slot, :h * w].view(h, w)

    def step(self):
        torch = self.torch
        scope = getattr(self.ops, "reduction_cache", None) or contextlib.nullcontext
        with scope():
            for t, l in self.my_units():
                _, slot = unit_owner(t, l, self.n_tiles, self.world)
                rsq = self.ops.tile_layer(t, l, self._plane(self.mine, slot, t))
                self.mine[slot, -2:] = torch.tensor([float(rsq[0]), float(rsq[1])], dtype=torch.float64).to(self.mine.device)
        if self.world > 1:
            self.dist.all_gather_into_tensor(self.full, self.mine)
        stats = self.full[:, -2:].cpu().numpy()
        out = {"layers": {}, "rsq_model": np.full((self.n_layers, self.n_tiles), np.nan),
               "rsq_final": np.full((self.n_layers, self.n_tiles), np.nan)}
        for l in range(self.n_layers):
            rows = []
            for t in range(self.n_tiles):
                r, slot = unit_owner(t, l, self.n_tiles, self.world)
                rows.append(r * self.slots + slot)
                out["rsq_model"][l, t], out["rsq_final"][l, t] = stats[rows[-1]]
            if self.merge_on == "all" or l % self.world == self.rank:
                out["layers"][l] = self.ops.merge(l, [self._plane(self.full, rows[t], t) for t in range(self.n_tiles)])
        return out


class HipTileOps:

    def __init__(self, geom, tiles, stack_for_tile, int_values, fitted, tile_edge=1500, lambda_=None, gcv_mode="fields",
                 tps: bool = True):
        import torch
        from . import _lib
        self.torch = torch
        self.device = torch.device("cuda", _lib.init())
        self.geom, self.tiles, self.stack_for_tile = geom, tiles, stack_for_tile
        self.int_values = np.asarray(int_values, dtype=np.float64)
        self.fitted, self.tile_edge, self.lambda_, self.gcv_mode, self.tps = fitted, tile_edge, lambda_, gcv_mode, tps
        self.tile_shapes = [(int(w[1] - w[0]), int(w[3] - w[2])) for w in tiles["win"]]
        self.n_layers = self.int_values.shape[1] - 2
        self._stacks, self._keep = {}, {}
        self.unit_ms = {}

    def _stack(self, t):
        if t not in self._stacks:
            from .mltps import complete_cases
            self._stacks[t] = self.stack_for_tile(t)
            sel = self.tiles["dat"][t]
            self._keep[t] = complete_cases(self._stacks[t], self.int_values[sel])
        return self._stacks[t]

    def tile_layer(self, t, l, out):
        import time
        from .mltps import mltps_predict
        stack = self._stack(t)
        sel = self.tiles["dat"][t]
        f = self.fitted[t][l]
        t0 = time.perf_counter()
        res = mltps_predict(stack, self.int_values[sel, :2], self.int_values[sel, 2 + l], f["models"], f["weights"],
                            f["wt_total"], tps=self.tps, tile_edge=self.tile_edge, lambda_=self.lambda_,
                            gcv_mode=self.gcv_mode, keep=self._keep[t])
        out.copy_(res["final"])
        self.unit_ms[(t, l)] = (time.perf_counter() - t0) * 1e3
        return res["rsq_model"], res.get("rsq_final", float("nan"))

    def reduction_cache(self):
        from .tps import reduction_cache
        return reduction_cache()

    def merge(self, l, planes):
        from . import tiles as tl
        return tl.tiles_merge(self.geom, self.tiles["win"], [p.contiguous() for p in planes], in_ncol=self.tiles["nC"],
                              in_nrow=self.tiles["nR"])
```

machisplin_amd/tps.py:

```python
from __future__ import annotations

import contextlib
import ctypes as C
import math

import numpy as np

from . import _lib
from .raster import Geometry


class Tps:

    def __init__(self, x, Y, lambda_: float | None = None, gcv_mode: str = "fields"):
        x = np.ascontiguousarray(np.asarray(x, dtype=np.float64))
        if x.ndim != 2 or x.shape[1] != 2:
            raise ValueError("x must be an N x 2 matrix of (LONG, LAT)")
        y = np.ascontiguousarray(np.asarray(Y, dtype=np.float64).reshape(-1))
        if y.shape[0] != x.shape[0]:
            raise ValueError("x and Y have different numbers of rows")
        xy_cm = np.asfortranarray(x)
        mode = {"fields": _lib.GCV_FIELDS, "converged": _lib.GCV_CONVERGED}[gcv_mode]
        lam = math.nan if lambda_ is None else float(lambda_)
        h = C.c_void_p()
        _lib.check(_lib.lib().mhs_tps_fit(xy_cm.ctypes.data, y.ctypes.data, x.shape[0], lam, mode,
                                          C.byref(h)))
        self._h = h
        self._pull()

    @classmethod
    def from_coef(cls, knots_uv, c, d, lambda_, center, scale) -> "Tps":
        self = cls.__new__(cls)
        kn = np.asfortranarray(np.asarray(knots_uv, dtype=np.float64))
        c = np.ascontiguousarray(np.asarray(c, dtype=np.float64))
        d = np.ascontiguousarray(np.asarray(d, dtype=np.float64))
        ce = np.ascontiguousarray(np.asarray(center, dtype=np.float64))
        sc = np.ascontiguousarray(np.asarray(scale, dtype=np.float64))
        if kn.ndim != 2 or kn.shape[1] != 2 or c.shape != (kn.shape[0],) or d.shape != (3,):
            raise ValueError("knots must be n x 2, c length n, d length 3")
        h = C.c_void_p()
        _lib.check(_lib.lib().mhs_tps_from_coef(kn.ctypes.data, c.ctypes.data, d.ctypes.data,
                                                kn.shape[0], float(lambda_), ce.ctypes.data,
                                                sc.ctypes.data, C.byref(h)))
        self._h = h
        self._pull()
        return self

    def _pull(self):
        lib = _lib.lib()
        n = C.c_int64()
        _lib.check(lib.mhs_tps_size(self._h, C.byref(n)))
        n = n.value
        self.c = np.empty(n)
        self.d = np.empty(3)
        kn = np.empty((n, 2), order="F")
        lam, edf, gcv = C.c_double(), C.c_double(), C.c_double()
        self.center, self.scale = np.empty(2), np.empty(2)
        _lib.check(lib.mhs_tps_get(self._h, self.c.ctypes.data, self.d.ctypes.data, kn.ctypes.data,
                                   C.byref(lam), self.center.ctypes.data, self.scale.ctypes.data,
                                   C.byref(edf), C.byref(gcv)))
        self.knots = np.ascontiguousarray(kn)
        self.lambda_, self.eff_df, self.gcv = lam.value, edf.value, gcv.value
        self.n = n

    def predict(self, xy) -> np.ndarray:
        xy = np.asfortranarray(np.asarray(xy, dtype=np.float64).reshape(-1, 2))
        out = np.empty(xy.shape[0])
        _lib.check(_lib.lib().mhs_tps_predict_points(self._h, xy.ctypes.data, xy.shape[0],
                                                     out.ctypes.data))
        return out

    @property
    def sigma2(self) -> float:
        s2 = C.c_double()
        _lib.check(_lib.lib().mhs_tps_sigma2(self._h, C.byref(s2)))
        return s2.value

    def predict_se(self, xy, sigma2=None) -> np.ndarray:
        xy = np.asfortranarray(np.asarray(xy, dtype=np.float64).reshape(-1, 2))
        out = np.empty(xy.shape[0])
        s2 = math.nan if sigma2 is None else float(sigma2)
        _lib.check(_lib.lib().mhs_tps_predict_se_points(self._h, xy.ctypes.data, xy.shape[0], s2, out.ctypes.data))
        return out

    def eval_plan(self):
        tc, tr, a, b = C.c_int(0), C.c_int(0), C.c_int64(0), C.c_int64(0)
        _lib.check(_lib.lib().mhs_tps_eval_plan(self._h, C.byref(tc), C.byref(tr), C.byref(a), C.byref(b)))
        return tc.value, tr.value, a.value, b.value

    def __del__(self):
        h = getattr(self, "_h", None)
        if h is not None and _lib._lib is not None:
            _lib._lib.mhs_tps_free(h)
            self._h = None


def fit_many(xs, Ys, lambda_: float | None = None, gcv_mode: str = "fields"):
    lib = _lib.lib()
    k = len(xs)
    if len(Ys) != k:
        raise ValueError("xs and Ys have different lengths")
    xcm, ycm = [], []
    for x, Y in zip(xs, Ys):
        x = np.asarray(x, dtype=np.float64)
        if x.ndim != 2 or x.shape[1] != 2:
            raise ValueError("every x must be an N x 2 matrix of (LONG, LAT)")
        y = np.ascontiguousarray(np.asarray(Y, dtype=np.float64).reshape(-1))
        if y.shape[0] != x.shape[0]:
            raise ValueError("x and Y have different numbers of rows")
        xcm.append(np.asfortranarray(x)); ycm.append(y)
    _lib.init()
    px = (C.c_void_p * k)(*[a.ctypes.data for a in xcm])
    py = (C.c_void_p * k)(*[a.ctypes.data for a in ycm])
    ns = (C.c_int64 * k)(*[a.shape[0] for a in xcm])
    out = (C.c_void_p * k)()
    st = (C.c_int * k)()
    mode = {"fields": _lib.GCV_FIELDS, "converged": _lib.GCV_CONVERGED}[gcv_mode]
    lam = math.nan if lambda_ is None else float(lambda_)
    _lib.check(lib.mhs_tps_fit_many(px, py, ns, k, lam, mode, out, st))
    fits = []
    for i in range(k):
        if not out[i]:
            fits.append(None)
            continue
        t = Tps.__new__(Tps)
        t._h = C.c_void_p(out[i])
        t._pull()
        fits.append(t)
    return fits


def interpolate(geom: Geometry, model: Tps, window=None, out=None, stream=None, rows=None):
    import torch
    r0, r1, c0, c1 = window if window is not None else (0, geom.nrow, 0, geom.ncol)
    b0, b1 = rows if rows is not None else (r0, r1)
    dev = torch.device("cuda", _lib.init())
    if out is None:
        out = torch.empty((b1 - b0, c1 - c0), dtype=torch.float64, device=dev)
    if out.dtype != torch.float64 or not out.is_cuda or out.dim() != 2 or out.stride(1) != 1:
        raise ValueError("out must be a 2-D float64 device tensor with unit column stride")
    if tuple(out.shape) != (b1 - b0, c1 - c0):
        raise ValueError("out has the wrong shape for the window")
    g = geom.c_struct()
    s = stream if stream is not None else torch.cuda.current_stream(dev).cuda_stream
    if b1 > b0:
        _lib.check(_lib.lib().mhs_tps_predict_rows_dev(model._h, C.byref(g), r0, r1, c0, c1, b0, b1,
                                                       out.data_ptr(), out.stride(0), s))
    return out


def interpolate_se(geom: Geometry, model: Tps, window=None, out=None, stream=None, sigma2=None):
    import torch
    r0, r1, c0, c1 = window if window is not None else (0, geom.nrow, 0, geom.ncol)
    dev = torch.device("cuda", _lib.init())
    if out is None:
        out = torch.empty((r1 - r0, c1 - c0), dtype=torch.float64, device=dev)
    if out.dtype != torch.float64 or not out.is_cuda or out.dim() != 2 or out.stride(1) != 1:
        raise ValueError("out must be a 2-D float64 device tensor with unit column stride")
    if tuple(out.shape) != (r1 - r0, c1 - c0):
        raise ValueError("out has the wrong shape for the window")
    g = geom.c_struct()
    s = stream if stream is not None else torch.cuda.current_stream(dev).cuda_stream
    s2 = math.nan if sigma2 is None else float(sigma2)
    _lib.check(_lib.lib().mhs_tps_predict_se_grid_dev(model._h, C.byref(g), r0, r1, c0, c1, s2, out.data_ptr(),
                                                      out.stride(0), s))
    return out


EVAL_AUTO, EVAL_DIRECT, EVAL_FAR_FIELD = 0, 1, 2


@contextlib.contextmanager
def reduction_cache():
    _lib.init()
    _lib.check(_lib.lib().mhs_tps_reduction_cache(1))
    try:
        yield
    finally:
        _lib.check(_lib.lib().mhs_tps_reduction_cache(0))


def eval_mode(mode: int) -> None:
    _lib.init()
    _lib.check(_lib.lib().mhs_tps_eval_mode(int(mode)))
```

Measured before the change: 413.4 Mcells/s.

## Fuse ensemble add and station gather into TPS grid evaluation epilogue

Adds an epilogue to the TPS direct and far-field grid kernels that adds the ensemble prediction into the output and scatters values at station cells. This replaces the separate scale-add pass over the band and the host-side gather. It also reuses the rank-0 fit handle instead of rebuilding it from packed coefficients, and prebuilds a per-tile station plan. The cost is extra addend reads and station-loop work inside the eval kernels, plus a host-side station bucketing plan.

```diff
diff --git a/include/machisplin_hip.h b/include/machisplin_hip.h
--- a/include/machisplin_hip.h
+++ b/include/machisplin_hip.h
@@ -82,6 +82,12 @@
                              int64_t c0, int64_t c1, double *out_dev, int64_t ld, void *stream);
 MHS_API int mhs_tps_predict_rows_dev(const mhs_tps *t, const mhs_grid *g, int64_t r0, int64_t r1, int64_t c0, int64_t c1,
                                      int64_t b0, int64_t b1, double *out_dev, int64_t ld, void *stream);
+MHS_API int mhs_tps_predict_rows_add_dev(const mhs_tps *t, const mhs_grid *g, int64_t r0, int64_t r1, int64_t c0, int64_t c1,
+                                         int64_t b0, int64_t b1, const double *addend_dev, int64_t ld_add, double *out_dev,
+                                         int64_t ld, const int64_t *rows, const int64_t *cols, int64_t n, double *vals_dev,
+                                         void *stream);
+MHS_API int mhs_tps_plan_rows_dev(const mhs_tps *t, const mhs_grid *g, int64_t r0, int64_t r1, int64_t c0, int64_t c1,
+                                  int64_t b0, int64_t b1, const int64_t *rows, const int64_t *cols, int64_t n);
 MHS_API int mhs_tps_predict_points(const mhs_tps *t, const double *xy, int64_t n, double *out_host);
 
 #define MHS_TPS_SE_MAX_N 2048
diff --git a/machisplin_amd/_lib.py b/machisplin_amd/_lib.py
--- a/machisplin_amd/_lib.py
+++ b/machisplin_amd/_lib.py
@@ -86,6 +86,9 @@
     "mhs_tps_predict_grid": (C.c_int, [_vp, C.POINTER(Grid), _i64, _i64, _i64, _i64, _vp]),
     "mhs_tps_predict_grid_dev": (C.c_int, [_vp, C.POINTER(Grid), _i64, _i64, _i64, _i64, _vp, _i64, _vp]),
     "mhs_tps_predict_rows_dev": (C.c_int, [_vp, C.POINTER(Grid), _i64, _i64, _i64, _i64, _i64, _i64, _vp, _i64, _vp]),
+    "mhs_tps_predict_rows_add_dev": (C.c_int, [_vp, C.POINTER(Grid), _i64, _i64, _i64, _i64, _i64, _i64, _vp, _i64, _vp, _i64,
+                                               _vp, _vp, _i64, _vp, _vp]),
+    "mhs_tps_plan_rows_dev": (C.c_int, [_vp, C.POINTER(Grid), _i64, _i64, _i64, _i64, _i64, _i64, _vp, _vp, _i64]),
     "mhs_tps_predict_points": (C.c_int, [_vp, _vp, _i64, _vp]),
     "mhs_tps_sigma2": (C.c_int, [_vp, _dp]),
     "mhs_tps_predict_se_points": (C.c_int, [_vp, _vp, _i64, C.c_double, _vp]),
diff --git a/machisplin_amd/csrc/common.h b/machisplin_amd/csrc/common.h
--- a/machisplin_amd/csrc/common.h
+++ b/machisplin_amd/csrc/common.h
@@ -134,6 +134,9 @@
 int tps_free_quiet(mhs_tps *t);
 int tps_predict_rows_dev(const mhs_tps *t, const mhs_grid *g, int64_t r0, int64_t r1, int64_t c0, int64_t c1,
                          int64_t b0, int64_t b1, double *out_dev, int64_t ld, void *stream);
+int tps_predict_rows_add_dev(const mhs_tps *t, const mhs_grid *g, int64_t r0, int64_t r1, int64_t c0, int64_t c1,
+                             int64_t b0, int64_t b1, const double *addend_dev, int64_t ld_add, double *out_dev, int64_t ld,
+                             const int64_t *rows, const int64_t *cols, int64_t n, double *vals_dev, void *stream);
 }
 
 struct mhs_model;
@@ -168,7 +171,20 @@
         hipStream_t last_stream = nullptr;
         bool in_flight = false;
         int64_t node_pairs = 0, cell_pairs = 0;
+        int pre_lo = 0, pre_hi = 0;
+        hipEvent_t pre_done = nullptr;
     } far;
+    struct StationPlan {
+        std::vector<int64_t> rows, cols;
+        int64_t r0 = -1, r1 = -1, c0 = -1, c1 = -1;
+        int tx = 0, ty = 0, ntx = 0, nty = 0;
+        bool valid = false;
+        int *start_dev = nullptr;
+        int4 *rec_dev = nullptr;
+        size_t start_cap = 0, rec_cap = 0;
+        hipStream_t last_stream = nullptr;
+        bool in_flight = false;
+    } stations;
     std::mutex mu;
     std::shared_ptr<const mhs::TpsPrep> prep;
     mhs::SeState *se = nullptr;
diff --git a/machisplin_amd/csrc/multi.hip b/machisplin_amd/csrc/multi.hip
--- a/machisplin_amd/csrc/multi.hip
+++ b/machisplin_amd/csrc/multi.hip
@@ -696,7 +696,10 @@
                 if (cut[q + 1] > cut[q]) {
                     if (int rc2 = members_rows_dev(my + banded, weights + banded, n_models - banded, 1, 1, wt_total, &g, b.cov, b.r0, b.r1, ms->C,
                                                    ms->dtype, ms->ld, ms->nodata, cut[q], cut[q + 1], b.ens + off, g.ncol, M->s)) return rc2;
-                    if (int rc2 = mhs_scale_add_dev(b.ens + off, 1.0, b.tot + off, b.tot + off, (cut[q + 1] - cut[q]) * g.ncol, M->s)) return rc2;
+                    if (!tiled) {
+                        if (int rc2 = tps_predict_rows_add_dev(tps[(size_t)slot], &g, 0, g.nrow, 0, g.ncol, cut[q], cut[q + 1], b.ens + off, g.ncol,
+                                                               b.tot + off, g.ncol, nullptr, nullptr, 0, nullptr, M->s)) return rc2;
+                    } else if (int rc2 = mhs_scale_add_dev(b.ens + off, 1.0, b.tot + off, b.tot + off, (cut[q + 1] - cut[q]) * g.ncol, M->s)) return rc2;
                 }
                 MHS_HIP(hipEventRecord(M->dn[q], M->s));
             }
@@ -717,8 +720,9 @@
         if (!tiled) {
             if (slot != 0 && nb > 0)
                 TEAM_DO(team, mhs_tps_from_coef(S.knots_uv.data(), S.c.data(), S.d, S.nk, S.lambda, S.center, S.scale, &tps[(size_t)slot]));
-            if (nb > 0)
-                TEAM_DO(team, tps_predict_rows_dev(tps[(size_t)slot], &g, 0, g.nrow, 0, g.ncol, b.r0, b.r1, b.tot, g.ncol, M->s));
+            if (nb > 0 && !piped)
+                TEAM_DO(team, tps_predict_rows_add_dev(tps[(size_t)slot], &g, 0, g.nrow, 0, g.ncol, b.r0, b.r1, b.ens, g.ncol, b.tot, g.ncol,
+                                                       nullptr, nullptr, 0, nullptr, M->s));
             if (piped && nb > 0) {
                 const int rcd = team.failed() ? MHS_OK : down();
                 if (rcd) { (void)hipStreamSynchronize(M->u); team.fail(rcd); }
@@ -766,7 +770,7 @@
         }
         if (nb > 0 && !team.failed()) {
             auto step5 = [&]() -> int {
-                if (!piped) if (int rc2 = mhs_scale_add_dev(b.ens, 1.0, b.tot, b.tot, nb * g.ncol, M->s)) return rc2;
+                if (!piped && tiled) if (int rc2 = mhs_scale_add_dev(b.ens, 1.0, b.tot, b.tot, nb * g.ncol, M->s)) return rc2;
                 std::vector<int64_t> rr, cc, idx;
                 for (int64_t i = 0; i < n; ++i)
                     if (rows[(size_t)i] >= b.r0 && rows[(size_t)i] < b.r1 && cols[(size_t)i] >= 0) {
diff --git a/machisplin_amd/csrc/tps_eval.hip b/machisplin_amd/csrc/tps_eval.hip
--- a/machisplin_amd/csrc/tps_eval.hip
+++ b/machisplin_amd/csrc/tps_eval.hip
@@ -22,6 +22,27 @@
     int64_t ld;
 };
 
+struct EvalEpilogue {
+    const double *addend = nullptr;
+    int64_t ld_add = 0;
+    const int *st_start = nullptr;
+    const int4 *st = nullptr;
+    double *vals = nullptr;
+};
+
+__device__ __forceinline__ void eval_stations(const EvalEpilogue &ep, int b, int col, int row0, int lo, int hi,
+                                              const double (&res)[EVAL_ROWS]) {
+    const int s1 = ep.st_start[b + 1];
+    for (int s = ep.st_start[b]; s < s1; ++s) {
+        const int4 q = ep.st[s];
+        const int dr = q.x - row0;
+        if (q.y != col || dr < 0 || dr >= EVAL_ROWS || q.x < lo || q.x >= hi) continue;
+#pragma unroll
+        for (int k = 0; k < EVAL_ROWS; ++k)
+            if (dr == k) ep.vals[q.z] = res[k];
+    }
+}
+
 __device__ __forceinline__ void tps_accumulate(const Knot *__restrict__ knots, const int j0, const int j1,
                                                const double u, const double (&v)[EVAL_ROWS],
                                                double (&acc)[EVAL_ROWS], const double2 *tab) {
@@ -40,7 +61,8 @@
 }
 
 __device__ __forceinline__ void eval_direct_block(const Knot *__restrict__ knots, int n, const double2 *tab, const EvalGeom &g,
-                                                  double *__restrict__ out, int bx, int by) {
+                                                  double *__restrict__ out, int bx, int by, const EvalEpilogue &ep = EvalEpilogue(),
+                                                  int st_row0 = 0) {
     const int lane = threadIdx.x & 63;
     const int wave = threadIdx.x >> 6;
     const int col = bx * 64 + lane;
@@ -59,20 +81,26 @@
 
     tps_accumulate(knots, 0, n, u, v, acc, tab);
 
+    double res[EVAL_ROWS] = {};
     if (col < g.nc) {
 #pragma unroll
         for (int k = 0; k < EVAL_ROWS; ++k)
-            if (row0 + k < g.nr)
-                out[(int64_t)(row0 + k) * g.ld + col] = g.d0 + g.d1 * u + g.d2 * v[k] + acc[k];
+            if (row0 + k < g.nr) {
+                double r = g.d0 + g.d1 * u + g.d2 * v[k] + acc[k];
+                if (ep.addend) r = ep.addend[(int64_t)(row0 + k) * ep.ld_add + col] + r;
+                out[(int64_t)(row0 + k) * g.ld + col] = r;
+                res[k] = r;
+            }
+        if (ep.st_start) eval_stations(ep, 0, col, st_row0 + row0, st_row0, st_row0 + g.nr, res);
     }
 }
 
 __global__ __launch_bounds__(64 * EVAL_WAVES) void tps_eval_grid_kernel(
     const Knot *__restrict__ knots, int n, const double2 *__restrict__ gtab, EvalGeom g,
-    double *__restrict__ out) {
+    double *__restrict__ out, EvalEpilogue ep, int st_row0) {
     __shared__ double2 tab[LOG_TAB_N];
     stage_log_table(tab, gtab);
-    eval_direct_block(knots, n, tab, g, out, blockIdx.x, blockIdx.y);
+    eval_direct_block(knots, n, tab, g, out, blockIdx.x, blockIdx.y, ep, st_row0);
 }
 
 __global__ __launch_bounds__(256) void tps_eval_points_kernel(
@@ -156,7 +184,7 @@
                                                const double2 *__restrict__ gtab, const EvalGeom &g, const FarGeom &f,
                                                const double *__restrict__ nodes, const double *__restrict__ lx,
                                                const double *__restrict__ ly, double *__restrict__ out, FfCellsShared &sh,
-                                               int bx, int by_in) {
+                                               int bx, int by_in, const EvalEpilogue &ep = EvalEpilogue()) {
     const int lane = threadIdx.x & 63;
     const int wave = threadIdx.x >> 6;
     const int cchunks = f.tx / 64, rchunks = f.ty / EVAL_TILE_ROWS;
@@ -209,16 +237,20 @@
     if (col < g.nc) {
 #pragma unroll
         for (int k = 0; k < EVAL_ROWS; ++k)
-            if (row0 + k >= f.row_lo && row0 + k < f.row_hi) out[(int64_t)(row0 + k - f.row_lo) * g.ld + col] = acc[k];
+            if (row0 + k >= f.row_lo && row0 + k < f.row_hi) {
+                if (ep.addend) acc[k] = ep.addend[(int64_t)(row0 + k - f.row_lo) * ep.ld_add + col] + acc[k];
+                out[(int64_t)(row0 + k - f.row_lo) * g.ld + col] = acc[k];
+            }
+        if (ep.st_start) eval_stations(ep, tile, col, row0, f.row_lo, f.row_hi, acc);
     }
 }
 
 __global__ __launch_bounds__(64 * EVAL_WAVES) void tps_ff_cells_kernel(
     const Knot *__restrict__ knots, const int *__restrict__ bin_start, const double2 *__restrict__ gtab,
     EvalGeom g, FarGeom f, const double *__restrict__ nodes, const double *__restrict__ lx,
-    const double *__restrict__ ly, double *__restrict__ out) {
+    const double *__restrict__ ly, double *__restrict__ out, EvalEpilogue ep) {
     __shared__ FfCellsShared sh;
-    ff_cells_block(knots, bin_start, gtab, g, f, nodes, lx, ly, out, sh, blockIdx.x, blockIdx.y);
+    ff_cells_block(knots, bin_start, gtab, g, f, nodes, lx, ly, out, sh, blockIdx.x, blockIdx.y, ep);
 }
 
 struct EvalWindow {
@@ -396,6 +428,7 @@
                       P.r0 == e.r0 && P.r1 == r1 && P.c0 == e.c0 && P.c1 == c1 && P.tx == btx && P.ty == bty;
     if (same) return MHS_OK;
     if (P.in_flight) { MHS_HIP(hipStreamSynchronize(P.last_stream)); P.in_flight = false; }
+    P.pre_lo = P.pre_hi = 0;
     std::vector<int> start, order;
     far_plan_sort(N, e, *f, kc, kr, start, order, &P.node_pairs, &P.cell_pairs);
     std::vector<Knot> sorted((size_t)N);
@@ -419,6 +452,40 @@
     if (int rc = h2d_sync(P.ly_dev, ly.data(), sizeof(double) * ly.size())) return rc;
     P.xmin = e.xmin; P.ymax = e.ymax; P.xres = e.xres; P.yres = e.yres;
     P.r0 = e.r0; P.r1 = r1; P.c0 = e.c0; P.c1 = c1; P.tx = btx; P.ty = bty; P.ntx = f->ntx; P.nty = f->nty;
+    return MHS_OK;
+}
+
+static int plan_stations(mhs_tps *t, const EvalGeom &e, int64_t r1, int64_t c1, bool far, const FarGeom &f,
+                         const int64_t *rows, const int64_t *cols, int64_t n) {
+    mhs_tps::StationPlan &S = t->stations;
+    const int tx = far ? f.tx : 0, ty = far ? f.ty : 0, ntx = far ? f.ntx : 1, nty = far ? f.nty : 1;
+    if (S.valid && S.r0 == e.r0 && S.r1 == r1 && S.c0 == e.c0 && S.c1 == c1 && S.tx == tx && S.ty == ty &&
+        S.ntx == ntx && S.nty == nty && (int64_t)S.rows.size() == n &&
+        memcmp(S.rows.data(), rows, sizeof(int64_t) * (size_t)n) == 0 && memcmp(S.cols.data(), cols, sizeof(int64_t) * (size_t)n) == 0)
+        return MHS_OK;
+    S.valid = false;
+    if (S.in_flight) { MHS_HIP(hipStreamSynchronize(S.last_stream)); S.in_flight = false; }
+    const size_t nb = (size_t)ntx * (size_t)nty;
+    std::vector<int> start(nb + 1, 0), bucket((size_t)n, -1);
+    for (int64_t i = 0; i < n; ++i) {
+        const int64_t r = rows[i] - e.r0, c = cols[i] - e.c0;
+        if (r < 0 || r >= e.nr || c < 0 || c >= e.nc) continue;
+        bucket[(size_t)i] = far ? (int)(r / ty) * ntx + (int)(c / tx) : 0;
+        ++start[(size_t)bucket[(size_t)i] + 1];
+    }
+    for (size_t b = 0; b < nb; ++b) start[b + 1] += start[b];
+    std::vector<int> fill(start.begin(), start.end() - 1);
+    std::vector<int4> rec((size_t)start[nb]);
+    for (int64_t i = 0; i < n; ++i)
+        if (bucket[(size_t)i] >= 0)
+            rec[(size_t)fill[(size_t)bucket[(size_t)i]]++] = make_int4((int)(rows[i] - e.r0), (int)(cols[i] - e.c0), (int)i, 0);
+    if (int rc = grow(&S.start_dev, &S.start_cap, start.size())) return rc;
+    if (int rc = grow(&S.rec_dev, &S.rec_cap, rec.size())) return rc;
+    if (int rc = h2d_sync(S.start_dev, start.data(), sizeof(int) * start.size())) return rc;
+    if (int rc = h2d_sync(S.rec_dev, rec.data(), sizeof(int4) * rec.size())) return rc;
+    S.rows.assign(rows, rows + n); S.cols.assign(cols, cols + n);
+    S.r0 = e.r0; S.r1 = r1; S.c0 = e.c0; S.c1 = c1; S.tx = tx; S.ty = ty; S.ntx = ntx; S.nty = nty;
+    S.valid = true;
     return MHS_OK;
 }
 
@@ -571,6 +638,10 @@
 
 using namespace mhs;
 
+static int tps_rows_impl(const mhs_tps *t, const mhs_grid *g, int64_t r0, int64_t r1, int64_t c0, int64_t c1, int64_t b0, int64_t b1,
+                         const double *addend_dev, int64_t ld_add, double *out_dev, int64_t ld, const int64_t *rows,
+                         const int64_t *cols, int64_t n, double *vals_dev, void *stream, bool plan_only);
+
 extern "C" {
 
 int mhs_tps_from_coef(const double *knots_uv, const double *c, const double *d3, int64_t n,
@@ -617,7 +688,9 @@
 int mhs::tps_free_quiet(mhs_tps *t) {
     if (!t) return MHS_OK;
     for (void *q : {(void *)t->knots_dev, (void *)t->far.sorted_dev, (void *)t->far.bin_start_dev, (void *)t->far.nodes_dev,
-                    (void *)t->far.lx_dev, (void *)t->far.ly_dev}) pool_release(q);
+                    (void *)t->far.lx_dev, (void *)t->far.ly_dev, (void *)t->stations.start_dev, (void *)t->stations.rec_dev})
+        if (q) pool_release(q);
+    if (t->far.pre_done) (void)hipEventDestroy(t->far.pre_done);
     se_state_free(t->se);
     delete t;
     return MHS_OK;
@@ -656,12 +729,36 @@
     return tps_predict_rows_dev(t, g, r0, r1, c0, c1, b0, b1, out_dev, ld, stream);
 }
 
+int mhs_tps_predict_rows_add_dev(const mhs_tps *t, const mhs_grid *g, int64_t r0, int64_t r1, int64_t c0, int64_t c1,
+                                 int64_t b0, int64_t b1, const double *addend_dev, int64_t ld_add, double *out_dev, int64_t ld,
+                                 const int64_t *rows, const int64_t *cols, int64_t n, double *vals_dev, void *stream) {
+    return tps_predict_rows_add_dev(t, g, r0, r1, c0, c1, b0, b1, addend_dev, ld_add, out_dev, ld, rows, cols, n, vals_dev, stream);
+}
+
+int mhs_tps_plan_rows_dev(const mhs_tps *t, const mhs_grid *g, int64_t r0, int64_t r1, int64_t c0, int64_t c1,
+                          int64_t b0, int64_t b1, const int64_t *rows, const int64_t *cols, int64_t n) {
+    return tps_rows_impl(t, g, r0, r1, c0, c1, b0, b1, nullptr, 0, nullptr, c1 - c0, rows, cols, n, nullptr, nullptr, true);
+}
+
 }
 
 int mhs::tps_predict_rows_dev(const mhs_tps *t, const mhs_grid *g, int64_t r0, int64_t r1, int64_t c0, int64_t c1,
                               int64_t b0, int64_t b1, double *out_dev, int64_t ld, void *stream) {
+    return tps_rows_impl(t, g, r0, r1, c0, c1, b0, b1, nullptr, 0, out_dev, ld, nullptr, nullptr, 0, nullptr, stream, false);
+}
+int mhs::tps_predict_rows_add_dev(const mhs_tps *t, const mhs_grid *g, int64_t r0, int64_t r1, int64_t c0, int64_t c1,
+                                  int64_t b0, int64_t b1, const double *addend_dev, int64_t ld_add, double *out_dev, int64_t ld,
+                                  const int64_t *rows, const int64_t *cols, int64_t n, double *vals_dev, void *stream) {
+    return tps_rows_impl(t, g, r0, r1, c0, c1, b0, b1, addend_dev, ld_add, out_dev, ld, rows, cols, n, vals_dev, stream, false);
+}
+
+static int tps_rows_impl(const mhs_tps *t, const mhs_grid *g, int64_t r0, int64_t r1, int64_t c0, int64_t c1, int64_t b0, int64_t b1,
+                         const double *addend_dev, int64_t ld_add, double *out_dev, int64_t ld, const int64_t *rows,
+                         const int64_t *cols, int64_t n, double *vals_dev, void *stream, bool plan_only) {
     if (int rc = require_ready()) return rc;
-    MHS_REQUIRE(t && g && out_dev, "NULL argument");
+    MHS_REQUIRE(t && g && (out_dev || plan_only), "NULL argument");
+    MHS_REQUIRE(n >= 0 && n < (1LL << 31) && (n == 0 || (rows && cols && (vals_dev || plan_only))), "bad station list");
+    MHS_REQUIRE(!addend_dev || (addend_dev != out_dev && ld_add >= c1 - c0), "addend must be another plane, ld_add >= the window width");
     MHS_REQUIRE(g->nrow > 0 && g->ncol > 0 && g->xres > 0 && g->yres > 0, "bad grid geometry");
     MHS_REQUIRE(0 <= r0 && r0 <= r1 && r1 <= g->nrow && 0 <= c0 && c0 <= c1 && c1 <= g->ncol,
                 "window outside the grid");
@@ -676,21 +773,49 @@
     std::lock_guard<std::mutex> lk(tm->mu);
     if (int rc = plan_far(tm, g, e, r1, c1, &f, &far)) return rc;
     tm->far.last_used = far;
+    EvalEpilogue ep;
+    ep.addend = addend_dev; ep.ld_add = ld_add;
+    if (n > 0) {
+        if (int rc = plan_stations(tm, e, r1, c1, far, f, rows, cols, n)) return rc;
+        mhs_tps::StationPlan &S = tm->stations;
+        ep.st_start = S.start_dev; ep.st = S.rec_dev; ep.vals = vals_dev;
+        if (!plan_only) { S.last_stream = pick_stream(stream); S.in_flight = true; }
+    }
+    if (plan_only && !far) return MHS_OK;
     if (far) {
         mhs_tps::FarPlan &Pm = tm->far;
-        if (Pm.in_flight && Pm.last_stream != pick_stream(stream)) MHS_HIP(hipStreamSynchronize(Pm.last_stream));
-        Pm.last_stream = pick_stream(stream);
-        Pm.in_flight = true;
         const mhs_tps::FarPlan &P = t->far;
         f.row_lo = (int)(b0 - r0); f.row_hi = (int)(b1 - r0);
         f.ty_lo = f.row_lo / f.ty; f.ty_hi = (f.row_hi + f.ty - 1) / f.ty;
         const int ntiles = f.ntx * (f.ty_hi - f.ty_lo);
+        const bool ahead = Pm.pre_lo <= f.ty_lo && f.ty_hi <= Pm.pre_hi;
+        if (plan_only) {
+            if (ahead) return MHS_OK;
+            hipStream_t ls = ctx().stream;
+            if (Pm.in_flight && Pm.last_stream != ls) MHS_HIP(hipStreamSynchronize(Pm.last_stream));
+            if (!Pm.pre_done) MHS_HIP(hipEventCreateWithFlags(&Pm.pre_done, hipEventDisableTiming));
+            hipLaunchKernelGGL(tps_ff_nodes_kernel, dim3((unsigned)((ntiles + 3) / 4)), dim3(256), 0, ls,
+                               P.sorted_dev, (int)t->n, P.bin_start_dev, ctx().log_tab, e, f, P.nodes_dev);
+            MHS_HIP(hipGetLastError());
+            MHS_HIP(hipEventRecord(Pm.pre_done, ls));
+            Pm.pre_lo = f.ty_lo; Pm.pre_hi = f.ty_hi;
+            Pm.last_stream = ls; Pm.in_flight = true;
+            return MHS_OK;
+        }
+        if (ahead) MHS_HIP(hipStreamWaitEvent(pick_stream(stream), Pm.pre_done, 0));
+        else {
+            if (Pm.in_flight && Pm.last_stream != pick_stream(stream)) MHS_HIP(hipStreamSynchronize(Pm.last_stream));
+            Pm.pre_lo = Pm.pre_hi = 0;
+        }
+        Pm.last_stream = pick_stream(stream);
+        Pm.in_flight = true;
         dim3 cgrid((unsigned)(f.ntx * (f.tx / 64)), (unsigned)((f.ty_hi - f.ty_lo) * (f.ty / EVAL_TILE_ROWS)));
         MHS_REQUIRE(cgrid.y <= 65535u, "too many rows for one launch");
-        hipLaunchKernelGGL(tps_ff_nodes_kernel, dim3((unsigned)((ntiles + 3) / 4)), dim3(256), 0, pick_stream(stream),
-                           P.sorted_dev, (int)t->n, P.bin_start_dev, ctx().log_tab, e, f, P.nodes_dev);
+        if (!ahead)
+            hipLaunchKernelGGL(tps_ff_nodes_kernel, dim3((unsigned)((ntiles + 3) / 4)), dim3(256), 0, pick_stream(stream),
+                               P.sorted_dev, (int)t->n, P.bin_start_dev, ctx().log_tab, e, f, P.nodes_dev);
         hipLaunchKernelGGL(tps_ff_cells_kernel, cgrid, dim3(64 * EVAL_WAVES), 0, pick_stream(stream), P.sorted_dev,
-                           P.bin_start_dev, ctx().log_tab, e, f, P.nodes_dev, P.lx_dev, P.ly_dev, out_dev);
+                           P.bin_start_dev, ctx().log_tab, e, f, P.nodes_dev, P.lx_dev, P.ly_dev, out_dev, ep);
         MHS_HIP(hipGetLastError());
         return MHS_OK;
     }
@@ -698,7 +823,7 @@
     dim3 grid((unsigned)((eb.nc + 63) / 64), (unsigned)((eb.nr + EVAL_TILE_ROWS - 1) / EVAL_TILE_ROWS));
     MHS_REQUIRE(grid.y <= 65535u, "too many rows for one launch");
     hipLaunchKernelGGL(tps_eval_grid_kernel, grid, dim3(64 * EVAL_WAVES), 0, pick_stream(stream),
-                       t->knots_dev, (int)t->n, ctx().log_tab, eb, out_dev);
+                       t->knots_dev, (int)t->n, ctx().log_tab, eb, out_dev, ep, (int)(b0 - r0));
     MHS_HIP(hipGetLastError());
     return MHS_OK;
 }
diff --git a/machisplin_amd/sharded.py b/machisplin_amd/sharded.py
--- a/machisplin_amd/sharded.py
+++ b/machisplin_amd/sharded.py
@@ -124,25 +124,34 @@
                 ops.ensemble_band(self.r0, self.r1, self.pred[off:off + nb])
             knots, resid, resp, rows, cols = ops.station_residuals()
             n = knots.shape[0]
-            msg = torch.zeros(tps_msg_len(n), dtype=torch.float64, device=ops.device)
+            rows, cols = np.asarray(rows), np.asarray(cols)
+            fused = getattr(ops, "tps_band_add", None)
+            msg = torch.zeros(tps_msg_len(n), dtype=torch.float64, device=ops.device) if self.world > 1 else None
             if self.rank == 0:
                 packed0 = np.ascontiguousarray(ops.tps_fit(knots, resid))
-                msg[:packed0.size].copy_(torch.from_numpy(packed0))
+                plan = getattr(ops, "tps_plan", None)
+                if fused and plan and nb > 0:
+                    plan(self.r0, self.r1, rows, cols)
+                if msg is not None:
+                    msg[:packed0.size].copy_(torch.from_numpy(packed0))
         finally:
             if prev is not None:
                 reserve(prev)
         if self.world > 1:
             self.dist.broadcast(msg, src=0)
-        packed = msg.cpu().numpy()
-        rows, cols = np.asarray(rows), np.asarray(cols)
+        packed = packed0 if self.rank == 0 else msg.cpu().numpy()
         band_pred, band_tot = self.pred[off:off + nb], self.tot[off:off + nb]
         f_actual = np.zeros(n)
         if nb > 0:
-            ops.tps_band(packed, self.r0, self.r1, band_tot)
-            ops.add(band_pred, band_tot, band_tot)
             mine = (rows >= self.r0) & (rows < self.r1)
-            if mine.any():
-                f_actual[mine] = ops.gather(band_tot, rows[mine] - self.r0, cols[mine])
+            if fused:
+                vals = fused(packed, self.r0, self.r1, band_pred, band_tot, rows, cols)
+                f_actual[mine] = vals[mine]
+            else:
+                ops.tps_band(packed, self.r0, self.r1, band_tot)
+                ops.add(band_pred, band_tot, band_tot)
+                if mine.any():
+                    f_actual[mine] = ops.gather(band_tot, rows[mine] - self.r0, cols[mine])
         if self.world > 1:
             t = torch.from_numpy(f_actual).to(ops.device)
             self.dist.all_reduce(t)
@@ -276,6 +285,7 @@
         self.timed = timed
         self.timings = {"ensemble_ms": [], "tps_eval_ms": [], "tps_fit_ms": [], "residuals_ms": []}
         self.last_fit = None
+        self._retired = None
         self._pending = []
 
     def _timed(self, key, fn):
@@ -338,11 +348,40 @@
         t0 = time.perf_counter()
         fit = Tps(knots, resid, lambda_=self.lambda_, gcv_mode=self.gcv_mode)
         self.timings["tps_fit_ms"].append((time.perf_counter() - t0) * 1e3)
+        self._retired = self.last_fit
         self.last_fit = fit
-        return pack_tps(fit.knots, fit.c, fit.d, fit.center, fit.scale, fit.lambda_)
+        self._last_packed = pack_tps(fit.knots, fit.c, fit.d, fit.center, fit.scale, fit.lambda_)
+        return self._last_packed
+
+    def _handle_for(self, packed):
+        from .tps import Tps
+        mine = getattr(self, "_last_packed", None)
+        if self.last_fit is not None and mine is not None and np.array_equal(np.asarray(packed)[:mine.size], mine):
+            return self.last_fit
+        d = unpack_tps(packed)
+        return Tps.from_coef(d["knots"], d["c"], d["d"], d["lambda"], d["center"], d["scale"])
+
+    def tps_plan(self, r0, r1, rows, cols):
+        from .tps import plan_rows
+        plan_rows(self.stack.geom, self.last_fit, rows=(r0, r1), cells=(rows, cols))
+
+    def tps_band_add(self, packed, r0, r1, ens, out, rows, cols):
+        from .tps import interpolate_add
+        torch = self.torch
+        fit = self._handle_for(packed)
+        n = len(rows)
+        if getattr(self, "_vals", None) is None or self._vals.numel() != n:
+            self._vals = torch.full((n,), float("nan"), dtype=torch.float64, device=self.device)
+        self._timed("tps_eval_ms", lambda: interpolate_add(self.stack.geom, fit, addend=ens, out=out, rows=(r0, r1),
+                                                           cells=(rows, cols), vals=self._vals))
+        self.last_eval_plan = fit.eval_plan()
+        vals = self._vals.cpu().numpy()
+        self._retired = None
+        return vals
 
     def tps_band(self, packed, r0, r1, out):
         from .tps import Tps, interpolate
+        self._retired = None
         d = unpack_tps(packed)
         fit = Tps.from_coef(d["knots"], d["c"], d["d"], d["lambda"], d["center"], d["scale"])
         g = self.stack.geom
diff --git a/machisplin_amd/tps.py b/machisplin_amd/tps.py
--- a/machisplin_amd/tps.py
+++ b/machisplin_amd/tps.py
@@ -149,6 +149,57 @@
     return out
 
 
+def _cell_list(cells):
+    rows, cols = cells
+    rows = np.ascontiguousarray(rows, dtype=np.int64)
+    cols = np.ascontiguousarray(cols, dtype=np.int64)
+    if rows.ndim != 1 or rows.shape != cols.shape:
+        raise ValueError("cells must be two 1-D index arrays of equal length")
+    return rows, cols
+
+
+def interpolate_add(geom: Geometry, model: Tps, addend=None, out=None, rows=None, cells=None, vals=None, stream=None):
+    import torch
+    b0, b1 = rows if rows is not None else (0, geom.nrow)
+    dev = torch.device("cuda", _lib.init())
+    if out is None:
+        out = torch.empty((b1 - b0, geom.ncol), dtype=torch.float64, device=dev)
+    for name, a in (("out", out), ("addend", addend)):
+        if a is None:
+            continue
+        if a.dtype != torch.float64 or not a.is_cuda or a.dim() != 2 or a.stride(1) != 1 or tuple(a.shape) != (b1 - b0, geom.ncol):
+            raise ValueError(f"{name} must be a (b1 - b0) x ncol float64 device tensor with unit column stride")
+    n = 0
+    cr = cc = None
+    if cells is not None:
+        cr, cc = _cell_list(cells)
+        n = cr.shape[0]
+        if vals is None:
+            vals = torch.full((n,), float("nan"), dtype=torch.float64, device=dev)
+        if vals.dtype != torch.float64 or not vals.is_cuda or not vals.is_contiguous() or vals.numel() != n:
+            raise ValueError("vals must be a contiguous float64 device vector, one entry per cell")
+    g = geom.c_struct()
+    s = stream if stream is not None else torch.cuda.current_stream(dev).cuda_stream
+    if b1 > b0:
+        _lib.check(_lib.lib().mhs_tps_predict_rows_add_dev(
+            model._h, C.byref(g), 0, geom.nrow, 0, geom.ncol, b0, b1, None if addend is None else addend.data_ptr(),
+            0 if addend is None else addend.stride(0), out.data_ptr(), out.stride(0), None if n == 0 else cr.ctypes.data,
+            None if n == 0 else cc.ctypes.data, n, None if n == 0 else vals.data_ptr(), s))
+    return out, vals
+
+
+def plan_rows(geom: Geometry, model: Tps, rows=None, cells=None) -> None:
+    g = geom.c_struct()
+    b0, b1 = rows if rows is not None else (0, geom.nrow)
+    n = 0
+    cr = cc = None
+    if cells is not None:
+        cr, cc = _cell_list(cells)
+        n = cr.shape[0]
+    _lib.check(_lib.lib().mhs_tps_plan_rows_dev(model._h, C.byref(g), 0, geom.nrow, 0, geom.ncol, b0, b1,
+                                                None if n == 0 else cr.ctypes.data, None if n == 0 else cc.ctypes.data, n))
+
+
 def interpolate_se(geom: Geometry, model: Tps, window=None, out=None, stream=None, sigma2=None):
     import torch
     r0, r1, c0, c1 = window if window is not None else (0, geom.nrow, 0, geom.ncol)
```

New measurement: 414.6 Mcells/s (median of 5 runs). About the same (+0.3%).
